# soz223/multi_modal_normative_modeling

Hardware: AMD Instinct MI355X
Metric: cVAE training-steps/sec (batch 256, 379-ROI x 3-modality) (higher is better)
Workload: dtype bf16; 1 GPU; SE-gPoE cVAE_multimodal sweep: 3 x 379 ROI, batch 256, c=29, H=[110,110], Z=10, 5 folds x replicas, 256 independent models per GPU, in-kernel reparameterisation draw; jobs_per_gpu=256, steps_per_launch=128, params_per_model=355437, train_rows_per_model=1024, parallelism=sweep-sharded x1

## Files before the change

include/nmhip.h:

```cpp
#ifndef NMHIP_H
#define NMHIP_H

#include <stddef.h>
#include <stdint.h>

#ifdef __cplusplus
extern "C" {
#endif

#define NM_MAX_MOD 8
#define NM_MAX_EXP 4
#define NM_MAX_CLS 5
#define NM_MAX_CLS_WIDTH 512
#define NM_MAX_CLASSES 4
#define NM_MAX_HID 8
#define NM_BATCH   256
#define NM_MAX_WIDTH 127
#define NM_MAX_LATENT 64
#define NM_WIDE_MAX_WIDTH 4096
#define NM_WIDE_MAX_LATENT 128

enum {
  NM_OK            = 0,
  NM_E_NULL        = -1,
  NM_E_MODALITIES  = -2,
  NM_E_LAYERS      = -3,
  NM_E_WIDTH       = -4,
  NM_E_LATENT      = -5,
  NM_E_LATENT_COV  = -6,
  NM_E_PITCH       = -7,
  NM_E_GEOMETRY    = -8,
  NM_E_COMBINE     = -9,
  NM_E_OFFSETS     = -10,
  NM_E_REG_HEAD    = -11,
  NM_E_METRICS     = -12,
  NM_E_CLS_HEAD    = -13,
  NM_E_COUNTS      = -14,
  NM_E_SHADOW      = -15,
  NM_E_RESIDENCY   = -16,
  NM_E_PREP        = -17,
  NM_E_OUTPUT      = -18,
  NM_E_WIDE_TC     = -19,
  NM_E_ROWSPLIT    = -20,
  NM_E_N_PARAMS    = -21,
  NM_E_DEVPASS     = -22
};

enum { NM_COMBINE_POE = 0, NM_COMBINE_GPOE = 1, NM_COMBINE_MOE = 2, NM_COMBINE_MOPOE = 3,
       NM_COMBINE_POE2V = 4 };

enum {
  NM_F_BACKWARD = 1,
  NM_F_ADAM     = 2,
  NM_F_GRADS    = 4,
  NM_F_EXPORT   = 8,
  NM_F_PROFILE  = 16,
  NM_F_ZGIVEN   = 32,
  NM_F_TRACE    = 64,
  NM_F_BNSTATS  = 256,
  NM_F_SPLIT    = 512,
  NM_F_FAULT_INJECT = 1024
};

typedef struct nm_modality {
  int32_t D;
  int32_t Kx;
  int32_t x_pitch;
  int32_t Cz;
  const float*    x_f32;
  const uint16_t* xb;
  const uint16_t* cz;
  int64_t enc_w[NM_MAX_HID], enc_b[NM_MAX_HID];
  int64_t mu_w, mu_b, lv_w, lv_b;
  int64_t logvar_out;
  int64_t dec_w[NM_MAX_HID], dec_b[NM_MAX_HID];
  int64_t out_w, out_b;
  int64_t alpha;
  int64_t enc_s[NM_MAX_HID];
  int64_t heads_s;
  int64_t dec_s[NM_MAX_HID];
  int64_t out_s;
  float* out_loc;
  float* out_sqerr;
  float* out_rowdev;
  const float* dloc_extra;
  const float* dloc_rowcoef;
} nm_modality_t;

typedef struct nm_job {
  int32_t M;
  int32_t M_enc;
  int32_t C;
  int32_t L;
  int32_t Z;
  int32_t H[NM_MAX_HID];
  int32_t combine;
  int32_t single_bypass;
  int32_t n_rows;
  int32_t non_linear;
  float   act_slope;
  int32_t out_kind;
  int32_t n_private;
  float   var_floor;
  float   tc_weight;
  int64_t w_off;
  int32_t dephase;
  int32_t shared_cov;
  int32_t wide;
  int32_t loss_cap;
  int32_t eps_cap;
  float   lr, beta1, beta2, adam_eps;
  int64_t adam_off;
  const double* lr_table;
  int32_t lr_cap;
  float   kl_weight;
  float   ll_weight;
  float*  params;
  float*  adam_m;
  float*  adam_v;
  float*  grads;
  const float* eps;
  uint64_t seed;
  float*  loss_log;
  void*   wsh;
  void*   workspace;
  int64_t workspace_stride;
  float*  out_mu;
  float*  out_logvar;
  float*  out_z;
  const float* dz_extra;
  int32_t reg_head;
  float   reg_lambda;
  int64_t reg_w[3], reg_b[3];
  int64_t reg_s;
  uint16_t* reg_resid;
  uint16_t* reg_dres;
  const float* fi_target;
  float*  out_fi_pred;
  int32_t cls_layers;
  int32_t cls_classes;
  int32_t cls_width[NM_MAX_CLS];
  int32_t cls_train;
  int32_t cls_use_mu;
  int64_t cls_w[NM_MAX_CLS + 1], cls_b[NM_MAX_CLS + 1];
  int64_t cls_bn_w[NM_MAX_CLS], cls_bn_b[NM_MAX_CLS];
  int64_t cls_bn_mean[NM_MAX_CLS], cls_bn_var[NM_MAX_CLS];
  float   cls_dropout;
  float   cls_margin;
  float   cls_w_ce;
  float   cls_w_contrast;
  const int32_t* labels;
  float*  out_logits;
  float*  dz_out;
  float*  rowcoef_out[NM_MAX_MOD];
  float*  gpart;
  int64_t gpart_stride;
  int64_t n_params;
  nm_modality_t mod[NM_MAX_MOD];
} nm_job_t;

#define NM_LOSS_STRIDE 16
#define NM_LOSS_TOTAL 0
#define NM_LOSS_KL    1
#define NM_LOSS_LL    2
#define NM_LOSS_LL_M  3
#define NM_LOSS_TC    11
#define NM_LOSS_REG   12
#define NM_LOSS_CE    13
#define NM_LOSS_CONTRAST 14

int64_t nm_fill_shadow(nm_job_t* job_host);

int nm_sync_shadow(const nm_job_t* jobs_dev, int n_jobs, void* stream);

int64_t nm_workspace_bytes(const nm_job_t* job_host);

int64_t nm_workspace_offset(const nm_job_t* job_host, int what);

int nm_validate_job(const nm_job_t* job_host);

int nm_launch(const nm_job_t* jobs_dev, int n_jobs, int step0, int steps_per_tile, int n_tiles,
              int flags, void* stream);

int nm_launch_split(const nm_job_t* jobs_dev, int n_jobs, int parts, int step0, int n_steps, int flags, void* stream);
int nm_launch_wide(const nm_job_t* jobs_dev, int n_jobs, int step0, int steps_per_tile, int n_tiles, int flags, void* stream);
int nm_launch_rowsplit(const nm_job_t* jobs_dev, int n_jobs, int M, int k, int helpers, int step0, int n_steps, int flags,
                       int spread_us, void* stream);
int nm_launch_rowsplit_mixed(const nm_job_t* jobs_dev, int n_jobs, const int* job_M_host, int k, int helpers, int step0,
                             int n_steps, int flags, int spread_us, void* stream);
#define NM_RS_MAX_GROUPS 128
#define NM_RS_GROUP_PAD  65535
int nm_rowsplit_groups(const int* job_M_host, int n_jobs, int* table_out, int cap);
#define NM_RS_MAX_PASSES 128
#define NM_RS_MAX_VSEGS  144
#define NM_RS_MAX_VEC    3072
int nm_rowsplit_ok(const nm_job_t* job_host);
int nm_sync_reset(const nm_job_t* jobs_dev, int n_jobs, void* stream);
int nm_devpass(const nm_job_t* jobs_dev, int n_jobs, int tile0, int n_tiles, int flags, void* stream);
int nm_trace_read_dv(unsigned long long* out512, int reset);
int nm_devpass_ok(const nm_job_t* job_host);
int nm_devpass_multi(const nm_job_t* jobs_dev, int n_jobs, int tile0, int n_tiles, int flags, void* stream);
int nm_devpass_multi_ok(const nm_job_t* job_host);
int nm_latent_pass(const nm_job_t* jobs_dev, int n_jobs, int tile0, int n_tiles, int flags, void* stream);
int nm_latent_pass_ok(const nm_job_t* job_host);
int nm_trace_read_rs(unsigned long long* out512, int reset);
#define NM_SYNC_ERR_TIMEOUT 1
#define NM_SYNC_ERR_SHAPE   2
int nm_split_errors(const nm_job_t* jobs_dev, int n_jobs, int* out_dev, int clear, void* stream);

int nm_train_steps(const nm_job_t* jobs_dev, int n_jobs, int step0, int n_steps, void* stream);
int nm_grads(const nm_job_t* jobs_dev, int n_jobs, int step, void* stream);
int nm_forward(const nm_job_t* jobs_dev, int n_jobs, int tile0, int n_tiles, void* stream);

int nm_head_regression(const nm_job_t* jobs_dev, int n_jobs, int step, int tile0, int n_tiles, int flags,
                       void* stream);

int nm_head_classifier(const nm_job_t* jobs_dev, int n_jobs, int step, int tile0, int n_tiles, int flags,
                       void* stream);

int nm_train_steps_head(const nm_job_t* jobs_dev, int n_jobs, int step0, int n_steps, int flags, void* stream);

int nm_train_steps_head_split(const nm_job_t* jobs_dev, int n_jobs, int parts, int step0, int n_steps, int flags, void* stream);

#define NM_METRICS_MAX_N  8192
#define NM_METRICS_STRIDE 8
int nm_posthoc_metrics(const float* scores, const int32_t* labels, const int32_t* offsets, int n_sets, int max_set,
                       const double* thr_in, double* out, void* stream);
int nm_confusion_metrics(const int32_t* pred, const int32_t* labels, const int32_t* offsets, int n_sets, double* out,
                         void* stream);
int nm_latent_stats(const float* mu, const int32_t* offsets, int n_sets, int Z, int pitch, float* mean_out, float* var_out,
                    void* stream);
int nm_latent_score(const float* mu, const float* logvar, const int32_t* offsets, int n_sets, int Z, int pitch,
                    const float* mean, const float* var, float* zsep_out, float* score_out, void* stream);

#define NM_ROI_Y_CHUNK 128
typedef struct { const float* x; const int32_t* group; int32_t rows; int32_t pitch; } nm_roi_set_t;
int nm_roi_effect(const nm_roi_set_t* sets_dev, int n_sets, int D, int max_rows, double* out, void* stream);

#define NM_ROI_MAX_PERM   65535
#define NM_ROI_PERM_CHUNK 64
#define NM_ROI_ROW_CHUNK  256
size_t nm_roi_significance_workspace(int n_sets, int D, int max_rows, int n_perm);
int nm_roi_significance(const nm_roi_set_t* sets_dev, int n_sets, int D, int max_rows, int n_perm, uint64_t seed,
                        void* workspace, size_t workspace_bytes, double* out, int32_t* maxstat_out, void* stream);

#define NM_BOOT_MAX   16384
#define NM_BOOT_CHUNK 64
size_t nm_auc_bootstrap_workspace(int n_sets, int max_set, int n_boot, int n_pairs);
int nm_auc_bootstrap(const float* scores, const int32_t* labels, const int32_t* offsets, const int32_t* streams,
                     int n_sets, int max_set, int n_boot, int lo_index, int hi_index, uint64_t seed,
                     const int32_t* pairs, int n_pairs, void* workspace, size_t workspace_bytes,
                     double* out, double* pairs_out, int32_t* boot_out, void* stream);

#define NM_REG_OLS      0
#define NM_REG_LOGIT    1
#define NM_REG_MAX_COV  4
#define NM_REG_MAX_ITER 35
#define NM_REG_TOL      1e-8
typedef struct nm_reg_set {
  const float*   x;
  const float*   target;
  const float*   cov;
  const int32_t* include;
  int32_t rows, pitch, cov_pitch, pad;
} nm_reg_set_t;
int nm_column_regress(const nm_reg_set_t* sets_dev, int n_sets, int D, int max_rows, int n_cov, int kind,
                      double* out , void* stream);
double nm_student_t_two_sided(double t, double df);

int nm_combine_latent(const float* mus, const float* variances, int M, int64_t n, int combine, const float* alpha_raw,
                      int single_bypass, int in_log, int out_log, float var_floor, float* out_mu, float* out_var,
                      void* stream);
int nm_total_correlation(const float* qz_xs, int M, int B, int Z, float* out, void* stream);

int nm_train_steps_persistent(const nm_job_t* jobs_dev, int n_jobs, int step0, int n_steps, void* stream);
int nm_deviation(const nm_job_t* jobs_dev, int n_jobs, int tile0, int n_tiles, void* stream);

int nm_adam_step(float* params, const float* grads, float* m, float* v, int64_t n,
                 float lr, float beta1, float beta2, float eps, int64_t t, void* stream);

int64_t nm_xb_elems(int rows_alloc, int Kx);
int nm_pack_table(const float* x, const float* c, int n_rows, int rows_alloc, int D, int C, int Kx,
                  uint16_t* xb, float* x_f32_out, int x_pitch, uint16_t* cz_out, int Cz, void* stream);

#define NM_PREP_MAX_ROWS 8192
int nm_prep_scaler_fit(const double* const* srcs_dev, const int32_t* src_D_dev, int n_src, int D, const int32_t* rows_dev,
                       int n_rows, double* center_dev, double* scale_dev, void* stream);
int nm_prep_onehot(const double* age_dev, const double* gender_dev, const int32_t* rows_dev, int n_rows, const double* age_edges_dev,
                   int age_bins, const double* gender_edges_dev, int gender_bins, float* c_out_dev, void* stream);
int nm_pack_table_raw(const double* const* srcs_dev, const int32_t* src_D_dev, int n_src, const int32_t* rows_dev, int n_rows,
// ... 23 lines not shown
```

multi_modal_normative_modeling_amd/_lib.py:

```python
from __future__ import annotations

import ctypes as C
from pathlib import Path

NM_MAX_MOD = 8
NM_MAX_EXP = 4
NM_RS_MAX_PASSES = 128
NM_RS_MAX_VSEGS = 144
NM_RS_MAX_VEC = 3 * 2 * 512
NM_RS_MAX_GROUPS = 128
NM_RS_GROUP_PAD = 65535
NM_MAX_HID = 8
NM_MAX_CLS = 5
NM_MAX_CLS_WIDTH = 512
NM_MAX_CLASSES = 4
NM_BATCH = 256
NM_MAX_WIDTH = 127
NM_MAX_LATENT = 64
NM_WIDE_MAX_WIDTH = 4096
NM_WIDE_MAX_LATENT = 128
NM_LOSS_STRIDE = 16

NM_COMBINE = {"poe": 0, "gpoe": 1, "moe": 2, "mopoe": 3, "poe2v": 4}

NM_F_BACKWARD = 1
NM_F_ADAM = 2
NM_F_GRADS = 4
NM_F_EXPORT = 8
NM_F_PROFILE = 16
NM_F_ZGIVEN = 32
NM_F_TRACE = 64
NM_LOSS_TC = 11
NM_LOSS_REG = 12
NM_LOSS_CE = 13
NM_LOSS_CONTRAST = 14
NM_F_BNSTATS = 256
NM_F_SPLIT = 512
NM_F_FAULT_INJECT = 1024
NM_SYNC_ERR_TIMEOUT = 1
NM_SYNC_ERR_SHAPE = 2
NM_METRICS_MAX_N = 8192
NM_METRICS_STRIDE = 8
NM_ROI_Y_CHUNK = 128
NM_ROI_MAX_PERM = 65535
NM_ROI_PERM_CHUNK = 64
NM_ROI_ROW_CHUNK = 256
NM_BOOT_MAX = 16384
NM_BOOT_CHUNK = 64
NM_REG_OLS = 0
NM_REG_LOGIT = 1
NM_REG_MAX_COV = 4
NM_REG_MAX_ITER = 35
NM_REG_TOL = 1e-8

NM_OK = 0
NM_E_NULL = -1
NM_E_MODALITIES = -2
NM_E_LAYERS = -3
NM_E_WIDTH = -4
NM_E_LATENT = -5
NM_E_LATENT_COV = -6
NM_E_PITCH = -7
NM_E_GEOMETRY = -8
NM_E_COMBINE = -9
NM_E_OFFSETS = -10
NM_E_REG_HEAD = -11
NM_E_METRICS = -12
NM_E_CLS_HEAD = -13
NM_E_COUNTS = -14
NM_E_SHADOW = -15
NM_E_RESIDENCY = -16
NM_E_PREP = -17
NM_E_OUTPUT = -18
NM_E_WIDE_TC = -19
NM_E_ROWSPLIT = -20
NM_E_N_PARAMS = -21
NM_E_DEVPASS = -22

LIB_PATH = Path(__file__).resolve().parent / "libnmhip.so"


class NmModality(C.Structure):
    _fields_ = [
        ("D", C.c_int32), ("Kx", C.c_int32), ("x_pitch", C.c_int32), ("Cz", C.c_int32),
        ("x_f32", C.c_void_p), ("xb", C.c_void_p), ("cz", C.c_void_p),
        ("enc_w", C.c_int64 * NM_MAX_HID), ("enc_b", C.c_int64 * NM_MAX_HID),
        ("mu_w", C.c_int64), ("mu_b", C.c_int64), ("lv_w", C.c_int64), ("lv_b", C.c_int64),
        ("logvar_out", C.c_int64),
        ("dec_w", C.c_int64 * NM_MAX_HID), ("dec_b", C.c_int64 * NM_MAX_HID),
        ("out_w", C.c_int64), ("out_b", C.c_int64),
        ("alpha", C.c_int64),
        ("enc_s", C.c_int64 * NM_MAX_HID), ("heads_s", C.c_int64), ("dec_s", C.c_int64 * NM_MAX_HID), ("out_s", C.c_int64),
        ("out_loc", C.c_void_p), ("out_sqerr", C.c_void_p), ("out_rowdev", C.c_void_p),
        ("dloc_extra", C.c_void_p), ("dloc_rowcoef", C.c_void_p),
    ]


class NmJob(C.Structure):
    _fields_ = [
        ("M", C.c_int32), ("M_enc", C.c_int32), ("C", C.c_int32), ("L", C.c_int32), ("Z", C.c_int32),
        ("H", C.c_int32 * NM_MAX_HID),
        ("combine", C.c_int32), ("single_bypass", C.c_int32), ("n_rows", C.c_int32), ("non_linear", C.c_int32),
        ("act_slope", C.c_float), ("out_kind", C.c_int32), ("n_private", C.c_int32),
        ("var_floor", C.c_float), ("tc_weight", C.c_float), ("w_off", C.c_int64), ("dephase", C.c_int32), ("shared_cov", C.c_int32), ("wide", C.c_int32),
        ("loss_cap", C.c_int32), ("eps_cap", C.c_int32),
        ("lr", C.c_float), ("beta1", C.c_float), ("beta2", C.c_float), ("adam_eps", C.c_float),
        ("adam_off", C.c_int64), ("lr_table", C.c_void_p), ("lr_cap", C.c_int32),
        ("kl_weight", C.c_float), ("ll_weight", C.c_float),
        ("params", C.c_void_p), ("adam_m", C.c_void_p), ("adam_v", C.c_void_p), ("grads", C.c_void_p),
        ("eps", C.c_void_p), ("seed", C.c_uint64),
        ("loss_log", C.c_void_p), ("wsh", C.c_void_p), ("workspace", C.c_void_p), ("workspace_stride", C.c_int64),
        ("out_mu", C.c_void_p), ("out_logvar", C.c_void_p), ("out_z", C.c_void_p), ("dz_extra", C.c_void_p),
        ("reg_head", C.c_int32), ("reg_lambda", C.c_float), ("reg_w", C.c_int64 * 3), ("reg_b", C.c_int64 * 3),
        ("reg_s", C.c_int64), ("reg_resid", C.c_void_p), ("reg_dres", C.c_void_p),
        ("fi_target", C.c_void_p), ("out_fi_pred", C.c_void_p),
        ("cls_layers", C.c_int32), ("cls_classes", C.c_int32), ("cls_width", C.c_int32 * NM_MAX_CLS),
        ("cls_train", C.c_int32), ("cls_use_mu", C.c_int32),
        ("cls_w", C.c_int64 * (NM_MAX_CLS + 1)), ("cls_b", C.c_int64 * (NM_MAX_CLS + 1)),
        ("cls_bn_w", C.c_int64 * NM_MAX_CLS), ("cls_bn_b", C.c_int64 * NM_MAX_CLS),
        ("cls_bn_mean", C.c_int64 * NM_MAX_CLS), ("cls_bn_var", C.c_int64 * NM_MAX_CLS),
        ("cls_dropout", C.c_float), ("cls_margin", C.c_float), ("cls_w_ce", C.c_float), ("cls_w_contrast", C.c_float),
        ("labels", C.c_void_p), ("out_logits", C.c_void_p), ("dz_out", C.c_void_p),
        ("rowcoef_out", C.c_void_p * NM_MAX_MOD),
        ("gpart", C.c_void_p), ("gpart_stride", C.c_int64), ("n_params", C.c_int64),
        ("mod", NmModality * NM_MAX_MOD),
    ]


class NmRoiSet(C.Structure):
    _fields_ = [("x", C.c_void_p), ("group", C.c_void_p), ("rows", C.c_int32), ("pitch", C.c_int32)]


class NmRegSet(C.Structure):
    _fields_ = [("x", C.c_void_p), ("target", C.c_void_p), ("cov", C.c_void_p), ("include", C.c_void_p),
                ("rows", C.c_int32), ("pitch", C.c_int32), ("cov_pitch", C.c_int32), ("pad", C.c_int32)]


class NmError(RuntimeError):
    pass


_lib = None


def load():
    global _lib
    if _lib is not None:
        return _lib
    if not LIB_PATH.exists():
        raise NmError(
            f"{LIB_PATH} is missing: build it with `python -c 'import __graft_entry__ as g; g.build()'` "
            f"(hipcc --offload-arch=gfx950).  There is no CPU fallback for the product path.")
    lib = C.CDLL(str(LIB_PATH))
    vp, i32, i64, f32 = C.c_void_p, C.c_int, C.c_int64, C.c_float
    lib.nm_version.restype = C.c_int
    lib.nm_status_string.restype = C.c_char_p
    lib.nm_status_string.argtypes = [C.c_int]
    lib.nm_abi_sizes.argtypes = [C.POINTER(i64), C.POINTER(i64)]
    lib.nm_workspace_bytes.restype = i64
    lib.nm_fill_shadow.restype = i64
    lib.nm_fill_shadow.argtypes = [C.POINTER(NmJob)]
    lib.nm_sync_shadow.argtypes = [vp, i32, vp]
    lib.nm_xb_elems.restype = i64
    lib.nm_xb_elems.argtypes = [i32, i32]
    lib.nm_workspace_bytes.argtypes = [C.POINTER(NmJob)]
    lib.nm_workspace_offset.restype = i64
    lib.nm_workspace_offset.argtypes = [C.POINTER(NmJob), i32]
    lib.nm_validate_job.argtypes = [C.POINTER(NmJob)]
    for name in ("nm_launch", "nm_launch_scalar_tr"):
        getattr(lib, name).argtypes = [vp, i32, i32, i32, i32, i32, vp]
    lib.nm_launch_split.argtypes = [vp, i32, i32, i32, i32, i32, vp]
    lib.nm_launch_wide.argtypes = [vp, i32, i32, i32, i32, i32, vp]
    lib.nm_split_errors.argtypes = [vp, i32, vp, i32, vp]
    lib.nm_launch_rowsplit.argtypes = [vp, i32, i32, i32, i32, i32, i32, i32, i32, vp]
    lib.nm_launch_rowsplit_mixed.argtypes = [vp, i32, C.POINTER(i32), i32, i32, i32, i32, i32, i32, vp]
    lib.nm_rowsplit_groups.argtypes = [C.POINTER(i32), i32, C.POINTER(i32), i32]
    lib.nm_rowsplit_ok.argtypes = [C.POINTER(NmJob)]
    lib.nm_sync_reset.argtypes = [vp, i32, vp]
    lib.nm_trace_read_rs.argtypes = [C.POINTER(C.c_ulonglong), i32]
    lib.nm_devpass.argtypes = [vp, i32, i32, i32, i32, vp]
    lib.nm_trace_read_dv.argtypes = [C.POINTER(C.c_ulonglong), i32]
    lib.nm_devpass_ok.argtypes = [C.POINTER(NmJob)]
    lib.nm_devpass_multi.argtypes = [vp, i32, i32, i32, i32, vp]
    lib.nm_devpass_multi_ok.argtypes = [C.POINTER(NmJob)]
    lib.nm_latent_pass.argtypes = [vp, i32, i32, i32, i32, vp]
    lib.nm_latent_pass_ok.argtypes = [C.POINTER(NmJob)]
    lib.nm_latent_stats.argtypes = [vp, vp, i32, i32, i32, vp, vp, vp]
    lib.nm_latent_score.argtypes = [vp, vp, vp, i32, i32, i32, vp, vp, vp, vp, vp]
    lib.nm_combine_latent.argtypes = [vp, vp, i32, i64, i32, vp, i32, i32, i32, f32, vp, vp, vp]
    lib.nm_total_correlation.argtypes = [vp, i32, i32, i32, vp, vp]
    lib.nm_train_steps.argtypes = [vp, i32, i32, i32, vp]
    lib.nm_train_steps_persistent.argtypes = [vp, i32, i32, i32, vp]
    lib.nm_deviation.argtypes = [vp, i32, i32, i32, vp]
    lib.nm_grads.argtypes = [vp, i32, i32, vp]
    lib.nm_forward.argtypes = [vp, i32, i32, i32, vp]
    lib.nm_head_regression.argtypes = [vp, i32, i32, i32, i32, i32, vp]
    lib.nm_head_classifier.argtypes = [vp, i32, i32, i32, i32, i32, vp]
    lib.nm_train_steps_head.argtypes = [vp, i32, i32, i32, i32, vp]
    lib.nm_train_steps_head.restype = i32
    lib.nm_train_steps_head_split.argtypes = [vp, i32, i32, i32, i32, i32, vp]
    lib.nm_train_steps_head_split.restype = i32
    lib.nm_posthoc_metrics.argtypes = [vp, vp, vp, i32, i32, vp, vp, vp]
    lib.nm_confusion_metrics.argtypes = [vp, vp, vp, i32, vp, vp]
    lib.nm_roi_effect.argtypes = [vp, i32, i32, i32, vp, vp]
    lib.nm_roi_significance_workspace.restype = C.c_size_t
    lib.nm_roi_significance_workspace.argtypes = [i32, i32, i32, i32]
    lib.nm_roi_significance.argtypes = [vp, i32, i32, i32, i32, C.c_uint64, vp, C.c_size_t, vp, vp, vp]
    lib.nm_auc_bootstrap_workspace.restype = C.c_size_t
    lib.nm_auc_bootstrap_workspace.argtypes = [i32, i32, i32, i32]
    lib.nm_auc_bootstrap.argtypes = [vp, vp, vp, vp, i32, i32, i32, i32, i32, C.c_uint64, vp, i32, vp, C.c_size_t, vp, vp, vp, vp]
    lib.nm_column_regress.argtypes = [vp, i32, i32, i32, i32, i32, vp, vp]
    lib.nm_student_t_two_sided.restype = C.c_double
    lib.nm_student_t_two_sided.argtypes = [C.c_double, C.c_double]
    lib.nm_adam_step.argtypes = [vp, vp, vp, vp, i64, f32, f32, f32, f32, i64, vp]
    lib.nm_pack_table.argtypes = [vp, vp, i32, i32, i32, i32, i32, vp, vp, i32, vp, i32, vp]
    lib.nm_prep_scaler_fit.argtypes = [vp, vp, i32, i32, vp, i32, vp, vp, vp]
    lib.nm_prep_onehot.argtypes = [vp, vp, vp, i32, vp, i32, vp, i32, vp, vp]
    lib.nm_pack_table_raw.argtypes = [vp, vp, i32, vp, i32, vp, vp, vp, i32, i32, i32, i32, vp, vp, i32, vp, i32, vp]
    lib.nm_test_gemm.argtypes = [i32, vp, vp, vp, i32, i32, i32, vp]
    lib.nm_prof_read.argtypes = [C.POINTER(C.c_ulonglong), i32]
    lib.nm_trace_read.argtypes = [C.POINTER(C.c_ulonglong), i32]
    lib.nm_wgtimes_read.argtypes = [C.POINTER(C.c_ulonglong)]
    sj, sm = i64(0), i64(0)
    lib.nm_abi_sizes(C.byref(sj), C.byref(sm))
    if sj.value != C.sizeof(NmJob) or sm.value != C.sizeof(NmModality):
        raise NmError(f"ABI mismatch: C sizeof(nm_job_t)={sj.value}, sizeof(nm_modality_t)={sm.value}; "
                      f"ctypes {C.sizeof(NmJob)}, {C.sizeof(NmModality)}")
    _lib = lib
    return lib


EXPORTED_SYMBOLS = [
    "nm_version", "nm_status_string", "nm_abi_sizes", "nm_workspace_bytes", "nm_validate_job", "nm_launch",
    "nm_launch_scalar_tr", "nm_train_steps", "nm_grads", "nm_forward", "nm_adam_step", "nm_pack_table",
    "nm_test_gemm", "nm_prof_read", "nm_trace_read", "nm_wgtimes_read", "nm_head_regression", "nm_head_classifier", "nm_train_steps_head", "nm_train_steps_head_split", "nm_train_steps_persistent", "nm_deviation", "nm_posthoc_metrics", "nm_confusion_metrics",
    "nm_fill_shadow", "nm_sync_shadow", "nm_xb_elems", "nm_launch_split", "nm_launch_wide", "nm_split_errors", "nm_combine_latent", "nm_total_correlation",
    "nm_prep_scaler_fit", "nm_prep_onehot", "nm_pack_table_raw",
    "nm_launch_rowsplit", "nm_rowsplit_ok", "nm_sync_reset", "nm_trace_read_rs", "nm_devpass", "nm_devpass_ok", "nm_trace_read_dv", "nm_workspace_offset",
    "nm_launch_rowsplit_mixed", "nm_rowsplit_groups", "nm_devpass_multi", "nm_devpass_multi_ok",
    "nm_latent_pass", "nm_latent_pass_ok", "nm_latent_stats", "nm_latent_score",
    "nm_roi_effect", "nm_roi_significance_workspace", "nm_roi_significance",
    "nm_auc_bootstrap_workspace", "nm_auc_bootstrap",
    "nm_column_regress", "nm_student_t_two_sided",
]


def check(status: int, what: str = "nmhip"):
    if status != 0:
        msg = load().nm_status_string(status).decode()
        raise NmError(f"{what} failed with status {status}: {msg}")
```

multi_modal_normative_modeling_amd/csrc/nm_core.inc:

```
#include <hip/hip_runtime.h>
#include <stdint.h>
#include <math.h>
#include "nmhip.h"
#include "nm_host.inc"

namespace {

constexpr int NWM = 2;
constexpr int NWN = 4;
constexpr int NWAVES = NWM * NWN;
constexpr int WG = NWAVES * 64;
constexpr int TROWS = NM_BATCH;
constexpr int RT = NM_BATCH / (NWM * 16);
constexpr int WROWS = RT * 16;
constexpr int ROWS = NM_BATCH;
#define NM_GEOM(RTV)                                                                                              \
  [[maybe_unused]] constexpr int RT = (RTV), WROWS = (RTV) * 16, ROWS = (RTV) * 32, XIMG_BYTES = ROWS * LDX * 2, \
                                 ACT_BYTES = ROWS * LDP * 2
constexpr int PW = 128;
constexpr int LDP = 136;
constexpr int LDX = 72;
constexpr int XCH = 64;
constexpr int STAGE_FLOATS = 4608;
constexpr int IMG_ROWS = 128;
constexpr int IMG_BYTES = IMG_ROWS * LDP * 2;
constexpr int VEC_BYTES = 1024;
constexpr int BLOB_BYTES = IMG_BYTES + VEC_BYTES;
constexpr int XIMG_BYTES = ROWS * LDX * 2;
constexpr int XIMG_TILE_BYTES = TROWS * LDX * 2;
constexpr int W0IMG_BYTES = 128 * LDX * 2;
constexpr int OCH = 64;
constexpr int OIMG_BYTES = OCH * LDP * 2;
constexpr int OBLOB_BYTES = 18432;
constexpr int ACT_BYTES = ROWS * LDP * 2;
constexpr int ROWS_BYTES_P = NM_BATCH * LDP * 2;
constexpr int PATCH_FLOATS = 16 * 16;
constexpr int SPATCH_OFF = 8192;
constexpr float LOG_SQRT_2PI = 0.91893853320467274178f;

typedef __attribute__((ext_vector_type(4))) float f32x4;
typedef __attribute__((ext_vector_type(8))) __bf16 bf16x8;
typedef __attribute__((ext_vector_type(4))) __bf16 bf16x4;
typedef __attribute__((ext_vector_type(4))) unsigned u32x4;

#define GAS __attribute__((address_space(1)))
typedef GAS float* gf32;
typedef const GAS float* gcf32;
typedef GAS __bf16* gbf16;
typedef const GAS __bf16* gcbf16;

__device__ unsigned long long nm_prof_cycles[32];
__device__ unsigned long long nm_trace_cycles[8][64];
__device__ unsigned long long nm_wg_times[512][2];

struct Ctx {
  unsigned long long t_last;
  const nm_job_t* job;
  __bf16* P;
  __bf16* Q;
  float* stage;
  float* vec;
  int part, nparts;
  int rsk, rsq, rloc0;
  int x_pre;
  GAS float* gpart;
  int64_t gp_stride;
  GAS char* ws0;
  int xwg;
  int gwt;
  int lstep;
  float slope;
  float* red;
  float* colacc;
  float* rowacc;
  float* lse;
  float* bgrad;
  unsigned* abort;
  unsigned long long* tlast;
  int wave_s;
  int tid, lane, wave, wm, wn, g, c16;
  int row0;
  int nrows;
  int flags;
  float inv_b;
  float step_size;
  float inv_bc2_sqrt;
  GAS char* ws;
};

__host__ __device__ inline int rup(int x, int m) { return (x + m - 1) / m * m; }
__host__ __device__ inline int wpad(int n) { return rup(n + 1, 32); }

constexpr int WS_RS_TAB_BYTES = 8192;
struct WsLayout {
  int64_t sync, rs_tab, mu_m, lv_m, mu_j, lv_j, es, dz, enc_act, dec_act, zc, total;
  int64_t lat, act;
  int Zs;
};
constexpr int WS_SYNC_BYTES = 256;
constexpr int WS_SYNC_ERR_WORD = 32;
constexpr unsigned WS_SYNC_ERR_TIMEOUT = NM_SYNC_ERR_TIMEOUT, WS_SYNC_ERR_SHAPE = NM_SYNC_ERR_SHAPE;
constexpr int WS_SYNC_C_WORD = 33, WS_SYNC_D_WORD = 40, WS_SYNC_LOSS_WORD = 48, WS_SYNC_XCC_WORD = 57;
__host__ __device__ inline WsLayout ws_layout(int M, int L, int Z) {
  WsLayout w;
  w.Zs = rup(Z, 16);
  int64_t o = 0;
  w.sync = o; o += WS_SYNC_BYTES;
  w.rs_tab = o; o += (int64_t)NM_MAX_EXP * WS_RS_TAB_BYTES;
  const int64_t lat = (int64_t)ROWS * w.Zs * 4;
  w.lat = lat;
  w.mu_m = o; o += lat * M * 2;
  w.lv_m = o; o += lat * M * 2;
  w.mu_j = o; o += lat * M;
  w.lv_j = o; o += lat * M;
  w.es = o; o += lat * M;
  w.dz = o; o += lat * M;
  const int64_t act = (int64_t)ROWS * LDP * 2;
  w.act = act;
  w.enc_act = o; o += act * M * L;
  w.dec_act = o; o += act * M * L;
  w.zc = o; o += act * M;
  w.total = (o + 255) / 256 * 256;
  return w;
}

enum { PH_ENC_L0 = 0, PH_ENC_REST, PH_HEADS, PH_LATENT, PH_DEC_ZC, PH_DEC_HID, PH_OUT_GEMM, PH_OUT_DLV, PH_OUT_DGRAD,
       PH_OUT_WGRAD, PH_NLL_RED, PH_DEC_FINISH, PH_DEC_LOAD, PH_DEC_DGRAD, PH_DEC_WGRAD, PH_DEC_DELTA, PH_ALPHA,
       PH_ENCB_PREP, PH_ENCB_HEADS_DGRAD, PH_ENCB_HEADS_WGRAD, PH_ENCB_LOAD, PH_ENCB_DGRAD, PH_ENCB_WGRAD,
       PH_ENCB_DELTA, PH_ENCB_L0_WGRAD, PH_X_LOADS, PH_X_MFMA, PH_X_EPI, PH_COUNT };
__device__ __forceinline__ void tr(const Ctx& c, int tag) {
  if ((c.flags & 64) && blockIdx.x == 0 && blockIdx.y == 0) {
    unsigned long long t = clock64();
    const int w = c.wave_s;
    nm_trace_cycles[w][tag] += t - c.tlast[w];
    c.tlast[w] = t;
  }
}
__device__ __forceinline__ void prof(Ctx& c, int phase) {
  if ((c.flags & NM_F_PROFILE) && blockIdx.x == 0 && blockIdx.y == 0 && c.wave_s == 0) {
    unsigned long long t = clock64();
    nm_prof_cycles[phase] += t - c.t_last;
    c.t_last = t;
  }
}

__device__ __forceinline__ void relaunder(Ctx& c) {
  int l = (int)__builtin_amdgcn_mbcnt_hi(~0u, __builtin_amdgcn_mbcnt_lo(~0u, 0u));
  asm volatile("" : "+v"(l));
  int w = c.wave_s;
  asm volatile("" : "+s"(w));
  c.lane = l;
  c.tid = w * 64 + l;
  c.wave = w;
  c.wm = w / NWN;
  c.wn = w % NWN;
  c.g = c.lane >> 4;
  c.c16 = c.lane & 15;
}

template <class T>
__device__ __forceinline__ GAS T* asg(T* p) {
  return (GAS T*)p;
}

__device__ __forceinline__ void lds_barrier() {
  asm volatile("s_waitcnt lgkmcnt(0)" ::: "memory");
  __builtin_amdgcn_s_barrier();
}

__device__ __forceinline__ float lrelu(float v, bool nl, float slope) { return (nl && v < 0.f) ? v * slope : v; }

__device__ __forceinline__ float fx_exp(float x) { return __builtin_amdgcn_exp2f(x * 1.4426950408889634f); }
__device__ __forceinline__ float fx_log(float x) { return __builtin_amdgcn_logf(x) * 0.6931471805599453f; }
__device__ __forceinline__ float fx_rcp(float x) { return __builtin_amdgcn_rcpf(x); }

__device__ __forceinline__ unsigned lds_addr(const void* p) {
  return (unsigned)(size_t)(const __attribute__((address_space(3))) void*)p;
}

__device__ __forceinline__ int idiv(int a, int b, float rb) {
  int q = (int)((float)a * rb);
  q += ((q + 1) * b <= a) ? 1 : 0;
  q -= (q * b > a) ? 1 : 0;
  return q;
// ... 674 lines not shown
    for (int rt = 0; rt < RT; ++rt) {
      bf16x8 a = lds_frag(A, lda, c.wm * WROWS + rt * 16 + c.c16, n_col0 + s * 32 + 8 * c.g);
      acc[0][rt] = mfma(wf0, a, acc[0][rt]);
      acc[1][rt] = mfma(wf1, a, acc[1][rt]);
    }
  }
}
template <int RTV>
__device__ __forceinline__ const __bf16* dgrad_hidden(const Ctx& cc, f32x4 (&acc)[2][RTV], const GAS char* w_img,
                                                      const GAS char* act_img, int N, int K) {
  NM_GEOM(RTV);
  Ctx c = cc;
  relaunder(c);
  char* Qb = reinterpret_cast<char*>(c.Q);
  dma_img(c, w_img, Qb, N, blob_kp(K), (const GAS char*)c.job->wsh);
  if (RTV < 8) {
    const int n_act = dma_act(c, act_img, Qb + IMG_BYTES, 0, ROWS, act_segs(K));
    wait_vm(n_act);
    lds_barrier();
    dgrad_tile(c, acc, c.P, LDP, 0, c.Q, LDP, wpad(N) / 32);
    return c.Q + IMG_ROWS * LDP;
  }
  const int n_hi = dma_act(c, act_img, Qb + IMG_BYTES, ROWS / 2, ROWS / 2, act_segs(K));
  wait_vm(n_hi);
  lds_barrier();
  dgrad_tile(c, acc, c.P, LDP, 0, c.Q, LDP, wpad(N) / 32);
  lds_barrier();
  dma_act(c, act_img, Qb, 0, ROWS / 2, act_segs(K));
  return c.Q;
}

template <int RTV>
__device__ __forceinline__ void finish_delta(const Ctx& cc, const f32x4 (&acc)[2][RTV], const __bf16* src, int K,
                                             bool act) {
  NM_GEOM(RTV);
  Ctx c = cc;
  relaunder(c);
  const int ntk = wpad(K) / 16;
#pragma unroll
  for (int t = 0; t < 2; ++t) {
    int kt = c.wn + 4 * t;
    if (kt >= ntk) continue;
    int k0 = kt * 16 + 4 * c.g;
#pragma unroll
    for (int rt = 0; rt < RT; ++rt) {
      int r = c.wm * WROWS + rt * 16 + c.c16;
      bf16x4 a = *reinterpret_cast<const bf16x4*>(src + r * LDP + k0);
      bf16x4 pk;
#pragma unroll
      for (int i = 0; i < 4; ++i) {
        float d = acc[t][rt][i];
        if (act && !((float)a[i] > 0.f)) d *= c.slope;
        if (k0 + i >= K) d = 0.f;
        pk[i] = (__bf16)d;
      }
      *reinterpret_cast<bf16x4*>(c.P + r * LDP + k0) = pk;
    }
  }
}

struct WgT {
  int64_t w_off;
  int64_t b_off;
  GAS char* sh;
  int sh_pitch;
  GAS float* sh_b;
  float* patch;
};
struct WgGeom { int N, K, k_base, ncols; WgT T; };
struct PMV { f32x4 p0, m0, v0, p1, m1, v1; };
__device__ __forceinline__ int wg_units(const WgGeom& G) { return ((G.N + 15) >> 4) * ((((G.ncols + 15) >> 4) + 1) >> 1); }
__device__ __forceinline__ int wg_bias_pair(const WgGeom& G) {
  const bool has_bias = (G.T.b_off >= 0) && (G.K >= G.k_base) && (G.K < G.k_base + G.ncols);
  return has_bias ? ((G.K - G.k_base) >> 5) : -1;
}
#define NM_GLOAD16(dst, voff, sbase) \
  asm volatile("s_nop 4\n\tglobal_load_dwordx4 %0, %1, %2" : "+v"(dst) : "v"(voff), "s"(sbase) : "memory")
#define NM_GLOAD16_NT(dst, voff, sbase) \
  asm volatile("s_nop 4\n\tglobal_load_dwordx4 %0, %1, %2 nt" : "+v"(dst) : "v"(voff), "s"(sbase) : "memory")
#define NM_GLOAD4(dst, voff, sbase) \
  asm volatile("s_nop 4\n\tglobal_load_dword %0, %1, %2" : "+v"(dst) : "v"(voff), "s"(sbase) : "memory")
constexpr int WG_LOADS = 6;

template <bool SCALAR_TR, int RTV = RT, bool PART = false>
__device__ __forceinline__ int wgrad_adam(const Ctx& cc, const __bf16* A, int lda, int a_col0, const __bf16* B, int ldb,
                                          const WgGeom& G, int pending = -1, int b_chunk = 0, float* bgrad_buf = nullptr) {
  NM_GEOM(RTV);
  Ctx c = cc;
  relaunder(c);
  const nm_job_t* J = c.job;
  const WgT& T = G.T;
  const int N = G.N, K = G.K, k_base = G.k_base, ncols = G.ncols;
  const int KT = ktiles(K), kt0 = k_base >> 4;
  const int nktp = (ncols + 15) >> 4;
  const int nkp = (nktp + 1) >> 1;
  const int nunits = wg_units(G);
  const int kb = K - k_base;
  const int kb_pair = wg_bias_pair(G), kb_j = (kb >> 4) & 1, kb_col = kb & 15;
  const bool do_adam = !PART && (c.flags & NM_F_ADAM) != 0;
  const bool do_grads = !PART && (c.flags & NM_F_GRADS) != 0;
  const AdamK ak = adam_consts(c);
  gf32 Pp = asg(J->params), Mp = asg(J->adam_m), Vp = asg(J->adam_v);
  float* patch = T.patch + c.wave * PATCH_FLOATS;
  float* const bgp = bgrad_buf ? bgrad_buf : c.bgrad;
  const int prow = c.lane >> 2, pcol = (c.lane & 3) * 4;
  float* const pw = patch + c.c16 * 16 + 4 * (c.g ^ ((c.c16 >> 1) & 3));
  const float* const pr = patch + prow * 16 + 4 * ((c.lane & 3) ^ ((prow >> 1) & 3));
  const float* const pb = patch + prow * 16 + 4 * ((kb_col >> 2) ^ ((prow >> 1) & 3)) + (kb_col & 3);
  const unsigned lane16 = (unsigned)c.lane << 4;

  const bool bias_wave = kb_pair >= 0 && do_adam && c.wave < 2;
  float bp, bm, bv;
  asm volatile("" : "=v"(bp), "=v"(bm), "=v"(bv));
  if (bias_wave) {
    const unsigned boff = (unsigned)(T.b_off + min(c.tid, N - 1)) << 2;
    NM_GLOAD4(bp, boff, Pp); NM_GLOAD4(bm, boff, Mp); NM_GLOAD4(bv, boff, Vp);
  }
  int young = 0;

  auto issue = [&](int u, PMV& s) {
    const int nt = u / nkp, kp = u - nt * nkp;
    const int ktl0 = 2 * kp, ktl1 = 2 * kp + 1;
    const bool v0 = ktl0 < nktp && kt0 + ktl0 < KT, v1 = ktl1 < nktp && kt0 + ktl1 < KT;
    const unsigned o0 = (v0 ? (unsigned)((T.w_off + ((int64_t)(nt * KT + kt0 + ktl0) << 8)) << 2) : 0u) + lane16;
    const unsigned o1 = (v1 ? (unsigned)((T.w_off + ((int64_t)(nt * KT + kt0 + ktl1) << 8)) << 2) : 0u) + lane16;
    NM_GLOAD16(s.p0, o0, Pp); NM_GLOAD16_NT(s.m0, o0, Mp); NM_GLOAD16_NT(s.v0, o0, Vp);
    NM_GLOAD16(s.p1, o1, Pp); NM_GLOAD16_NT(s.m1, o1, Mp); NM_GLOAD16_NT(s.v1, o1, Vp);
  };
  auto wait_set = [&](PMV& s, int younger) {
    wait_vm(younger);
    asm volatile("" : "+v"(s.p0), "+v"(s.m0), "+v"(s.v0), "+v"(s.p1), "+v"(s.m1), "+v"(s.v1));
  };
  auto unit_mfma = [&](int u, f32x4 (&acc)[2]) {
    const int nt = u / nkp, kp = u - nt * nkp;
    acc[0] = f32x4{0.f, 0.f, 0.f, 0.f}; acc[1] = acc[0];
    const int ncol0 = a_col0 + nt * 16;
    const __bf16* const Bu = b_chunk ? B + (kp >> 1) * b_chunk : B;
    const int kcol = b_chunk ? (kp & 1) * 32 : kp * 32;
    if (SCALAR_TR) {
      for (int rs = 0; rs < ROWS / 32; ++rs) {
        bf16x8 nf = lds_frag_tr_scalar(A, lda, rs * 32, ncol0, c.lane);
        acc[0] = mfma(lds_frag_tr_scalar(Bu, ldb, rs * 32, kcol, c.lane), nf, acc[0]);
        acc[1] = mfma(lds_frag_tr_scalar(Bu, ldb, rs * 32, kcol + 16, c.lane), nf, acc[1]);
      }
    } else {
      unsigned na = tr_addr_il(A, lda, 0, ncol0, c.lane);
      unsigned ka = tr_addr_il(Bu, ldb, 0, kcol, c.lane);
      const unsigned n_step = 32u * lda * 2u, k_step = 32u * ldb * 2u;
      const unsigned n4 = 1u * lda * 2u, k4 = 1u * ldb * 2u;
#pragma unroll 2
      for (int rs = 0; rs < ROWS / 32; rs += 2) {
        bf16x4 n0v, n1v, n2v, n3v, a0, a1, a2, a3, b0, b1, b2, b3;
        unsigned na1 = na + n4, ka1 = ka + k4, na2 = na + n_step, ka2 = ka + k_step;
        unsigned na3 = na2 + n4, ka3 = ka2 + k4;
        NM_TR_READ(n0v, na, 0);  NM_TR_READ(n1v, na1, 0);
        NM_TR_READ(a0, ka, 0);   NM_TR_READ(a1, ka1, 0);
        NM_TR_READ(b0, ka, 32);  NM_TR_READ(b1, ka1, 32);
        NM_TR_READ(n2v, na2, 0); NM_TR_READ(n3v, na3, 0);
        NM_TR_READ(a2, ka2, 0);  NM_TR_READ(a3, ka3, 0);
        NM_TR_READ(b2, ka2, 32); NM_TR_READ(b3, ka3, 32);
        asm volatile("s_waitcnt lgkmcnt(0)"
                     : "+v"(n0v), "+v"(n1v), "+v"(n2v), "+v"(n3v), "+v"(a0), "+v"(a1), "+v"(a2), "+v"(a3), "+v"(b0),
                       "+v"(b1), "+v"(b2), "+v"(b3));
        bf16x8 nf0 = join4(n0v, n1v), nf1 = join4(n2v, n3v);
        acc[0] = mfma(join4(a0, a1), nf0, acc[0]);
        acc[1] = mfma(join4(b0, b1), nf0, acc[1]);
        acc[0] = mfma(join4(a2, a3), nf1, acc[0]);
        acc[1] = mfma(join4(b2, b3), nf1, acc[1]);
        na += 2 * n_step; ka += 2 * k_step;
      }
    }
  };
  auto finish_unit = [&](int u, PMV& s, const f32x4 (&acc)[2]) {
    const int nt = u / nkp, kp = u - nt * nkp;
    const int n = nt * 16 + prow;
    int nst = 0;
    if constexpr (PART) {
      const int nr = nt * 16 + c.c16;
#pragma unroll
      for (int j = 0; j < 2; ++j) {
        const int ktl = 2 * kp + j;
        f32x4 g = acc[j];
        const int k0 = k_base + ktl * 16 + 4 * c.g;
        if (nt * 16 + 16 > N || k_base + ktl * 16 + 16 > K) {
#pragma unroll
          for (int i = 0; i < 4; ++i) g[i] = (nr < N && k0 + i < K) ? g[i] : 0.f;
        }
        if (ktl < nktp && kt0 + ktl < KT) {
          const int64_t idx = T.w_off + ((int64_t)(nt * KT + kt0 + ktl) << 8) + c.c16 * 16 + 4 * c.g;
          st16_g(c, c.gpart + idx, g);
          ++nst;
        }
        if (kp == kb_pair && j == kb_j) {
          if (c.g == (kb_col >> 2) && nr < N) bgp[nr] = acc[j][kb_col & 3];
        }
      }
      return nst;
    }
#pragma unroll
    for (int j = 0; j < 2; ++j) {
      const int ktl = 2 * kp + j;
      *reinterpret_cast<f32x4*>(pw) = acc[j];
      f32x4 g = *reinterpret_cast<const f32x4*>(pr);
      const float bg = *pb;
      const int k0 = k_base + ktl * 16 + pcol;
      if (nt * 16 + 16 > N || k_base + ktl * 16 + 16 > K) {
#pragma unroll
        for (int i = 0; i < 4; ++i) g[i] = (n < N && k0 + i < K) ? g[i] : 0.f;
      }
      if (ktl < nktp && kt0 + ktl < KT) {
        const int64_t idx = T.w_off + ((int64_t)(nt * KT + kt0 + ktl) << 8) + c.lane * 4;
        if (do_grads) { *(GAS f32x4*)(asg(J->grads) + idx) = g; ++nst; }
        if (do_adam) {
          f32x4 p4 = j ? s.p1 : s.p0, m4 = j ? s.m1 : s.m0, v4 = j ? s.v1 : s.v0;
#pragma unroll
          for (int i = 0; i < 4; ++i) { float pp = p4[i], mm = m4[i], v2 = v4[i]; adam1(ak, g[i], pp, mm, v2); p4[i] = pp; m4[i] = mm; v4[i] = v2; }
          *(GAS f32x4*)(Pp + idx) = p4;
          __builtin_nontemporal_store(m4, (GAS f32x4*)(Mp + idx));
          __builtin_nontemporal_store(v4, (GAS f32x4*)(Vp + idx));
          nst += 3;
          if (T.sh) {
            bf16x4 pk;
#pragma unroll
            for (int i = 0; i < 4; ++i) pk[i] = (__bf16)p4[i];
            *(GAS bf16x4*)(T.sh + (int64_t)n * T.sh_pitch + (ktl * 16 + pcol) * 2) = pk;
            ++nst;
          }
        }
      }
      if (kp == kb_pair && j == kb_j) {
        if (pcol == 0 && n < N) bgp[n] = bg;
      }
    }
    return nst;
  };

  PMV sa, sb;
  asm volatile("" : "=v"(sa.p0), "=v"(sa.m0), "=v"(sa.v0), "=v"(sa.p1), "=v"(sa.m1), "=v"(sa.v1));
  asm volatile("" : "=v"(sb.p0), "=v"(sb.m0), "=v"(sb.v0), "=v"(sb.p1), "=v"(sb.m1), "=v"(sb.v1));
  int u = c.wave, st_prev = 0;
  if (do_adam && u < nunits) { issue(u, sa); young += WG_LOADS; }
  if (pending >= 0) {
    wait_vm(min(pending + young + (bias_wave ? 3 : 0), 20));
    lds_barrier();
  }
  while (u < nunits) {
    f32x4 acc[2];
    const int u1 = u + NWAVES, u2 = u + 2 * NWAVES;
    const bool h1 = do_adam && u1 < nunits;
    if (h1) { issue(u1, sb); young += WG_LOADS; }
    unit_mfma(u, acc);
    if (do_adam) wait_set(sa, st_prev + (h1 ? WG_LOADS : 0));
    st_prev = finish_unit(u, sa, acc);
    young += st_prev;
    if (u1 >= nunits) break;
    const bool h2 = do_adam && u2 < nunits;
    if (h2) { issue(u2, sa); young += WG_LOADS; }
    unit_mfma(u1, acc);
    if (do_adam) wait_set(sb, st_prev + (h2 ? WG_LOADS : 0));
    st_prev = finish_unit(u1, sb, acc);
    young += st_prev;
    u = u2;
  }
  lds_barrier();
  if (PART) {
    if (kb_pair >= 0) {
      relaunder(c);
      for (int n = c.tid; n < N; n += WG) st4_g(c, c.gpart + T.b_off + n, bgp[n]);
    }
  } else if (kb_pair >= 0 && c.wave < 2) {
    relaunder(c);
    if (bias_wave) { wait_vm(min(young, 20)); asm volatile("" : "+v"(bp), "+v"(bm), "+v"(bv)); }
    const int n = c.tid;
    if (n < N) {
      const float bg = bgp[n];
      const int64_t bidx = T.b_off + n;
      if (do_grads) asg(J->grads)[bidx] = bg;
      if (do_adam) {
        adam1(ak, bg, bp, bm, bv);
        Pp[bidx] = bp; Mp[bidx] = bm; Vp[bidx] = bv;
        if (T.sh_b) T.sh_b[n] = bp;
      }
    }
  }
  return young;
}

__device__ __forceinline__ WgGeom geom_out(const nm_job_t* J, const nm_modality_t& md, int ch, float* patch) {
  const int Hl = J->H[0], d0 = ch * OCH, valid = min(OCH, md.D - d0);
  GAS char* const oimg = (GAS char*)J->wsh + md.out_s + (int64_t)ch * OBLOB_BYTES;
  return WgGeom{valid, Hl, 0, rup(Hl + 1, 16),
                WgT{md.out_w + (int64_t)(d0 >> 4) * ktiles(Hl) * 256, md.out_b + d0, oimg, LDP * 2, (GAS float*)(oimg + OIMG_BYTES), patch}};
}
__device__ __forceinline__ WgGeom geom_dec(const nm_job_t* J, const nm_modality_t& md, int d, float* patch) {
  const int L = J->L, Kin = (d == 0) ? J->Z + J->C : J->H[L - d], Nout = J->H[L - 1 - d];
  GAS char* const dimg = (GAS char*)J->wsh + md.dec_s[d];
  return WgGeom{Nout, Kin, 0, rup(Kin + 1, 16),
                WgT{md.dec_w[d], md.dec_b[d], dimg, blob_kp(Kin) * 2, (GAS float*)(dimg + cimg_bytes(Nout, Kin)), patch}};
}
__device__ __forceinline__ WgGeom geom_head(const nm_job_t* J, const nm_modality_t& md, int which, float* patch) {
  const int Hh = J->H[J->L - 1], Zs = rup(J->Z, 16), hkp = blob_kp(Hh);
  GAS char* const img = (GAS char*)J->wsh + md.heads_s;
  GAS float* const hvec = (GAS float*)(img + cimg_bytes(2 * Zs, Hh));
  return which == 0 ? WgGeom{J->Z, Hh, 0, rup(Hh + 1, 16), WgT{md.mu_w, md.mu_b, img, hkp * 2, hvec, patch}}
                    : WgGeom{J->Z, Hh, 0, rup(Hh + 1, 16), WgT{md.lv_w, md.lv_b, img + (int64_t)Zs * hkp * 2, hkp * 2, hvec + Zs, patch}};
}
__device__ __forceinline__ WgGeom geom_enc(const nm_job_t* J, const nm_modality_t& md, int e, float* patch) {
  const int Kin = J->H[e - 1], Nout = J->H[e];
  GAS char* const eimg = (GAS char*)J->wsh + md.enc_s[e];
  return WgGeom{Nout, Kin, 0, rup(Kin + 1, 16),
                WgT{md.enc_w[e], md.enc_b[e], eimg, blob_kp(Kin) * 2, (GAS float*)(eimg + cimg_bytes(Nout, Kin)), patch}};
}
__device__ __forceinline__ WgGeom geom_l0(const nm_job_t* J, const nm_modality_t& md, int kc, float* patch) {
  const int Kx = md.Kx, K0 = md.D + J->C, N0 = J->H[0];
  GAS char* const img = (GAS char*)J->wsh + md.enc_s[0];
  return WgGeom{N0, K0, kc * XCH, min(XCH, Kx - kc * XCH),
                WgT{md.enc_w[0], md.enc_b[0], img + (int64_t)kc * XCH * 2, Kx * 2, (GAS float*)(img + l0_img_bytes(N0, Kx)), patch}};
}

__device__ __forceinline__ int experts(const nm_job_t* J) { return J->M_enc > 0 ? J->M_enc : J->M; }
__host__ __device__ inline int head_chunk0(const nm_job_t* J, int m) {
  int q = 0;
  for (int i = 0; i < m; ++i) q += (J->mod[i].D + XCH - 1) / XCH;
  return q;
}
struct Fuse { float mu, lv, var; };
struct Lat { float mu[NM_MAX_EXP], lv[NM_MAX_EXP]; };
__device__ __forceinline__ void softmax_alpha(const nm_job_t* J, float (&al)[NM_MAX_EXP]) {
#pragma clang fp contract(off)
  float mx = -INFINITY;
#pragma unroll
  for (int m = 0; m < NM_MAX_EXP; ++m)
    if (m < experts(J)) mx = fmaxf(mx, asg(J->params)[J->mod[m].alpha]);
  float s = 0.f;
#pragma unroll
  for (int m = 0; m < NM_MAX_EXP; ++m) {
    al[m] = (m < experts(J)) ? fx_exp(asg(J->params)[J->mod[m].alpha] - mx) : 0.f;
    s += al[m];
  }
  const float rs_ = fx_rcp(s);
#pragma unroll
  for (int m = 0; m < NM_MAX_EXP; ++m) al[m] *= rs_;
}
__device__ __forceinline__ Fuse fuse_fwd(const nm_job_t* J, const Lat& L, const float (&al)[NM_MAX_EXP]) {
#pragma clang fp contract(off)
  const int M = experts(J);
  Fuse f;
  if (M == 1 && J->single_bypass) { f.mu = L.mu[0]; f.var = fx_exp(L.lv[0]); f.lv = fx_log(f.var); return f; }
  const int cb = J->combine;
  float S = 0.f, Smu = 0.f, sm = 0.f, sv = 0.f;
#pragma unroll
  for (int m = 0; m < NM_MAX_EXP; ++m) {
    if (m < M) {
      float var = fx_exp(L.lv[m]);
      float w = (cb == NM_COMBINE_POE2V) ? fx_exp(-var) : ((cb == NM_COMBINE_GPOE) ? al[m] * fx_rcp(var) : fx_rcp(var));
      S += w; Smu += L.mu[m] * w;
      sm += L.mu[m]; sv += var;
    }
  }
  if (cb == NM_COMBINE_MOE) { f.mu = sm * fx_rcp((float)M); f.var = sv * fx_rcp((float)M); }
  else {
    f.var = fx_rcp(S); f.mu = Smu * f.var;
    if (cb == NM_COMBINE_MOPOE) { f.mu = (sm + f.mu) * fx_rcp((float)(M + 1)); f.var = (sv + f.var) * fx_rcp((float)(M + 1)); }
    if (cb == NM_COMBINE_POE2V) f.var = fx_log(fx_rcp(S));
  }
  if (J->var_floor > 0.f) f.var = fmaxf(f.var, J->var_floor);
  f.lv = fx_log(f.var);
  return f;
}
struct FuseGrad { float dmu[NM_MAX_EXP], dlv[NM_MAX_EXP], dal[NM_MAX_EXP]; };
__device__ __forceinline__ FuseGrad fuse_bwd(const nm_job_t* J, const Lat& L, const float (&al)[NM_MAX_EXP], float dmu_j,
                                             float dlv_j) {
#pragma clang fp contract(off)
  const int M = experts(J);
  FuseGrad G;
#pragma unroll
  for (int m = 0; m < NM_MAX_EXP; ++m) { G.dmu[m] = 0.f; G.dlv[m] = 0.f; G.dal[m] = 0.f; }
  if (M == 1 && J->single_bypass) { G.dmu[0] = dmu_j; G.dlv[0] = dlv_j; return G; }
  const int cb = J->combine;
  float S = 0.f, Smu = 0.f, sv = 0.f;
#pragma unroll
  for (int m = 0; m < NM_MAX_EXP; ++m) {
    if (m < M) {
      float w = (cb == NM_COMBINE_POE2V) ? fx_exp(-fx_exp(L.lv[m])) : fx_exp(-L.lv[m]) * ((cb == NM_COMBINE_GPOE) ? al[m] : 1.0f);
      S += w; Smu += L.mu[m] * w;
      sv += fx_exp(L.lv[m]);
    }
  }
  if (J->var_floor > 0.f) {
    const float var_p0 = fx_rcp(S);
    const float var_u = (cb == NM_COMBINE_MOE) ? sv * fx_rcp((float)M) : (cb == NM_COMBINE_MOPOE) ? (sv + var_p0) * fx_rcp((float)(M + 1))
                        : (cb == NM_COMBINE_POE2V) ? fx_log(var_p0) : var_p0;
    if (!(var_u > J->var_floor)) dlv_j = 0.f;
  }
  if (cb == NM_COMBINE_POE2V) {
    const float rS = fx_rcp(S), mu_p = Smu * rS, u = fx_log(rS);
#pragma unroll
    for (int m = 0; m < NM_MAX_EXP; ++m) {
      if (m < M) {
        const float v = fx_exp(L.lv[m]), r = fx_exp(-v) * rS;
        G.dmu[m] = dmu_j * r;
        G.dlv[m] = -dmu_j * (L.mu[m] - mu_p) * r * v + dlv_j * r * v * fx_rcp(u);
      }
    }
    return G;
  }
  if (cb == NM_COMBINE_MOE) {
#pragma unroll
    for (int m = 0; m < NM_MAX_EXP; ++m)
      if (m < M) { G.dmu[m] = dmu_j * fx_rcp((float)M); G.dlv[m] = dlv_j * fx_exp(L.lv[m]) * fx_rcp(sv); }
    return G;
  }
  const float var_p = fx_rcp(S), mu_p = Smu * var_p;
  float dmu_p = dmu_j, dlv_p = dlv_j, e_mu = 0.f, e_lv = 0.f;
  if (cb == NM_COMBINE_MOPOE) {
    float var_j = (sv + var_p) * fx_rcp((float)(M + 1));
    dmu_p = dmu_j * fx_rcp((float)(M + 1));
    dlv_p = dlv_j * var_p * fx_rcp((M + 1) * var_j);
    e_mu = dmu_j * fx_rcp((float)(M + 1));
    e_lv = dlv_j * fx_rcp((M + 1) * var_j);
  }
#pragma unroll
  for (int m = 0; m < NM_MAX_EXP; ++m) {
    if (m < M) {
      float pm = fx_exp(-L.lv[m]);
      float r = var_p * pm * ((cb == NM_COMBINE_GPOE) ? al[m] : 1.0f);
      G.dmu[m] = dmu_p * r + e_mu;
      G.dlv[m] = -dmu_p * r * (L.mu[m] - mu_p) + dlv_p * r + e_lv * fx_exp(L.lv[m]);
      if (cb == NM_COMBINE_GPOE) G.dal[m] = dmu_p * var_p * pm * (L.mu[m] - mu_p) - dlv_p * var_p * pm;
    }
  }
  return G;
}
__device__ __forceinline__ float pick(const float (&a)[NM_MAX_EXP], int m) {
  float r = a[0];
#pragma unroll
  for (int q = 1; q < NM_MAX_EXP; ++q) {
    float t = (q == m) ? a[q] : r;
    asm volatile("" : "+v"(t));
    r = t;
  }
  return r;
}

template <bool SCALAR_TR, int MODE = 0, int RTV = RT>
__device__ __forceinline__ void run_step(Ctx& c, int step) {
  NM_GEOM(RTV);
  constexpr bool RS = RTV < 8;
  static_assert(!RS || MODE == 0, "row-split instantiations run the one-pass train step only");
  const nm_job_t* J = c.job;
  const int M = J->M, L = J->L, Z = J->Z, C = J->C;
  const int Me = experts(J);
  const bool nl = J->non_linear != 0;
  const bool bwd = MODE != 1 && MODE != 3 && (c.flags & NM_F_BACKWARD) != 0;
  constexpr bool FWD_ONLY = MODE == 1 || MODE == 3;
  const bool save = bwd || MODE == 1;
  const bool exportf = MODE != 2 && (c.flags & NM_F_EXPORT) != 0;
  const WsLayout wl = ws_layout(M, L, Z);
  const int Zs = wl.Zs;
  const bool split = c.part >= 0;
  const int part = split ? c.part : 0;
  const int S = J->n_private, Zc = Z - S;
  const float rZc = Zc > 0 ? 1.0f / (float)Zc : 0.f;
  const bool vec4 = S == 0 && (Z & 3) == 0;
  const bool fastlat = MODE == 3 && M == 1 && Me == 1 && J->single_bypass != 0 && !split && S == 0 && J->tc_weight == 0.f &&
                       J->w_off < 0 && !(c.flags & NM_F_ZGIVEN) && wl.Zs <= 32 &&
                       !((c.flags & NM_F_EXPORT) && (J->out_mu || J->out_logvar || J->out_z));
  __bf16* const zlds = reinterpret_cast<__bf16*>(c.stage);
  float kl_fast = 0.f;
  const bool sigm = J->out_kind == 1;
  gf32 ws_mu_m = (gf32)(c.ws + wl.mu_m + (int64_t)(step & 1) * M * wl.lat);
  gf32 ws_lv_m = (gf32)(c.ws + wl.lv_m + (int64_t)(step & 1) * M * wl.lat);
  gf32 ws_mu_j = (gf32)(c.ws + wl.mu_j + part * wl.lat);
  gf32 ws_lv_j = (gf32)(c.ws + wl.lv_j + part * wl.lat);
  gf32 ws_es = (gf32)(c.ws + wl.es + part * wl.lat);
  gf32 ws_dz0 = (gf32)(c.ws + wl.dz);
  GAS char* ws_enc = c.ws + wl.enc_act;
  GAS char* ws_dec0 = c.ws + wl.dec_act + (int64_t)part * L * wl.act;
  GAS char* ws_zc0 = c.ws + wl.zc + part * wl.act;
  GAS unsigned* sync_a = (GAS unsigned*)((RS ? c.ws0 : c.ws) + wl.sync) + (RS ? c.rsq : 0);
  GAS unsigned* sync_b = sync_a + 16;
  GAS unsigned* sync_err = (GAS unsigned*)((RS ? c.ws0 : c.ws) + wl.sync) + WS_SYNC_ERR_WORD;
  const unsigned sync_target = (unsigned)(c.lstep + 1) * (unsigned)c.nparts;
  GAS char* wsh = (GAS char*)J->wsh;
  char* const Sb = reinterpret_cast<char*>(c.stage);
  char* const Qb = reinterpret_cast<char*>(c.Q);
  char* const Pb = reinterpret_cast<char*>(c.P);

  tr(c, 17);
  for (int m = 0; m < (MODE == 2 ? 0 : Me); ++m) {
    if (split && m != part) continue;
    relaunder(c);
    const nm_modality_t& md = J->mod[m];
    gbf16 save0 = save ? (gbf16)(ws_enc + (int64_t)(m * L + 0) * ACT_BYTES) : (gbf16)nullptr;
    const GAS char* after0 = wsh + (L > 1 ? md.enc_s[1] : md.heads_s);
    fwd_first_layer<RTV>(c, (const GAS char*)asg(md.xb) + (int64_t)(c.row0 / TROWS) * ((md.Kx + XCH - 1) / XCH) * XIMG_TILE_BYTES +
                                (int64_t)c.rloc0 * (LDX * 2), md.Kx,
                         wsh + md.enc_s[0], blob_to_half(c, after0, 0, L > 1 ? J->H[1] : 2 * Zs, J->H[0]), J->H[0], nl, save0, true,
                         W0IMG_BYTES >> 10, 1 << 30, RS ? c.x_pre : 0);
    prof(c, PH_ENC_L0);
    int half = 0;
    for (int e = 1; e < L; ++e) {
      gbf16 sv = save ? (gbf16)(ws_enc + (int64_t)(m * L + e) * ACT_BYTES) : (gbf16)nullptr;
      const GAS char* nxt = wsh + (e + 1 < L ? md.enc_s[e + 1] : md.heads_s);
      fwd_layer<RTV>(c, half, blob_to_half(c, nxt, half ^ 1, e + 1 < L ? J->H[e + 1] : 2 * Zs, J->H[e]), J->H[e], J->H[e - 1], nl, sv,
                     save ? act_stores<RTV>(act_segs(J->H[e - 1])) : 0);
      half ^= 1;
    }
    tr(c, 1);
    prof(c, PH_ENC_REST);
    fwd_heads<RTV>(c, half, no_next(), Z, J->H[L - 1], ws_mu_m + (int64_t)m * ROWS * Zs, ws_lv_m + (int64_t)m * ROWS * Zs, Zs,
                   save ? act_stores<RTV>(act_segs(J->H[L - 1])) : 0, fastlat ? zlds : (__bf16*)nullptr, step, vec4, &kl_fast);
    prof(c, PH_HEADS);
  }

  if (split && c.nparts > 1) { if (!split_handoff(c, sync_a, sync_err, sync_target)) return; }
  else handoff_barrier();
  if (MODE != 2) issue_next(c, blob_to_half(c, wsh + J->mod[split ? part : 0].dec_s[0], 0, J->H[L - 1], Z + C));
  float al[NM_MAX_EXP] = {0.f, 0.f, 0.f, 0.f};
  if (J->combine == NM_COMBINE_GPOE && !(Me == 1 && J->single_bypass)) softmax_alpha(J, al);
  auto load_lat = [&](Lat& Lt, int r, int z) {
#pragma unroll
    for (int m = 0; m < NM_MAX_EXP; ++m) {
      Lt.mu[m] = (m < Me) ? ws_mu_m[((int64_t)m * ROWS + r) * Zs + z] : 0.f;
      Lt.lv[m] = (m < Me) ? ws_lv_m[((int64_t)m * ROWS + r) * Zs + z] : 0.f;
    }
  };
  float tc = 0.f;
  if (MODE != 2 && J->tc_weight != 0.f) {
    relaunder(c);
    for (int col = c.wave; col < Me * Z; col += NWAVES) {
      const int m = col / Z, z = col - m * Z;
      float v[4], mx = -3.0e38f;
#pragma unroll
      for (int k = 0; k < 4; ++k) {
        const int r = c.lane + 64 * k;
        const float x = ws_mu_m[((int64_t)m * ROWS + min(r, c.nrows - 1)) * Zs + z];
        v[k] = (r < c.nrows) ? x : -3.0e38f;
        mx = fmaxf(mx, v[k]);
      }
#pragma unroll
      for (int o = 32; o > 0; o >>= 1) mx = fmaxf(mx, __shfl_xor(mx, o, 64));
      float sx = 0.f;
#pragma unroll
      for (int k = 0; k < 4; ++k) sx += (c.lane + 64 * k < c.nrows) ? expf(v[k] - mx) : 0.f;
#pragma unroll
      for (int o = 32; o > 0; o >>= 1) sx += __shfl_xor(sx, o, 64);
      if (c.lane == 0) c.lse[col] = mx + logf(sx);
    }
    lds_barrier();
    for (int z = 0; z < Z; ++z) {
      float sm_ = 0.f;
      for (int m = 0; m < Me; ++m) sm_ += c.lse[m * Z + z];
      tc -= sm_ / (float)Me;
    }
  }
  float kl_w = J->kl_weight;
  if (J->w_off >= 0) {
    kl_w = 0.f;
    for (int m = 0; m < M; ++m) kl_w += asg(J->params)[J->w_off + m];
  }
  float kl_part = 0.f;
  relaunder(c);
  if (fastlat) {
    kl_part = kl_fast;
  } else if (vec4) {
    const int nq4 = (Z + 3) >> 2;
    const float rq4 = 1.0f / (float)nq4;
#pragma unroll 2
    for (int e = c.tid; e < (MODE == 2 ? 0 : ROWS * nq4); e += WG) {
      const int r = idiv(e, nq4, rq4), z0 = 4 * (e - r * nq4);
      f32x4 mu4[NM_MAX_EXP], lv4[NM_MAX_EXP];
#pragma unroll
      for (int m = 0; m < NM_MAX_EXP; ++m) {
        mu4[m] = f32x4{0.f, 0.f, 0.f, 0.f};
        lv4[m] = mu4[m];
        if (m < Me) {
          mu4[m] = *(const GAS f32x4*)(ws_mu_m + ((int64_t)m * ROWS + r) * Zs + z0);
          lv4[m] = *(const GAS f32x4*)(ws_lv_m + ((int64_t)m * ROWS + r) * Zs + z0);
        }
      }
      float ep[4];
      if (J->eps) {
#pragma unroll
        for (int i = 0; i < 4; ++i) ep[i] = asg(J->eps)[((int64_t)(step % J->eps_cap) * TROWS + c.rloc0 + r) * Z + min(z0 + i, Z - 1)];
      } else {
        randn2_ctr(J->seed, (uint32_t)step, (uint32_t)(c.row0 + r), (uint32_t)(z0 >> 1), ep[0], ep[1]);
        randn2_ctr(J->seed, (uint32_t)step, (uint32_t)(c.row0 + r), (uint32_t)(z0 >> 1) + 1u, ep[2], ep[3]);
      }
#pragma unroll
      for (int i = 0; i < 4; ++i) ep[i] = (z0 + i < Z) ? ep[i] : 0.f;
      f32x4 omu, olv, oes;
#pragma unroll
      for (int i = 0; i < 4; ++i) {
        Lat Lt;
#pragma unroll
        for (int m = 0; m < NM_MAX_EXP; ++m) { Lt.mu[m] = mu4[m][i]; Lt.lv[m] = lv4[m][i]; }
        Fuse f = fuse_fwd(J, Lt, al);
        float es = ep[i] * fx_exp(0.5f * f.lv);
        if (c.flags & NM_F_ZGIVEN) { f.mu = ep[i]; es = 0.f; }
        omu[i] = f.mu; olv[i] = f.lv; oes[i] = es;
        if (r < c.nrows && z0 + i < Z) {
          kl_part += -0.5f * (1.0f + f.lv - f.mu * f.mu - fx_exp(f.lv));
          if (exportf && part == 0) {
            int64_t gr = (int64_t)(c.row0 + r) * Z + z0 + i;
            if (J->out_mu) asg(J->out_mu)[gr] = f.mu;
            if (J->out_logvar) asg(J->out_logvar)[gr] = f.lv;
            if (J->out_z) asg(J->out_z)[gr] = f.mu + es;
          }
        }
      }
      *(GAS f32x4*)(ws_mu_j + r * Zs + z0) = omu;
      *(GAS f32x4*)(ws_lv_j + r * Zs + z0) = olv;
      *(GAS f32x4*)(ws_es + r * Zs + z0) = oes;
    }
  } else {
#pragma unroll 2
  for (int e = c.tid; e < (MODE == 2 ? 0 : ROWS * Zc); e += WG) {
    int r = idiv(e, Zc, rZc), z = e - r * Zc;
    Lat Lt;
    load_lat(Lt, r, S + z);
    Fuse f = fuse_fwd(J, Lt, al);
    float ep = J->eps ? asg(J->eps)[((int64_t)(step % J->eps_cap) * TROWS + c.rloc0 + r) * Z + z]
                      : randn_ctr(J->seed, (uint32_t)step, (uint32_t)(c.row0 + r), (uint32_t)z);
    float es = ep * fx_exp(0.5f * f.lv);
    if (c.flags & NM_F_ZGIVEN) { f.mu = ep; es = 0.f; }
    float zz = f.mu + es;
    ws_mu_j[r * Zs + z] = f.mu;
    ws_lv_j[r * Zs + z] = f.lv;
    ws_es[r * Zs + z] = es;
    if (r < c.nrows) {
      kl_part += -0.5f * (1.0f + f.lv - f.mu * f.mu - fx_exp(f.lv));
      if (exportf && part == 0) {
        int64_t gr = (int64_t)(c.row0 + r) * Z + z;
        if (J->out_mu) asg(J->out_mu)[gr] = f.mu;
        if (J->out_logvar) asg(J->out_logvar)[gr] = f.lv;
        if (J->out_z) asg(J->out_z)[gr] = zz;
      }
    }
  }
  }
  float kl = (MODE == 2) ? 0.f : block_sum(c, kl_part) * c.inv_b;
  GAS float* const lpart = (GAS float*)(c.ws + wl.sync) + WS_SYNC_LOSS_WORD;
  if (RS && c.tid == 0 && part == 0) st4_wt(lpart, kl);
  if (fastlat) lds_barrier();
  else handoff_barrier();
  tr(c, 3);
  prof(c, PH_LATENT);

  float ll_sum = 0.f;
  for (int m = 0; m < M; ++m) {
    if (split && m != part) continue;
    relaunder(c);
    const nm_modality_t& md = J->mod[m];
    const int D = md.D;
    const int Kd0 = Z + C;
    const int nck = (D + OCH - 1) / OCH;
    const GAS char* oblob = wsh + md.out_s;
    const bool reuse_zc = J->shared_cov && M > 1 && !split && S == 0;
    const bool part_slot = (MODE == 1 || MODE == 2) && split;
    GAS char* const ws_dec = ws_dec0 + ((MODE != 0 && !part_slot) ? (int64_t)m * L * wl.act : 0);
    GAS char* const ws_zc = ws_zc0 + ((MODE != 0 && !part_slot && !reuse_zc) ? (int64_t)m * wl.act : 0);
    if (MODE == 2) {
      lds_barrier();
      dma_act(c, ws_dec + (int64_t)(L - 1) * ACT_BYTES, Pb, 0, ROWS, act_segs(J->H[0]));
      dma_lin(c, oblob, Sb, OBLOB_BYTES >> 10);
    } else {
    if (m > 0 && !split) issue_next(c, blob_to_half(c, wsh + md.dec_s[0], 0, J->H[L - 1], Z + C));
    if (m == 0 || !reuse_zc) {
      build_zc<RTV>(c, c.P, md, ws_mu_j, ws_es, Z, C, Zs, S, ws_mu_m + (int64_t)min(m, Me - 1) * ROWS * Zs,
                    fastlat ? zlds : (const __bf16*)nullptr);
      lds_barrier();
      if (save || reuse_zc) store_act_img<RTV>(c, (gbf16)ws_zc, c.P, act_segs(Kd0));
    } else {
      dma_act(c, ws_zc, Pb, 0, ROWS, act_segs(Kd0));
    }
    tr(c, 4);
    prof(c, PH_DEC_ZC);
    int half = 0;
    for (int d = 0; d < L; ++d) {
      int Kin = (d == 0) ? Kd0 : J->H[L - d];
      int Nout = J->H[L - 1 - d];
      gbf16 sv = (save && (d < L - 1 || MODE == 1)) ? (gbf16)(ws_dec + (int64_t)d * ACT_BYTES) : (gbf16)nullptr;
      Next nx = (d + 1 < L) ? blob_to_half(c, wsh + md.dec_s[d + 1], half ^ 1, J->H[L - 2 - d], Nout)
                            : Next{oblob, Sb, OBLOB_BYTES >> 10, nullptr, nullptr, 0, 0};
      fwd_layer<RTV>(c, half, nx, Nout, Kin, nl, sv, (d > 0 && save) ? act_stores<RTV>(act_segs(Kin)) : 0);
      half ^= 1;
    }
    }
    tr(c, 5);
    prof(c, PH_DEC_HID);
    const int Hl = J->H[0];
    gcf32 xf = asg(md.x_f32);
    const int xp = md.x_pitch;
    constexpr int DEF_PITCH = 6 * OCH + 8;
    const bool deferred = RS && RTV == 2 && nck <= 6;
    static_assert(!(RS && RTV == 2) || (RTV * 32 * DEF_PITCH * 2 + OBLOB_BYTES <= ROWS_BYTES_P), "deferred output-layer layout of Q");
    __bf16* const Dq = c.Q;
    const int dpitch = deferred ? DEF_PITCH : LDX;
    char* const slotA = deferred ? Qb + ROWS * DEF_PITCH * 2 : Qb + XIMG_BYTES;
    float* const opatch = deferred ? reinterpret_cast<float*>(Pb + ROWS * LDP * 2) : reinterpret_cast<float*>(Qb + XIMG_BYTES + OBLOB_BYTES);
    f32x4 accg[2][RT];
    zero_acc(accg);
    float nll_part = 0.f;
    if (exportf && md.out_rowdev) { for (int r = c.tid; r < ROWS; r += WG) c.rowacc[r] = 0.f; }
    constexpr int NRC = MODE == 2 ? RT : 1, NRD = FWD_ONLY ? RT : 1;
    float rcv[NRC], rdev[NRD];
#pragma unroll
    for (int rt = 0; rt < NRD; ++rt) rdev[rt] = 0.f;
#pragma unroll
    for (int rt = 0; rt < NRC; ++rt)
      rcv[rt] = (MODE == 2 && md.dloc_rowcoef) ? asg(md.dloc_rowcoef)[c.row0 + c.wm * WROWS + rt * 16 + c.c16] : 0.f;
    const float ll_w = (J->w_off >= 0) ? asg(J->params)[J->w_off + m] : J->ll_weight;
    const float llw_b = ll_w * c.inv_b;
    const int hq_all = (J->reg_head && m < Me) ? head_chunk0(J, Me) : 0;
    const int64_t hq_m = (J->reg_head && m < Me) ? head_chunk0(J, m) : 0;
    GAS char* const res_out = (exportf && hq_all > 0 && J->reg_resid)
        ? (GAS char*)asg(J->reg_resid) + ((int64_t)(c.row0 / TROWS) * hq_all + hq_m) * XIMG_TILE_BYTES : (GAS char*)nullptr;
    const GAS char* const dres_in = (MODE == 2 && hq_all > 0 && J->reg_dres)
        ? (const GAS char*)asg(J->reg_dres) + hq_m * XIMG_TILE_BYTES : (const GAS char*)nullptr;
    int young_prev = RT;
    auto load_xin = [&](int chx, f32x4 (&xv)[RT]) {
      const int dcl = min(chx * OCH + c.wn * 16 + 4 * c.g, xp - 4);
#pragma unroll
      for (int rt = 0; rt < RT; ++rt)
        xv[rt] = *(const GAS f32x4*)(xf + (int64_t)(c.row0 + c.wm * WROWS + rt * 16 + c.c16) * xp + dcl);
    };
    auto chunk = [&](const int ch, f32x4 (&xin)[RT], f32x4 (&xnx)[RT]) {
      relaunder(c);
      const int d0 = ch * OCH;
      const int valid = min(OCH, D - d0);
      char* const slot = (ch & 1) ? slotA : Sb;
      char* const other = (ch & 1) ? Sb : slotA;
      const __bf16* Wc = reinterpret_cast<const __bf16*>(slot);
      const float* vb = reinterpret_cast<const float*>(slot + OIMG_BYTES);
      const WgGeom Go = geom_out(J, md, ch, opatch);
      if (c.tid < OCH) c.colacc[c.tid] = 0.f;
      const bool lvo_adam = !RS && bwd && (c.flags & NM_F_ADAM) && !sigm && c.wave == 0;
      float lvp, lvm, lvv;
      asm volatile("" : "=v"(lvp), "=v"(lvm), "=v"(lvv));
      if (lvo_adam) {
        const unsigned lo = (unsigned)(md.logvar_out + d0 + min(c.tid, valid - 1)) << 2;
        gf32 Pq = asg(J->params), Mq = asg(J->adam_m), Vq = asg(J->adam_v);
        NM_GLOAD4(lvp, lo, Pq); NM_GLOAD4(lvm, lo, Mq); NM_GLOAD4(lvv, lo, Vq);
      }
      wait_vm(ch > 0 ? min(young_prev + (lvo_adam ? 3 : 0), 20) : 0);
      lds_barrier();
      int n_blob = 0;
      if (ch + 1 < nck) n_blob = dma_lin(c, oblob + (int64_t)(ch + 1) * OBLOB_BYTES, other, OBLOB_BYTES >> 10);
      const int dl0 = c.wn * 16 + 4 * c.g;
      const int dg0 = d0 + dl0;
      if (!FWD_ONLY && !RS) load_xin(ch, xin);
      bf16x4 exh[RT];
      if (MODE == 2 && dres_in) {
#pragma unroll
        for (int rt = 0; rt < RT; ++rt)
          exh[rt] = *(const GAS bf16x4*)(dres_in + (int64_t)ch * XIMG_TILE_BYTES + ((c.wm * WROWS + rt * 16 + c.c16) * LDX + dl0) * 2);
      }
      f32x4 acc[RT];
#pragma unroll
      for (int rt = 0; rt < RT; ++rt) acc[rt] = f32x4{0.f, 0.f, 0.f, 0.f};
      {
        const int ksteps = wpad(Hl) / 32;
#pragma unroll
        for (int ks = 0; ks < 4; ++ks) {
          if (ks < ksteps) {
            const bf16x8 wf = lds_frag(Wc, LDP, c.wn * 16 + c.c16, ks * 32 + 8 * c.g);
#pragma unroll
            for (int rt = 0; rt < RT; ++rt) {
              bf16x8 a = lds_frag(c.P, LDP, c.wm * WROWS + rt * 16 + c.c16, ks * 32 + 8 * c.g);
              acc[rt] = mfma(wf, a, acc[rt]);
            }
          }
        }
      }
      tr(c, 6);
      if (RS && ch + 1 < nck) load_xin(ch + 1, xnx);
      if (FWD_ONLY) {
        wait_vm(ch > 0 ? young_prev - RT + n_blob : 0);
        if (ch + 1 < nck) load_xin(ch + 1, xnx);
      }
      {
        const f32x4 bo = *reinterpret_cast<const f32x4*>(vb + dl0);
        const f32x4 sv = *reinterpret_cast<const f32x4*>(vb + OCH + dl0);
        float inv[4], colq[4], coef[4];
#pragma unroll
        for (int i = 0; i < 4; ++i) {
          inv[i] = sigm ? 1.0f : expf(-sv[i]);
          colq[i] = 0.f;
          coef[i] = (dg0 + i < D) ? llw_b * inv[i] : 0.f;
        }
        int nvalid = 0;
#pragma unroll
        for (int rt = 0; rt < RT; ++rt) {
          const int r = c.wm * WROWS + rt * 16 + c.c16;
          const bool rv = r < c.nrows;
          nvalid += rv ? 1 : 0;
          acc[rt] += bo;
          float dsig[4] = {1.f, 1.f, 1.f, 1.f};
          if (sigm) {
#pragma unroll
            for (int i = 0; i < 4; ++i) {
              const float sg = 1.0f / (1.0f + expf(-acc[rt][i]));
              acc[rt][i] = sg;
              dsig[i] = sg * (1.0f - sg);
            }
          }
          bf16x4 pk;
          f32x4 ex = {0.f, 0.f, 0.f, 0.f};
          if (md.dloc_extra)
            ex = *(const GAS f32x4*)(asg(md.dloc_extra) + (int64_t)(c.row0 + r) * xp + min(dg0, xp - 4));
          if (MODE == 2 && dres_in) {
#pragma unroll
            for (int i = 0; i < 4; ++i) ex[i] += (float)exh[rt][i];
          }
          float rc = rcv[MODE == 2 ? rt : 0];
          if (MODE != 2 && md.dloc_rowcoef) rc = asg(md.dloc_rowcoef)[c.row0 + r];
#pragma unroll
          for (int i = 0; i < 4; ++i) {
            const float diff = rv ? acc[rt][i] - xin[rt][i] : 0.f;
            colq[i] = fmaf(diff, diff, colq[i]);
            const bool dv = dg0 + i < D;
            pk[i] = (__bf16)((diff * (coef[i] + (dv ? rc : 0.f)) + ((rv && dv) ? ex[i] : 0.f)) * dsig[i]);
          }
          if (bwd) *reinterpret_cast<bf16x4*>(Dq + r * dpitch + (deferred ? d0 : 0) + dl0) = pk;
          if (res_out) {
            bf16x4 rk;
#pragma unroll
            for (int i = 0; i < 4; ++i) rk[i] = (__bf16)((rv && dg0 + i < D) ? xin[rt][i] - acc[rt][i] : 0.f);
            *(GAS bf16x4*)(res_out + (int64_t)ch * XIMG_TILE_BYTES + (r * LDX + dl0) * 2) = rk;
          }
        }
        float colsum[4];
#pragma unroll
        for (int i = 0; i < 4; ++i) {
          const bool dv = dg0 + i < D;
          const float hq = 0.5f * inv[i] * colq[i];
          nll_part += dv ? hq + (sigm ? 0.f : (float)nvalid * (0.5f * sv[i] + LOG_SQRT_2PI)) : 0.f;
          colsum[i] = dv ? 0.5f * (float)nvalid - hq : 0.f;
        }
        const bool wave_cols = d0 + c.wn * 16 < xp;
        if (exportf && (FWD_ONLY ? wave_cols : dg0 < xp)) {
#pragma unroll
          for (int rt = 0; rt < RT; ++rt) {
            const int r = c.wm * WROWS + rt * 16 + c.c16;
            const bool rv = r < c.nrows;
            if (FWD_ONLY || rv) {
              f32x4 lo, sq;
              float rs = 0.f;
#pragma unroll
              for (int i = 0; i < 4; ++i) {
                const bool dv = dg0 + i < D && rv;
                const float xh = acc[rt][i], diff = xh - xin[rt][i];
                lo[i] = dv ? xh : 0.f;
                sq[i] = dv ? diff * diff : 0.f;
                rs += sq[i];
              }
              const int64_t gi = (int64_t)(c.row0 + r) * xp + dg0;
              if (!FWD_ONLY || dg0 < xp) {
                if (md.out_loc) *(GAS f32x4*)(asg(md.out_loc) + gi) = lo;
                if (md.out_sqerr) *(GAS f32x4*)(asg(md.out_sqerr) + gi) = sq;
              }
              if (FWD_ONLY) rdev[FWD_ONLY ? rt : 0] += rs;
              else if (md.out_rowdev) atomicAdd(&c.rowacc[r], rs);
            }
          }
        }
        if (FWD_ONLY)
          young_prev = RT + (res_out ? RT : 0) +
                       ((exportf && wave_cols) ? RT * ((md.out_loc ? 1 : 0) + (md.out_sqerr ? 1 : 0)) : 0);
        if (bwd) {
#pragma unroll
          for (int i = 0; i < 4; ++i) {
            float s = colsum[i];
            s += __shfl_xor(s, 1, 64);
            s += __shfl_xor(s, 2, 64);
            s += __shfl_xor(s, 4, 64);
            s += __shfl_xor(s, 8, 64);
            if (c.c16 == 0 && dg0 + i < D) atomicAdd(&c.colacc[dl0 + i], s);
          }
        }
      }
      prof(c, PH_X_EPI);
      tr(c, 7);
      if (!bwd) return;
      lds_barrier();
      relaunder(c);
      if (lvo_adam) {
        asm volatile("" : "+v"(lvp), "+v"(lvm), "+v"(lvv));
        if (c.tid < valid) {
          const float g = ll_w * c.colacc[c.tid] * c.inv_b;
          const int64_t idx = md.logvar_out + d0 + c.tid;
          if (c.flags & NM_F_GRADS) asg(J->grads)[idx] = g;
          adam1(adam_consts(c), g, lvp, lvm, lvv);
          asg(J->params)[idx] = lvp; asg(J->adam_m)[idx] = lvm; asg(J->adam_v)[idx] = lvv;
          ((GAS float*)(oblob + (int64_t)ch * OBLOB_BYTES + OIMG_BYTES))[OCH + c.tid] = lvp;
        }
      } else if (RS) {
        if (c.tid < valid && !sigm) st4_g(c, c.gpart + md.logvar_out + d0 + c.tid, ll_w * c.colacc[c.tid] * c.inv_b);
      } else if (c.tid < valid && !sigm) {
        apply_grad(c, md.logvar_out + d0 + c.tid, ll_w * c.colacc[c.tid] * c.inv_b,
                   (GAS float*)(oblob + (int64_t)ch * OBLOB_BYTES + OIMG_BYTES) + OCH + c.tid);
      }
      dgrad_tile(c, accg, Dq, dpitch, deferred ? d0 : 0, Wc, LDP, OCH / 32);
      tr(c, 8);
      prof(c, PH_OUT_DGRAD);
      const int n_wg = deferred ? 0 : wgrad_adam<SCALAR_TR, RTV, RS>(c, Dq, LDX, 0, c.P, LDP, Go);
      young_prev = RT + n_wg;
      tr(c, 9);
      prof(c, PH_OUT_WGRAD);
    };
    if (FWD_ONLY) {
      f32x4 xa[RT], xb[RT];
      load_xin(0, xa);
      for (int ch = 0; ch < nck; ch += 2) {
        chunk(ch, xa, xb);
        if (ch + 1 < nck) chunk(ch + 1, xb, xa);
      }
    } else if (RS) {
      f32x4 xa[RT], xb[RT];
      load_xin(0, xa);
      for (int ch = 0; ch < nck; ch += 2) {
        chunk(ch, xa, xb);
        if (ch + 1 < nck) chunk(ch + 1, xb, xa);
      }
    } else {
      f32x4 xa[RT];
      for (int ch = 0; ch < nck; ++ch) chunk(ch, xa, xa);
    }
    if constexpr (RS) {
      if (exportf && md.out_rowdev) {
        lds_barrier();
        for (int r = c.tid; r < c.nrows; r += WG) asg(md.out_rowdev)[c.row0 + r] = c.rowacc[r] / (float)D;
        lds_barrier();
      }
      if (deferred && bwd) {
        WgGeom Gall = geom_out(J, md, 0, opatch);
        Gall.N = D;
        wgrad_adam<SCALAR_TR, RTV, true>(c, Dq, DEF_PITCH, 0, c.P, LDP, Gall, -1, 0, c.rowacc);
        tr(c, 9);
      }
    }
    float nll = block_sum(c, nll_part);
    float ll_this = -nll * c.inv_b;
    if (J->w_off >= 0) {
      if (c.tid == 0 && bwd) apply_grad(c, J->w_off + m, kl - ll_this, nullptr);
      ll_this *= ll_w;
    }
    ll_sum += ll_this;
    if (RS) { if (c.tid == 0) st4_wt(lpart + 1 + m, ll_this); }
    else if (c.tid == 0 && J->loss_log)
      asg(J->loss_log)[(int64_t)(step % J->loss_cap) * NM_LOSS_STRIDE + NM_LOSS_LL_M + m] = ll_this;
    prof(c, PH_NLL_RED);
    if (!RS && exportf && md.out_rowdev) {
      if (FWD_ONLY) {
#pragma unroll
        for (int rt = 0; rt < NRD; ++rt) {
          float v = rdev[rt];
          v += __shfl_xor(v, 16, 64);
          v += __shfl_xor(v, 32, 64);
          if (c.g == 0) atomicAdd(&c.rowacc[c.wm * WROWS + rt * 16 + c.c16], v);
        }
      }
      lds_barrier();
      for (int r = c.tid; r < c.nrows; r += WG) asg(md.out_rowdev)[c.row0 + r] = c.rowacc[r] / (float)D;
    }
    if (!bwd) { lds_barrier(); continue; }

    finish_delta(c, accg, c.P, Hl, nl);
    lds_barrier();
    prof(c, PH_DEC_FINISH);
    float* const spatch = reinterpret_cast<float*>(Sb + SPATCH_OFF);
    for (int d = L - 1; d >= 0; --d) {
      relaunder(c);
      int Kin = (d == 0) ? Kd0 : J->H[L - d];
      int Nout = J->H[L - 1 - d];
      f32x4 acc[2][RT];
      zero_acc(acc);
      const GAS char* act_img = d == 0 ? ws_zc : ws_dec + (int64_t)(d - 1) * ACT_BYTES;
      GAS char* const dimg = wsh + md.dec_s[d];
      const WgGeom Gd = geom_dec(J, md, d, spatch);
      const __bf16* const Qact = dgrad_hidden(c, acc, dimg, act_img, Nout, Kin);
      tr(c, 10);
      prof(c, PH_DEC_DGRAD);
      wgrad_adam<SCALAR_TR, RTV, RS>(c, c.P, LDP, 0, Qact, LDP, Gd, 0);
      tr(c, 11);
      prof(c, PH_DEC_WGRAD);
      if (d > 0) {
        finish_delta(c, acc, Qact, Kin, nl);
        lds_barrier();
      } else {
        const int ntk = wpad(Kin) / 16;
#pragma unroll
        for (int t = 0; t < 2; ++t) {
          int kt = c.wn + 4 * t;
          if (kt >= ntk) continue;
          int k0 = kt * 16 + 4 * c.g;
          if (k0 < Z) {
#pragma unroll
            for (int rt = 0; rt < RT; ++rt) {
              int r = c.wm * WROWS + rt * 16 + c.c16;
              st16_x(c, ws_dz0 + (int64_t)m * ROWS * Zs + r * Zs + k0, acc[t][rt]);
            }
          }
        }
        lds_barrier();
      }
      prof(c, PH_DEC_DELTA);
    }
  }

  if (split && c.nparts > 1) { if (!split_handoff(c, sync_b, sync_err, sync_target)) return; }
  else handoff_barrier();
  if (!RS && MODE != 2 && c.tid == 0 && J->loss_log && part == 0) {
    gf32 row = asg(J->loss_log) + (int64_t)(step % J->loss_cap) * NM_LOSS_STRIDE;
    if (split) {
      ll_sum = 0.f;
      for (int m = 0; m < M; ++m) ll_sum += row[NM_LOSS_LL_M + m];
    }
    const float llw_tot = (J->w_off >= 0) ? 1.0f : J->ll_weight;
    row[NM_LOSS_KL] = kl_w * kl;
    row[NM_LOSS_LL] = ll_sum;
    row[NM_LOSS_TC] = tc;
    row[NM_LOSS_TOTAL] = kl_w * kl - llw_tot * ll_sum + J->tc_weight * tc;
  }
  if (!bwd) return;
  if (split && part >= Me) return;
  prof(c, PH_ALPHA);
  auto load_dz = [&](int r, int z) {
    float dq[NM_MAX_MOD];
#pragma unroll
    for (int q = 0; q < NM_MAX_MOD; ++q) dq[q] = (q < M) ? ws_dz0[(int64_t)q * ROWS * Zs + r * Zs + z] : 0.f;
    float d = dq[0];
#pragma unroll
    for (int q = 1; q < NM_MAX_MOD; ++q) d += dq[q];
    return d;
  };
  auto load_dz4 = [&](int r, int z0) {
    f32x4 dq[NM_MAX_MOD];
#pragma unroll
    for (int q = 0; q < NM_MAX_MOD; ++q) {
      dq[q] = f32x4{0.f, 0.f, 0.f, 0.f};
      if (q < M) dq[q] = *(const GAS f32x4*)(ws_dz0 + (int64_t)q * ROWS * Zs + r * Zs + z0);
    }
    f32x4 d = dq[0];
#pragma unroll
    for (int q = 1; q < NM_MAX_MOD; ++q) d += dq[q];
    return d;
  };

  const bool fused = !(Me == 1 && J->single_bypass);
  const float klw = kl_w * c.inv_b;
  const float tcw = J->tc_weight / (float)Me;
  gbf16 ws_fz = (gbf16)ws_zc0;
  const bool once = fused && Me >= 2 && Me * 2 * Zs <= PW && !split && S == 0;
  const bool once_ws = fused && Me >= 2 && !once && 2 * Zs <= PW && !split && S == 0;
  if (once || once_ws || (fused && J->combine == NM_COMBINE_GPOE && !split)) {
    relaunder(c);
    float dal[NM_MAX_EXP] = {0.f, 0.f, 0.f, 0.f};
    if (once) {
      const int npz = Zs - Z, cols = Me * 2 * npz;
      const float rc_ = cols > 0 ? 1.0f / (float)cols : 0.f;
      for (int e = c.tid; e < ROWS * cols; e += WG) {
        const int r = idiv(e, cols, rc_), j = e - r * cols;
        const int blk = idiv(j, npz, 1.0f / (float)npz), k = j - blk * npz;
        c.Q[r * LDP + blk * Zs + Z + k] = (__bf16)0.0f;
      }
    }
    if (once_ws && Zs > Z) {
      const int npz = Zs - Z, cols = Me * 2 * npz;
      const float rc_ = 1.0f / (float)cols;
      for (int e = c.tid; e < ROWS * cols; e += WG) {
        const int r = idiv(e, cols, rc_), j = e - r * cols;
        const int blk = idiv(j, npz, 1.0f / (float)npz), k = j - blk * npz;
        ((gbf16)(ws_zc0 + (int64_t)(blk >> 1) * wl.act))[r * PW + (blk & 1) * Zs + Z + k] = (__bf16)0.0f;
      }
    }
    if (vec4) {
      const int nq4 = (Z + 3) >> 2;
      const float rq4 = 1.0f / (float)nq4;
      for (int e = c.tid; e < ROWS * nq4; e += WG) {
        const int r = idiv(e, nq4, rq4), z0 = 4 * (e - r * nq4);
        f32x4 mu4[NM_MAX_EXP], lv4[NM_MAX_EXP];
#pragma unroll
        for (int m = 0; m < NM_MAX_EXP; ++m) {
          mu4[m] = f32x4{0.f, 0.f, 0.f, 0.f};
          lv4[m] = mu4[m];
          if (m < Me) {
            mu4[m] = *(const GAS f32x4*)(ws_mu_m + ((int64_t)m * ROWS + r) * Zs + z0);
            lv4[m] = *(const GAS f32x4*)(ws_lv_m + ((int64_t)m * ROWS + r) * Zs + z0);
          }
        }
        const f32x4 mj4 = *(const GAS f32x4*)(ws_mu_j + r * Zs + z0), lj4 = *(const GAS f32x4*)(ws_lv_j + r * Zs + z0);
        const f32x4 es4 = *(const GAS f32x4*)(ws_es + r * Zs + z0);
        f32x4 dz4 = load_dz4(r, z0);
        if (J->dz_extra) {
#pragma unroll
          for (int i = 0; i < 4; ++i) dz4[i] += asg(J->dz_extra)[(int64_t)(c.row0 + r) * Z + min(z0 + i, Z - 1)];
        }
        bf16x4 pmu[NM_MAX_EXP], plv[NM_MAX_EXP];
        const bool rv = r < c.nrows;
#pragma unroll
        for (int i = 0; i < 4; ++i) {
          Lat Lt;
#pragma unroll
          for (int m = 0; m < NM_MAX_EXP; ++m) { Lt.mu[m] = mu4[m][i]; Lt.lv[m] = lv4[m][i]; }
          const float dmu_j = dz4[i] + klw * mj4[i];
          const float dlv_j = 0.5f * dz4[i] * es4[i] + klw * 0.5f * (fx_exp(lj4[i]) - 1.0f);
          FuseGrad G = fuse_bwd(J, Lt, al, dmu_j, dlv_j);
          const bool ok = rv && z0 + i < Z;
#pragma unroll
          for (int m = 0; m < NM_MAX_EXP; ++m) {
            dal[m] += ok ? G.dal[m] : 0.f;
            if ((once || once_ws) && m < Me) {
              if (tcw != 0.f) G.dmu[m] -= tcw * expf(Lt.mu[m] - c.lse[m * Z + min(z0 + i, Z - 1)]);
              pmu[m][i] = (__bf16)(ok ? G.dmu[m] : 0.f);
              plv[m][i] = (__bf16)(ok ? G.dlv[m] : 0.f);
            }
          }
        }
#pragma unroll
        for (int m = 0; m < NM_MAX_EXP; ++m) {
          if (once && m < Me) {
            *reinterpret_cast<bf16x4*>(c.Q + r * LDP + m * 2 * Zs + z0) = pmu[m];
            *reinterpret_cast<bf16x4*>(c.Q + r * LDP + m * 2 * Zs + Zs + z0) = plv[m];
          }
          if (once_ws && m < Me) {
            gbf16 blk = (gbf16)(ws_zc0 + (int64_t)m * wl.act);
            *(GAS bf16x4*)(blk + r * PW + z0) = pmu[m];
            *(GAS bf16x4*)(blk + r * PW + Zs + z0) = plv[m];
          }
        }
      }
    } else {
      for (int e = c.tid; e < ROWS * Zc; e += WG) {
        int r = idiv(e, Zc, rZc), z = e - r * Zc;
        Lat Lt;
        load_lat(Lt, r, S + z);
        float mj = ws_mu_j[r * Zs + z], lj = ws_lv_j[r * Zs + z], es = ws_es[r * Zs + z], dz = load_dz(r, z);
        if (J->dz_extra) dz += asg(J->dz_extra)[(int64_t)(c.row0 + r) * Z + z];
        float dmu_j = dz + klw * mj;
        float dlv_j = 0.5f * dz * es + klw * 0.5f * (fx_exp(lj) - 1.0f);
        FuseGrad G = fuse_bwd(J, Lt, al, dmu_j, dlv_j);
        const bool rv = r < c.nrows;
  #pragma unroll
        for (int m = 0; m < NM_MAX_EXP; ++m) {
          dal[m] += rv ? G.dal[m] : 0.f;
          if (once && m < Me) {
            if (tcw != 0.f) G.dmu[m] -= tcw * expf(Lt.mu[m] - c.lse[m * Z + z]);
            c.Q[r * LDP + m * 2 * Zs + z] = (__bf16)(rv ? G.dmu[m] : 0.f);
            c.Q[r * LDP + m * 2 * Zs + Zs + z] = (__bf16)(rv ? G.dlv[m] : 0.f);
          }
          if (once_ws && m < Me) {
            if (tcw != 0.f) G.dmu[m] -= tcw * expf(Lt.mu[m] - c.lse[m * Z + z]);
            gbf16 blk = (gbf16)(ws_zc0 + (int64_t)m * wl.act);
            blk[r * PW + z] = (__bf16)(rv ? G.dmu[m] : 0.f);
            blk[r * PW + Zs + z] = (__bf16)(rv ? G.dlv[m] : 0.f);
          }
        }
      }
    }
    if (J->combine == NM_COMBINE_GPOE) {
      float tot[NM_MAX_EXP];
#pragma unroll
      for (int m = 0; m < NM_MAX_EXP; ++m) tot[m] = block_sum(c, dal[m]);
      if (c.tid == 0) {
        float dot = 0.f;
#pragma unroll
        for (int m = 0; m < NM_MAX_EXP; ++m) dot += al[m] * tot[m];
#pragma unroll
        for (int m = 0; m < NM_MAX_EXP; ++m)
          if (m < Me && (!split || m == part)) apply_grad(c, J->mod[m].alpha, al[m] * (tot[m] - dot), nullptr);
      }
    }
    lds_barrier();
    if (once) store_act<RTV>(c, ws_fz, c.Q, Me * 2 * Zs);
    handoff_barrier();
  }
  tr(c, 12);

  float* const spatch = reinterpret_cast<float*>(Sb + SPATCH_OFF);
  for (int m = 0; m < Me; ++m) {
    if (split && m != part) continue;
    relaunder(c);
    const nm_modality_t& md = J->mod[m];
    const int Hh = J->H[L - 1];
    const int whp = rup(2 * Zs, 32);
    const GAS char* act_last = ws_enc + (int64_t)(m * L + (L - 1)) * ACT_BYTES;
    dma_img(c, wsh + md.heads_s, Qb, 2 * Zs, blob_kp(Hh), (const GAS char*)J->wsh);
    if (RS) dma_act(c, act_last, Qb + IMG_BYTES, 0, ROWS, act_segs(Hh));
    else dma_act(c, act_last, Qb + IMG_BYTES, ROWS / 2, ROWS / 2, act_segs(Hh));
    const __bf16* Qact = RS ? c.Q + IMG_ROWS * LDP : c.Q;
    if (once || once_ws) {
      const int segs = (2 * Zs) >> 3;
      const float rs_ = 1.0f / (float)segs;
      gcbf16 src = once ? (gcbf16)(ws_fz + m * 2 * Zs) : (gcbf16)(ws_zc0 + (int64_t)m * wl.act);
      for (int p_ = c.tid; p_ < ROWS * segs; p_ += WG) {
        const int row = idiv(p_, segs, rs_), seg = p_ - row * segs;
        *reinterpret_cast<u32x4*>(c.P + row * LDP + seg * 8) = *(const GAS u32x4*)(src + row * PW + seg * 8);
      }
    } else {
      float dal_s[NM_MAX_EXP] = {0.f, 0.f, 0.f, 0.f};
      const int npad = whp - 2 * Z;
      const float rnp = npad > 0 ? 1.0f / (float)npad : 0.f;
      for (int e = c.tid; e < ROWS * npad; e += WG) {
        int r = idiv(e, npad, rnp), j = e - r * npad;
        int k = (j < Zs - Z) ? Z + j : Zs + Z + (j - (Zs - Z));
        c.P[r * LDP + k] = (__bf16)0.0f;
      }
      for (int e = c.tid; e < ROWS * S; e += WG) {
        const int r = e / S, i = e - r * S;
        const float d = ws_dz0[(int64_t)m * ROWS * Zs + r * Zs + Zc + i];
        c.P[r * LDP + i] = (__bf16)(r < c.nrows ? d : 0.f);
        c.P[r * LDP + Zs + i] = (__bf16)0.0f;
      }
      if (vec4) {
        const int nq4 = (Z + 3) >> 2;
        const float rq4 = 1.0f / (float)nq4;
        for (int e = c.tid; e < ROWS * nq4; e += WG) {
          const int r = idiv(e, nq4, rq4), z0 = 4 * (e - r * nq4);
          f32x4 mu4[NM_MAX_EXP], lv4[NM_MAX_EXP];
#pragma unroll
          for (int q = 0; q < NM_MAX_EXP; ++q) {
            mu4[q] = f32x4{0.f, 0.f, 0.f, 0.f};
            lv4[q] = mu4[q];
            if (q < Me) {
              mu4[q] = *(const GAS f32x4*)(ws_mu_m + ((int64_t)q * ROWS + r) * Zs + z0);
              lv4[q] = *(const GAS f32x4*)(ws_lv_m + ((int64_t)q * ROWS + r) * Zs + z0);
            }
          }
          const f32x4 mj4 = *(const GAS f32x4*)(ws_mu_j + r * Zs + z0), lj4 = *(const GAS f32x4*)(ws_lv_j + r * Zs + z0);
          const f32x4 es4 = *(const GAS f32x4*)(ws_es + r * Zs + z0);
          f32x4 dz4 = load_dz4(r, z0);
          if (J->dz_extra) {
#pragma unroll
            for (int i = 0; i < 4; ++i) dz4[i] += asg(J->dz_extra)[(int64_t)(c.row0 + r) * Z + min(z0 + i, Z - 1)];
          }
          bf16x4 pmu, plv;
          const bool rv = r < c.nrows;
#pragma unroll
          for (int i = 0; i < 4; ++i) {
            Lat Lt;
#pragma unroll
            for (int q = 0; q < NM_MAX_EXP; ++q) { Lt.mu[q] = mu4[q][i]; Lt.lv[q] = lv4[q][i]; }
            const float dmu_j = dz4[i] + klw * mj4[i];
            const float dlv_j = 0.5f * dz4[i] * es4[i] + klw * 0.5f * (fx_exp(lj4[i]) - 1.0f);
            FuseGrad G = fuse_bwd(J, Lt, al, dmu_j, dlv_j);
            const bool ok = rv && z0 + i < Z;
            float dmu_m = pick(G.dmu, m);
            if (tcw != 0.f) dmu_m -= tcw * expf(pick(Lt.mu, m) - c.lse[m * Z + min(z0 + i, Z - 1)]);
            pmu[i] = (__bf16)(ok ? dmu_m : 0.f);
            plv[i] = (__bf16)(ok ? pick(G.dlv, m) : 0.f);
#pragma unroll
            for (int q = 0; q < NM_MAX_EXP; ++q) dal_s[q] += ok ? G.dal[q] : 0.f;
          }
          *reinterpret_cast<bf16x4*>(c.P + r * LDP + z0) = pmu;
          *reinterpret_cast<bf16x4*>(c.P + r * LDP + Zs + z0) = plv;
        }
      } else {
#pragma unroll 2
        for (int e = c.tid; e < ROWS * Zc; e += WG) {
          int r = idiv(e, Zc, rZc), z = e - r * Zc;
          Lat Lt;
          load_lat(Lt, r, S + z);
          float mj = ws_mu_j[r * Zs + z], lj = ws_lv_j[r * Zs + z], es = ws_es[r * Zs + z], dz = load_dz(r, z);
          if (J->dz_extra) dz += asg(J->dz_extra)[(int64_t)(c.row0 + r) * Z + z];
          float dmu_j = dz + klw * mj;
          float dlv_j = 0.5f * dz * es + klw * 0.5f * (fx_exp(lj) - 1.0f);
          FuseGrad G = fuse_bwd(J, Lt, al, dmu_j, dlv_j);
          const bool rv = r < c.nrows;
          float dmu_m = pick(G.dmu, m);
          if (tcw != 0.f) dmu_m -= tcw * expf(pick(Lt.mu, m) - c.lse[m * Z + z]);
          c.P[r * LDP + S + z] = (__bf16)(rv ? dmu_m : 0.f);
          c.P[r * LDP + Zs + S + z] = (__bf16)(rv ? pick(G.dlv, m) : 0.f);
#pragma unroll
          for (int q = 0; q < NM_MAX_EXP; ++q) dal_s[q] += rv ? G.dal[q] : 0.f;
        }
      }
      if (split && fused && J->combine == NM_COMBINE_GPOE) {
        float tot[NM_MAX_EXP];
#pragma unroll
        for (int q = 0; q < NM_MAX_EXP; ++q) tot[q] = block_sum(c, dal_s[q]);
        if (c.tid == 0) {
          float dot = 0.f;
#pragma unroll
          for (int q = 0; q < NM_MAX_EXP; ++q) dot += al[q] * tot[q];
          if (RS) st4_g(c, c.gpart + md.alpha, pick(al, m) * (pick(tot, m) - dot));
          else apply_grad(c, md.alpha, pick(al, m) * (pick(tot, m) - dot), nullptr);
        }
      }
    }
    wait_vm(0);
    lds_barrier();
    prof(c, PH_ENCB_PREP);
    f32x4 acc[2][RT];
    zero_acc(acc);
    dgrad_tile(c, acc, c.P, LDP, 0, c.Q, LDP, (2 * Zs) / 32);
    lds_barrier();
    prof(c, PH_ENCB_HEADS_DGRAD);
    if (!RS) dma_act(c, act_last, Qb, 0, ROWS / 2, act_segs(Hh));
    tr(c, 13);
    {
      const WgGeom Gm = geom_head(J, md, 0, spatch);
      wgrad_adam<SCALAR_TR, RTV, RS>(c, c.P, LDP, 0, Qact, LDP, Gm, 0);
      const WgGeom Gl = geom_head(J, md, 1, spatch);
      wgrad_adam<SCALAR_TR, RTV, RS>(c, c.P, LDP, Zs, Qact, LDP, Gl, 0);
    }
    prof(c, PH_ENCB_HEADS_WGRAD);
    finish_delta(c, acc, Qact, Hh, nl);
    lds_barrier();
    prof(c, PH_ENCB_DELTA);
    for (int e = L - 1; e >= 1; --e) {
      int Kin = J->H[e - 1], Nout = J->H[e];
      zero_acc(acc);
      GAS char* const eimg = wsh + md.enc_s[e];
      const WgGeom Ge = geom_enc(J, md, e, spatch);
      Qact = dgrad_hidden(c, acc, eimg, ws_enc + (int64_t)(m * L + (e - 1)) * ACT_BYTES, Nout, Kin);
      prof(c, PH_ENCB_DGRAD);
      wgrad_adam<SCALAR_TR, RTV, RS>(c, c.P, LDP, 0, Qact, LDP, Ge, 0);
      prof(c, PH_ENCB_WGRAD);
      finish_delta(c, acc, Qact, Kin, nl);
      lds_barrier();
      prof(c, PH_ENCB_DELTA);
    }
    tr(c, 14);
    {
      const int Kx = md.Kx;
      const int nch = (Kx + XCH - 1) / XCH;
      const GAS char* xsrc = (const GAS char*)asg(md.xb) + (int64_t)(c.row0 / TROWS) * nch * XIMG_TILE_BYTES + (int64_t)c.rloc0 * (LDX * 2);
      auto geom = [&](int kc) { return geom_l0(J, md, kc, spatch); };
      if constexpr (RS) {
        constexpr int NS = ROWS_BYTES_P / XIMG_BYTES;
        if (nch <= NS) {
          for (int j = 0; j < nch; ++j) dma_lin<0>(c, xsrc + (int64_t)j * XIMG_TILE_BYTES, Qb + j * XIMG_BYTES, XIMG_BYTES >> 10);
          WgGeom Gall = geom_l0(J, md, 0, spatch);
          Gall.ncols = Kx;
          wgrad_adam<SCALAR_TR, RTV, RS>(c, c.P, LDP, 0, c.Q, LDX, Gall, 0, ROWS * LDX);
          prof(c, PH_ENCB_L0_WGRAD);
        } else {
        int cnt[NS];
#pragma unroll
        for (int j = 0; j < NS; ++j) cnt[j] = 0;
#pragma unroll
        for (int j = 0; j < NS - 1; ++j)
          if (j < nch) cnt[j] = dma_lin<0>(c, xsrc + (int64_t)j * XIMG_TILE_BYTES, Qb + j * XIMG_BYTES, XIMG_BYTES >> 10);
        for (int kc = 0; kc < nch; ++kc) {
          const int kn = kc + NS - 1;
          const int n_new = kn < nch ? dma_lin<0>(c, xsrc + (int64_t)kn * XIMG_TILE_BYTES, Qb + (kn % NS) * XIMG_BYTES, XIMG_BYTES >> 10) : 0;
          int behind = n_new;
#pragma unroll
          for (int j = 1; j < NS - 1; ++j) behind += cnt[j];
          const __bf16* Xc = reinterpret_cast<const __bf16*>(Qb + (kc % NS) * XIMG_BYTES);
          wgrad_adam<SCALAR_TR, RTV, RS>(c, c.P, LDP, 0, Xc, LDX, geom(kc), behind);
#pragma unroll
          for (int j = 0; j < NS - 2; ++j) cnt[j] = cnt[j + 1];
          cnt[NS - 2] = n_new;
        }
        prof(c, PH_ENCB_L0_WGRAD);
        }
      } else {
      dma_lin<0>(c, xsrc, Qb, XIMG_BYTES >> 10);
      for (int kc = 0; kc < nch; ++kc) {
        int n_next = 0;
        if (kc + 1 < nch) n_next = dma_lin<0>(c, xsrc + (int64_t)(kc + 1) * XIMG_TILE_BYTES, Qb + ((kc + 1) & 1) * XIMG_BYTES, XIMG_BYTES >> 10);
        const __bf16* Xc = reinterpret_cast<const __bf16*>(Qb + (kc & 1) * XIMG_BYTES);
        wgrad_adam<SCALAR_TR, RTV, RS>(c, c.P, LDP, 0, Xc, LDX, geom(kc), n_next);
      }
      prof(c, PH_ENCB_L0_WGRAD);
      }
    }
    tr(c, 15);
  }
}

constexpr int SMEM_BYTES = 2 * ROWS * LDP * 2 + STAGE_FLOATS * 4 + 2 * VEC_BYTES + (64 + 128 + 256 + 256 + 128 + 16 + 4) * 4;
static_assert(SMEM_BYTES <= 160 * 1024, "LDS budget");
static_assert(XIMG_BYTES + OBLOB_BYTES + NWAVES * PATCH_FLOATS * 4 <= ACT_BYTES, "output-chunk layout of Q");
static_assert(2 * XIMG_BYTES - ACT_BYTES <= SPATCH_OFF && SPATCH_OFF + NWAVES * PATCH_FLOATS * 4 <= STAGE_FLOATS * 4, "S layout");

__device__ __forceinline__ void carve_lds(Ctx& c, unsigned char* smem) {
  c.wave_s = __builtin_amdgcn_readfirstlane((int)(threadIdx.x >> 6));
  c.rsk = 1; c.rsq = 0; c.rloc0 = 0; c.x_pre = 0; c.gpart = nullptr; c.gp_stride = 0; c.ws0 = nullptr; c.xwg = 0; c.gwt = 0;
  c.P = reinterpret_cast<__bf16*>(smem);
  c.Q = c.P + ROWS * LDP;
  c.stage = reinterpret_cast<float*>(c.Q + ROWS * LDP);
  c.vec = c.stage + STAGE_FLOATS;
  c.red = c.vec + 2 * (VEC_BYTES / 4);
  c.colacc = c.red + 64;
  c.rowacc = c.colacc + 128;
  c.lse = c.rowacc + 256;
  c.bgrad = c.lse + 256;
  c.tlast = reinterpret_cast<unsigned long long*>(c.bgrad + 128);
  c.abort = reinterpret_cast<unsigned*>(c.tlast + 8);
}

__host__ __device__ __forceinline__ void adam_bias_consts(double lr, float beta1, float beta2, int64_t t, float& step_size,
                                                          float& inv_bc2_sqrt) {
  const double tt = (double)t;
  step_size = (float)(lr / (1.0 - pow((double)beta1, tt)));
  inv_bc2_sqrt = (float)(1.0 / sqrt(1.0 - pow((double)beta2, tt)));
}
__device__ __forceinline__ void adam_step_consts(const nm_job_t* J, int64_t t_opt, float& step_size, float& inv_bc2_sqrt) {
  const double lr_t = (J->lr_table && J->lr_cap > 0) ? J->lr_table[(t_opt - 1) % J->lr_cap] : (double)J->lr;
  adam_bias_consts(lr_t, J->beta1, J->beta2, t_opt, step_size, inv_bc2_sqrt);
}

__device__ __forceinline__ void tile_rows(Ctx& c, const nm_job_t* J, int b) {
  c.row0 = b * ROWS;
  c.nrows = min(ROWS, J->n_rows - c.row0);
  c.inv_b = 1.0f / (float)c.nrows;
}

__device__ __forceinline__ void wait_us(int us) {
  const unsigned long long t0 = __builtin_amdgcn_s_memrealtime(), ticks = 100ull * (unsigned long long)min(us, 20000);
  while (__builtin_amdgcn_s_memrealtime() - t0 < ticks) __builtin_amdgcn_s_sleep(16);
}

template <bool SCALAR_TR, int MODE = 0>
__global__ __launch_bounds__(WG) void nm_step_kernel(const nm_job_t* __restrict__ jobs, int step0, int steps_per_tile,
                                                     int flags, int n_jobs, int nparts) {
  extern __shared__ __attribute__((aligned(16))) unsigned char smem[];
  int job_idx = blockIdx.x, part = -1;
  if ((flags & 64) && blockIdx.y == 0 && blockIdx.x < 512 && threadIdx.x == 0) nm_wg_times[blockIdx.x][0] = __builtin_amdgcn_s_memrealtime();
  if (flags & NM_F_SPLIT) {
    const int xcd = blockIdx.x & 7, idx = blockIdx.x >> 3;
    job_idx = (idx / nparts) * 8 + xcd;
    part = idx % nparts;
    if (job_idx >= n_jobs) return;
    if ((flags & NM_F_FAULT_INJECT) && part == 1) return;
  }
  const int tile_idx = blockIdx.y;
  const nm_job_t* J = jobs + job_idx;
  Ctx c;
  c.job = J;
  c.part = part;
  c.nparts = nparts;
  c.slope = J->act_slope;
  carve_lds(c, smem);
  relaunder(c);
  c.flags = flags;
  c.t_last = 0;
  c.ws = (GAS char*)J->workspace + (int64_t)tile_idx * J->workspace_stride;
  for (int i = c.tid; i < SMEM_BYTES / 4; i += WG) reinterpret_cast<uint32_t*>(smem)[i] = 0u;
  __syncthreads();
  {
    constexpr int FWD_DEPHASE_DIV = 4;
    int us = steps_per_tile >= 64 ? J->dephase : (steps_per_tile >= 8 ? (J->dephase >> 2) : 0);
    if (MODE == 3) us = (tile_idx == 0 && gridDim.y > 1) ? J->dephase / FWD_DEPHASE_DIV : 0;
    if (us > 0) wait_us(us);
  }
  const int nb = (J->n_rows + ROWS - 1) / ROWS;
  const int s_begin = step0 + tile_idx * steps_per_tile;
  for (int s = s_begin; s < s_begin + steps_per_tile; ++s) {
    c.lstep = s - s_begin;
    tile_rows(c, J, s % nb);
    adam_step_consts(J, J->adam_off + (int64_t)s + 1, c.step_size, c.inv_bc2_sqrt);
    if (flags & NM_F_PROFILE) c.t_last = clock64();
    if (flags & 64) c.tlast[c.wave_s] = clock64();
    lds_barrier();
    relaunder(c);
    run_step<SCALAR_TR, MODE>(c, s);
    if ((flags & NM_F_SPLIT) && *c.abort != 0u) break;
    tr(c, 62);
    handoff_barrier();
    tr(c, 63);
  }
  if ((flags & 64) && blockIdx.y == 0 && blockIdx.x < 512 && c.tid == 0) nm_wg_times[blockIdx.x][1] = __builtin_amdgcn_s_memrealtime();
}
```

multi_modal_normative_modeling_amd/csrc/nmhip.hip:

```cpp
#include "nm_core.inc"

#include "nm_wide.inc"

__host__ __device__ inline int64_t trunk_ws_bytes(const nm_job_t* J) {
  return J->wide ? wide_ws_layout(J).total : ws_layout(J->M, J->L, J->Z).total;
}

__device__ __forceinline__ void relu_to_P(const Ctx& c, const f32x4 (&acc)[2][RT], int N) {
#pragma unroll
  for (int t = 0; t < 2; ++t) {
    const int f0 = (c.wn + 4 * t) * 16 + 4 * c.g;
    if (f0 >= N) continue;
#pragma unroll
    for (int rt = 0; rt < RT; ++rt) {
      const int r = c.wm * WROWS + rt * 16 + c.c16;
      bf16x4 pk;
#pragma unroll
      for (int i = 0; i < 4; ++i) pk[i] = (__bf16)fmaxf(acc[t][rt][i], 0.f);
      *reinterpret_cast<bf16x4*>(c.P + r * LDP + f0) = pk;
    }
  }
}

__device__ __forceinline__ bool head_setup(Ctx& c, unsigned char* smem, const nm_job_t* J, int step, int tile0, int flags) {
// ... 1086 lines not shown
  Ctx c;
  carve_lds(c, smem);
  relaunder(c);
  for (int i = c.tid; i < SMEM_BYTES / 4; i += WG) reinterpret_cast<uint32_t*>(smem)[i] = 0u;
  __syncthreads();
  if (mode == 0 || mode == 1) {
    int KA = (mode == 0) ? K : N;
    for (int e = c.tid; e < ROWS * KA; e += WG) { int r = e / KA, k = e - r * KA; c.P[r * LDP + k] = (__bf16)A[e]; }
    __syncthreads();
    f32x4 acc[2][RT];
    zero_acc(acc);
    int ncols = (mode == 0) ? N : K;
    if (mode == 0) {
      for (int ks = 0; ks < rup(K, 32) / 32; ++ks) {
        bf16x8 wf[2];
        for (int t = 0; t < 2; ++t) wf[t] = w_frag(asg(B), N, K, (c.wn + 4 * t) * 16 + c.c16, ks * 32 + 8 * c.g);
#pragma unroll
        for (int rt = 0; rt < RT; ++rt) {
          bf16x8 a = lds_frag(c.P, LDP, c.wm * WROWS + rt * 16 + c.c16, ks * 32 + 8 * c.g);
#pragma unroll
          for (int t = 0; t < 2; ++t) acc[t][rt] = mfma(wf[t], a, acc[t][rt]);
        }
      }
    } else {
      dgrad_acc(c, acc, c.P, asg(B), N, K, rup(N, 32) / 32, 0);
    }
#pragma unroll
    for (int t = 0; t < 2; ++t) {
      int f0 = (c.wn + 4 * t) * 16 + 4 * c.g;
#pragma unroll
      for (int rt = 0; rt < RT; ++rt)
#pragma unroll
        for (int i = 0; i < 4; ++i) {
          int r = c.wm * WROWS + rt * 16 + c.c16;
          if (f0 + i < ncols) Cout[(int64_t)r * ncols + f0 + i] = acc[t][rt][i];
        }
    }
  } else {
    for (int e = c.tid; e < ROWS * N; e += WG) { int r = e / N, k = e - r * N; c.P[r * LDP + k] = (__bf16)A[e]; }
    for (int e = c.tid; e < ROWS * K; e += WG) { int r = e / K, k = e - r * K; c.Q[r * LDP + k] = (__bf16)B[e]; }
    __syncthreads();
    const int ntn = (N + 15) / 16, nkt = (K + 15) / 16, kpairs = (nkt + 1) / 2;
    for (int u = c.wave; u < ntn * kpairs; u += NWAVES) {
      int nt = u / kpairs, kp = u % kpairs;
      f32x4 acc[2] = {f32x4{0, 0, 0, 0}, f32x4{0, 0, 0, 0}};
      for (int rs = 0; rs < ROWS / 32; ++rs) {
        bf16x8 bn, ak[2];
        if (mode == 3) {
          bn = lds_frag_tr_scalar(c.P, LDP, rs * 32, nt * 16, c.lane);
          for (int t = 0; t < 2; ++t) ak[t] = lds_frag_tr_scalar(c.Q, LDP, rs * 32, (kp * 2 + t) * 16, c.lane);
        } else {
          unsigned na = tr_addr_il(c.P, LDP, rs * 32, nt * 16, c.lane);
          unsigned ka = tr_addr_il(c.Q, LDP, rs * 32, kp * 32, c.lane);
          unsigned na1 = na + 1u * LDP * 2u, ka1 = ka + 1u * LDP * 2u;
          bf16x4 n0v, n1v, k0v[2], k1v[2];
          NM_TR_READ(n0v, na, 0); NM_TR_READ(n1v, na1, 0);
          NM_TR_READ(k0v[0], ka, 0);  NM_TR_READ(k1v[0], ka1, 0);
          NM_TR_READ(k0v[1], ka, 32); NM_TR_READ(k1v[1], ka1, 32);
          asm volatile("s_waitcnt lgkmcnt(0)"
                       : "+v"(n0v), "+v"(n1v), "+v"(k0v[0]), "+v"(k1v[0]), "+v"(k0v[1]), "+v"(k1v[1]));
          bn = join4(n0v, n1v);
          for (int t = 0; t < 2; ++t) ak[t] = join4(k0v[t], k1v[t]);
        }
#pragma unroll
        for (int t = 0; t < 2; ++t) acc[t] = mfma(ak[t], bn, acc[t]);
      }
#pragma unroll
      for (int t = 0; t < 2; ++t) {
        int n = nt * 16 + c.c16;
#pragma unroll
        for (int i = 0; i < 4; ++i) {
          int k = (kp * 2 + t) * 16 + 4 * c.g + i;
          if (n < N && k < K) Cout[(int64_t)n * K + k] = acc[t][i];
        }
      }
    }
  }
}

}

extern "C" {

int nm_version(void) { return 10; }

int nm_prof_read(unsigned long long* out32, int reset) {
  return read_counters(out32, nm_prof_cycles, reset);
}

int nm_trace_read(unsigned long long* out512, int reset) {
  return read_counters(out512, nm_trace_cycles, reset);
}

int nm_wgtimes_read(unsigned long long* out1024) {
  if (!out1024) return NM_E_NULL;
  return (int)hipMemcpyFromSymbol(out1024, HIP_SYMBOL(nm_wg_times), sizeof(unsigned long long) * 1024);
}

int nm_abi_sizes(int64_t* sizeof_job, int64_t* sizeof_modality) {
  if (!sizeof_job || !sizeof_modality) return NM_E_NULL;
  *sizeof_job = (int64_t)sizeof(nm_job_t);
  *sizeof_modality = (int64_t)sizeof(nm_modality_t);
  return 0;
}

const char* nm_status_string(int status) {
  switch (status) {
    case NM_OK: return "ok";
    case NM_E_NULL: return "null pointer";
    case NM_E_MODALITIES: return "modalities out of range (1..NM_MAX_MOD decoders, 1..NM_MAX_EXP experts)";
    case NM_E_LAYERS: return "hidden layers out of range (1..NM_MAX_HID)";
    case NM_E_WIDTH: return "hidden width out of range (1..NM_MAX_WIDTH)";
    case NM_E_LATENT: return "latent out of range (1..NM_MAX_LATENT)";
    case NM_E_LATENT_COV: return "latent + c_dim exceeds NM_MAX_WIDTH";
    case NM_E_PITCH: return "table pitch: Kx must be a multiple of 32 and >= D + C + 1, x_pitch a multiple of 4 and >= D, Cz a multiple of 8 and >= C + 1";
    case NM_E_GEOMETRY: return "bad launch geometry";
    case NM_E_COMBINE: return "unknown combine";
    case NM_E_OFFSETS: return "parameter tensor offsets must be multiples of 4 floats (weight matrices: of 256)";
    case NM_E_REG_HEAD: return "regression head: needs reg_w / reg_b offsets (weights: multiples of 256, biases: of 4) and the reg_resid / reg_dres image buffers (16-byte aligned)";
    case NM_E_METRICS: return "metrics: n_sets >= 1 and 1 <= max_set <= NM_METRICS_MAX_N";
    case NM_E_CLS_HEAD: return "classifier head: 0..NM_MAX_CLS blocks of width 1..NM_MAX_CLS_WIDTH, 2..NM_MAX_CLASSES classes, offsets multiples of 4, out_mu/out_z export";
    case NM_E_COUNTS: return "n_rows, loss_cap and eps_cap must be >= 1";
    case NM_E_SHADOW: return "wsh (shadow images) missing: allocate nm_fill_shadow() bytes, zero them and call nm_sync_shadow()";
    case NM_E_RESIDENCY: return "split launch: jobs x parts exceeds the number of CUs (the parts of a model wait for each other and must all be resident)";
    case NM_E_PREP: return "input preparation: 1 <= rows <= NM_PREP_MAX_ROWS, at least one source / column / bin";
    case NM_E_OUTPUT: return "out_kind must be 0 or 1, 0 <= n_private <= Z, and a private latent needs an encoder per decoder";
    case NM_E_WIDE_TC: return "general-shape path (wide): mvtCAE's total correlation needs experts x latent <= 256";
    case NM_E_ROWSPLIT: return "row-split launch: the job uses a switch that needs the whole batch in one workgroup, or lacks gpart / workspace tiles";
    case NM_E_N_PARAMS: return "n_params must be set and stay below 2^30 floats (32-bit byte offsets into params / adam_m / adam_v)";
    case NM_E_DEVPASS: return "deviation-pass kernel: one expert with the single-expert bypass, first hidden width <= 112, latent <= 32, Gaussian output only";
    default: return status > 0 ? hipGetErrorString((hipError_t)status) : "unknown argument error";
  }
}

int nm_validate_job(const nm_job_t* j) {
  if (!j) return NM_E_NULL;
  if (j->M < 1 || j->M > NM_MAX_MOD) return NM_E_MODALITIES;
  if (j->M_enc < 0 || j->M_enc > j->M || (j->M_enc == 0 ? j->M : j->M_enc) > NM_MAX_EXP) return NM_E_MODALITIES;
  if (j->L < 1 || j->L > NM_MAX_HID) return NM_E_LAYERS;
  if (j->wide) {
    for (int i = 0; i < j->L; ++i)
      if (j->H[i] < 1 || j->H[i] > NM_WIDE_MAX_WIDTH) return NM_E_WIDTH;
    if (j->Z < 1 || j->Z > NM_WIDE_MAX_LATENT) return NM_E_LATENT;
    if (j->tc_weight != 0.f && (j->M_enc > 0 ? j->M_enc : j->M) * j->Z > 256) return NM_E_WIDE_TC;
  } else {
  for (int i = 0; i < j->L; ++i)
    if (j->H[i] < 1 || j->H[i] > NM_MAX_WIDTH) return NM_E_WIDTH;
  if (j->Z < 1 || j->Z > NM_MAX_LATENT) return NM_E_LATENT;
  if (j->Z + j->C > NM_MAX_WIDTH) return NM_E_LATENT_COV;
  }
  if (j->combine < 0 || j->combine > NM_COMBINE_POE2V) return NM_E_COMBINE;
  if (j->out_kind < 0 || j->out_kind > 1 || j->n_private < 0 || j->n_private > j->Z) return NM_E_OUTPUT;
  if (j->n_private > 0 && j->M_enc != 0 && j->M_enc != j->M) return NM_E_OUTPUT;
  if (j->n_rows < 1 || j->loss_cap < 1 || j->eps_cap < 1) return NM_E_COUNTS;
  if (j->n_params < 1 || j->n_params >= ((int64_t)1 << 30)) return NM_E_N_PARAMS;
  if (!j->wsh && !j->wide) return NM_E_SHADOW;
  for (int m = 0; m < j->M; ++m) {
    const nm_modality_t& md = j->mod[m];
    if (md.D < 1 || md.Kx % 32 != 0 || md.Kx < md.D + j->C + 1) return NM_E_PITCH;
    if (md.x_pitch % 4 != 0 || md.x_pitch < md.D) return NM_E_PITCH;
    if (md.Cz % 8 != 0 || md.Cz < j->C + 1) return NM_E_PITCH;
    for (int i = 0; i < j->L; ++i) {
      if ((md.enc_b[i] | md.dec_b[i]) & 3) return NM_E_OFFSETS;
      if ((md.enc_w[i] | md.dec_w[i]) & 255) return NM_E_OFFSETS;
    }
    if ((md.mu_b | md.lv_b | md.out_b) & 3) return NM_E_OFFSETS;
    if (j->out_kind == 0 && (md.logvar_out < 0 || (md.logvar_out & 3))) return NM_E_OFFSETS;
// ... 16 lines not shown
  }
  return 0;
}

int64_t nm_fill_shadow(nm_job_t* j) {
  if (!j) return NM_E_NULL;
  if (j->M < 1 || j->M > NM_MAX_MOD || j->L < 1 || j->L > NM_MAX_HID) return NM_E_MODALITIES;
  const int Me = j->M_enc > 0 ? j->M_enc : j->M;
  const int Zs = rup(j->Z, 16), L = j->L;
  int64_t o = WSH_ZERO_BYTES;
  for (int m = 0; m < j->M; ++m) {
    nm_modality_t& md = j->mod[m];
    if (md.Kx < 32 || md.D < 1) return NM_E_PITCH;
    for (int i = 0; i < NM_MAX_HID; ++i) { md.enc_s[i] = 0; md.dec_s[i] = 0; }
    md.heads_s = 0;
    md.out_s = 0;
    if (j->wide) continue;
    if (m < Me) {
      const int nch = (md.Kx + XCH - 1) / XCH;
      md.enc_s[0] = o; o += (int64_t)l0_img_bytes(j->H[0], md.Kx) + VEC_BYTES;
      for (int e = 1; e < L; ++e) { md.enc_s[e] = o; o += cblob_bytes(j->H[e], j->H[e - 1]); }
      md.heads_s = o; o += cblob_bytes(2 * Zs, j->H[L - 1]);
    }
    for (int d = 0; d < L; ++d) {
      md.dec_s[d] = o;
      o += cblob_bytes(j->H[L - 1 - d], d == 0 ? j->Z + j->C : j->H[L - d]);
    }
    md.out_s = o; o += (int64_t)((md.D + OCH - 1) / OCH) * OBLOB_BYTES;
  }
  j->reg_s = 0;
  if (j->reg_head) { j->reg_s = o; o += (int64_t)head_chunk0(j, Me) * W0IMG_BYTES + VEC_BYTES; }
  return o;
}

int nm_sync_shadow(const nm_job_t* jobs_dev, int n_jobs, void* stream) {
  if (!jobs_dev) return NM_E_NULL;
  if (n_jobs < 1) return NM_E_GEOMETRY;
  const int slices = n_jobs >= 64 ? 4 : (n_jobs >= 8 ? 16 : 64);
  return launch_kernel(sync_shadow_kernel, dim3(n_jobs, slices), dim3(256), 0, stream, jobs_dev);
}

int64_t nm_workspace_offset(const nm_job_t* j, int what) {
  if (!j || what < 0 || what > 1) return NM_E_NULL;
  if (j->wide) {
    const WideWs ww = wide_ws_layout(j);
    return what == 0 ? ww.mu_m : ww.lv_m;
  }
  const WsLayout w = ws_layout(j->M, j->L, j->Z);
  return what == 0 ? w.mu_m : w.lv_m;
}

int64_t nm_workspace_bytes(const nm_job_t* j) {
  if (!j) return NM_E_NULL;
  int64_t b = trunk_ws_bytes(j);
  int64_t hb = 0;
  if (j->reg_head) hb = ACT_BYTES;
  if (j->cls_layers > 0 || j->cls_classes > 0) hb = hb > cls_ws_bytes(j) ? hb : cls_ws_bytes(j);
  return b + (hb + 255) / 256 * 256;
}

int nm_sync_reset(const nm_job_t* jobs_dev, int n_jobs, void* stream) {
  if (!jobs_dev) return NM_E_NULL;
  if (n_jobs < 1) return NM_E_GEOMETRY;
  return launch_kernel(sync_reset_kernel, dim3((n_jobs * (WS_SYNC_BYTES / 4) + 255) / 256), dim3(256), 0, stream, jobs_dev, n_jobs);
}

int nm_rowsplit_ok(const nm_job_t* j) {
  if (!j) return NM_E_NULL;
  if (j->wide || j->reg_head || j->cls_classes > 0 || j->cls_layers > 0) return NM_E_ROWSPLIT;
  if (j->w_off >= 0 || j->tc_weight != 0.f || j->n_private != 0 || j->out_kind != 0) return NM_E_ROWSPLIT;
  if (j->M_enc != 0 && j->M_enc != j->M) return NM_E_ROWSPLIT;
  if (j->M > NM_MAX_EXP) return NM_E_ROWSPLIT;
  for (int m = 0; m < j->M; ++m) {
    const int nck = (j->mod[m].D + OCH - 1) / OCH, nch = (j->mod[m].Kx + XCH - 1) / XCH;
    if (nck + 2 * j->L + 1 + nch > NM_RS_MAX_PASSES || 2 * nck + 2 * j->L + 3 > NM_RS_MAX_VSEGS) return NM_E_ROWSPLIT;
    int64_t vtot = 2 * (int64_t)j->mod[m].D + 2 * j->Z + 1;
    for (int i = 0; i < j->L; ++i) vtot += 2 * j->H[i];
    if (vtot > NM_RS_MAX_VEC) return NM_E_ROWSPLIT;
  }
  if (!j->gpart || j->gpart_stride < j->n_params || (j->gpart_stride & 255) || j->gpart_stride >= ((int64_t)1 << 28)) return NM_E_ROWSPLIT;
  return 0;
}

static int launch_impl(const nm_job_t* jobs_dev, int n_jobs, int step0, int steps_per_tile, int n_tiles, int flags,
                       void* stream, bool scalar_tr, int parts = 1) {
  if (int bad = check_launch_geometry(jobs_dev, n_jobs, n_tiles, steps_per_tile, step0, flags)) return bad;
  dim3 grid(n_jobs, n_tiles);
  flags &= ~NM_F_SPLIT;
  if (parts <= 1) flags &= ~NM_F_FAULT_INJECT;
  if (parts > 1) {
    if (n_tiles != 1 || parts > NM_MAX_MOD || !(flags & NM_F_BACKWARD)) return NM_E_GEOMETRY;
    const int cus = cu_count();
    if (cus < 1) return NM_E_GEOMETRY;
    const int wgs = (n_jobs + 7) / 8 * 8 * parts;
    if (wgs > cus) return NM_E_RESIDENCY;
    grid = dim3(wgs, 1);
    flags |= NM_F_SPLIT;
    nm_sync_reset(jobs_dev, n_jobs, stream);
  }
  auto kernel = nm_step_kernel<false, 3>;
  if (scalar_tr) kernel = nm_step_kernel<true>;
  else if (flags & NM_F_BACKWARD) kernel = nm_step_kernel<false>;
  return launch_kernel(kernel, grid, dim3(WG), SMEM_BYTES, stream, jobs_dev, step0, steps_per_tile, flags, n_jobs, parts);
}

int nm_launch_wide(const nm_job_t* jobs_dev, int n_jobs, int step0, int steps_per_tile, int n_tiles, int flags, void* stream) {
  if (int bad = check_launch_geometry(jobs_dev, n_jobs, n_tiles, steps_per_tile, step0, flags)) return bad;
  flags &= (NM_F_BACKWARD | NM_F_ADAM | NM_F_GRADS | NM_F_EXPORT | NM_F_ZGIVEN | NM_F_TRACE);
  return launch_kernel(nm_wide_step_kernel, dim3(n_jobs, n_tiles), dim3(WG), SMEM_BYTES, stream, jobs_dev, step0, steps_per_tile, flags);
}

int nm_launch_split(const nm_job_t* jobs_dev, int n_jobs, int parts, int step0, int n_steps, int flags, void* stream) {
  return launch_impl(jobs_dev, n_jobs, step0, n_steps, 1, flags, stream, false, parts);
}

int nm_split_errors(const nm_job_t* jobs_dev, int n_jobs, int* out_dev, int clear, void* stream) {
  if (!jobs_dev || !out_dev) return NM_E_NULL;
  if (n_jobs < 1) return NM_E_GEOMETRY;
  return launch_kernel(split_errors_kernel, dim3((n_jobs + 255) / 256), dim3(256), 0, stream, jobs_dev, n_jobs, out_dev, clear);
}

int nm_launch(const nm_job_t* jobs_dev, int n_jobs, int step0, int steps_per_tile, int n_tiles, int flags,
              void* stream) {
  return launch_impl(jobs_dev, n_jobs, step0, steps_per_tile, n_tiles, flags, stream, false);
}

int nm_launch_scalar_tr(const nm_job_t* jobs_dev, int n_jobs, int step0, int steps_per_tile, int n_tiles, int flags,
                        void* stream) {
  return launch_impl(jobs_dev, n_jobs, step0, steps_per_tile, n_tiles, flags, stream, true);
}

int nm_head_regression(const nm_job_t* jobs_dev, int n_jobs, int step, int tile0, int n_tiles, int flags, void* stream) {
  if (int bad = check_launch_geometry(jobs_dev, n_jobs, n_tiles, 1, step < tile0 ? step : tile0, flags)) return bad;
  return launch_kernel(nm_reghead_kernel, dim3(n_jobs, n_tiles), dim3(WG), SMEM_BYTES, stream, jobs_dev, step, tile0, flags);
}

int nm_head_classifier(const nm_job_t* jobs_dev, int n_jobs, int step, int tile0, int n_tiles, int flags, void* stream) {
  if (int bad = check_launch_geometry(jobs_dev, n_jobs, n_tiles, 1, step < tile0 ? step : tile0, flags)) return bad;
  return launch_kernel(nm_clshead_kernel, dim3(n_jobs, n_tiles), dim3(WG), SMEM_BYTES, stream, jobs_dev, step, tile0, flags);
}

int nm_train_steps_head(const nm_job_t* jobs_dev, int n_jobs, int step0, int n_steps, int flags, void* stream) {
  if (int bad = check_launch_geometry(jobs_dev, n_jobs, 1, n_steps, step0, flags)) return bad;
  if ((flags & NM_F_GRADS) && n_steps != 1) return NM_E_GEOMETRY;
  return launch_kernel(nm_head_step_kernel<false>, dim3(n_jobs), dim3(WG), SMEM_BYTES, stream, jobs_dev, step0, n_steps,
                       flags & (NM_F_PROFILE | NM_F_TRACE | NM_F_GRADS | NM_F_BNSTATS), n_jobs, 1);
}

int nm_train_steps_head_split(const nm_job_t* jobs_dev, int n_jobs, int parts, int step0, int n_steps, int flags, void* stream) {
  if (int bad = check_launch_geometry(jobs_dev, n_jobs, 1, n_steps, step0, flags)) return bad;
  if (parts < 2 || parts > NM_MAX_MOD) return NM_E_GEOMETRY;
  if ((flags & NM_F_GRADS) && n_steps != 1) return NM_E_GEOMETRY;
  const int cus = cu_count();
  if (cus < 1) return NM_E_GEOMETRY;
  const int wgs = (n_jobs + 7) / 8 * 8 * parts;
  if (wgs > cus) return NM_E_RESIDENCY;
  if (int bad = nm_sync_reset(jobs_dev, n_jobs, stream)) return bad;
  return launch_kernel(nm_head_step_kernel<true>, dim3(wgs), dim3(WG), SMEM_BYTES, stream, jobs_dev, step0, n_steps,
                       flags & (NM_F_PROFILE | NM_F_TRACE | NM_F_GRADS | NM_F_BNSTATS), n_jobs, parts);
}

int nm_train_steps(const nm_job_t* jobs_dev, int n_jobs, int step0, int n_steps, void* stream) {
  return nm_launch(jobs_dev, n_jobs, step0, n_steps, 1, NM_F_BACKWARD | NM_F_ADAM, stream);
}

int nm_grads(const nm_job_t* jobs_dev, int n_jobs, int step, void* stream) {
  return nm_launch(jobs_dev, n_jobs, step, 1, 1, NM_F_BACKWARD | NM_F_GRADS | NM_F_EXPORT, stream);
}

int nm_forward(const nm_job_t* jobs_dev, int n_jobs, int tile0, int n_tiles, void* stream) {
  return nm_launch(jobs_dev, n_jobs, tile0, 1, n_tiles, NM_F_EXPORT, stream);
}

int nm_train_steps_persistent(const nm_job_t* jobs_dev, int n_jobs, int step0, int n_steps, void* stream) {
  return nm_train_steps(jobs_dev, n_jobs, step0, n_steps, stream);
}

int nm_deviation(const nm_job_t* jobs_dev, int n_jobs, int tile0, int n_tiles, void* stream) {
  return nm_forward(jobs_dev, n_jobs, tile0, n_tiles, stream);
}

int nm_adam_step(float* params, const float* grads, float* m, float* v, int64_t n, float lr, float beta1, float beta2,
                 float eps, int64_t t, void* stream) {
  if (!params || !grads || !m || !v) return NM_E_NULL;
// ... 39 lines not shown
```

multi_modal_normative_modeling_amd/engine.py:

```python
from __future__ import annotations

import ctypes as C
import functools
import math
import os
import zlib
from typing import Dict, List, Optional, Sequence

import numpy as np
import torch

from . import _lib
from .layout import ModelSpec, ParamLayout, rowsplit_limit

BATCH = _lib.NM_BATCH

DEVPASS_MULTI_AUTO = {2: True, 3: True, 4: True}

LATENT_AUTO = {1: True, 2: False, 3: True, 4: True}


_RAW_STREAM = getattr(torch._C, "_cuda_getCurrentRawStream", None)


# ... 132 lines not shown
        self.loss_log = torch.zeros(self.loss_cap, _lib.NM_LOSS_STRIDE, dtype=torch.float32, device=dev)
        self.eps: Optional[torch.Tensor] = None
        self.eps_cap = 1
        self.lr_table: Optional[torch.Tensor] = None
        self._ws = None
        self._ws_tiles = 0
        self._version = 0
        self._wsh = None
        self._gpart = None
        self._gpart_k = 0
        self._rs_ok_version = None
        self._rs_limit = (None, None)
        self.shadow_dirty = True
        self._ensure_workspace(n_tiles_ws)
        self.out_mu = self.out_logvar = self.out_z = None
        nk = len(self.kmods)
        self.out_loc: List[Optional[torch.Tensor]] = [None] * nk
        self.out_sqerr: List[Optional[torch.Tensor]] = [None] * nk
        self.out_rowdev: List[Optional[torch.Tensor]] = [None] * nk

    def _ensure_workspace(self, n_tiles: int):
        if self._ws is not None and self._ws_tiles >= n_tiles:
            return
        lib = _lib.load()
        probe = _lib.NmJob()
        probe.M, probe.L, probe.Z = len(self.kmods), len(self.spec.hidden), self.spec.latent
        probe.C, probe.wide = self.spec.net_c_dim, int(self.spec.wide)
        for i, h in enumerate(self.spec.hidden):
            probe.H[i] = h
        probe.cls_layers, probe.cls_classes = len(self.spec.classifier_layers), (self.spec.num_classes if self.spec.classifier_layers else 0)
        for i, w in enumerate(self.spec.classifier_layers):
            probe.cls_width[i] = w
        probe.reg_head = 1 if self.spec.kind == "regression" else 0
        probe.M_enc = self.spec.M
        for k, (m, _, _) in enumerate(self.kmods):
            probe.mod[k].D = self.tables[m].D
            probe.mod[k].Kx = self.tables[m].Kx
        self.ws_bytes = int(lib.nm_workspace_bytes(C.byref(probe)))
        if self._wsh is None:
            if self.spec.wide and self.spec.kind != "regression":
                self._wsh = torch.zeros(256, dtype=torch.uint8, device=self.device)
            else:
                nb = int(lib.nm_fill_shadow(C.byref(probe)))
                if nb < 0:
                    _lib.check(nb, "nm_fill_shadow")
                self._wsh = torch.zeros(nb, dtype=torch.uint8, device=self.device)
        self._ws = torch.zeros(self.ws_bytes * n_tiles, dtype=torch.uint8, device=self.device)
        self._ws_tiles = n_tiles
        self._version += 1

    @property
    def gpart_stride(self) -> int:
        return (int(self.params.numel()) + 255) // 256 * 256

    def _ensure_rowsplit(self, k: int):
        self._ensure_workspace(k)
        if self._gpart is None or self._gpart_k < k:
            self._gpart = torch.zeros(k * self.gpart_stride, dtype=torch.float32, device=self.device)
            self._gpart_k = k
            self._version += 1

    def devpass_ok(self) -> bool:
        s = self.spec
        return (not s.wide and len(self.kmods) == 1 and s.M == 1 and self.single_bypass and s.n_private == 0 and not s.is_dm
                and self.tc_weight == 0.0 and s.kind != "weighted_dmvae" and s.hidden[0] <= 112 and (s.latent + 15) // 16 * 16 <= 32
                and self.out_mu is None and self.out_logvar is None and self.out_z is None)

    def devpass_multi_ok(self) -> bool:
        s = self.spec
        return (not s.wide and len(self.kmods) == s.M and 2 <= s.M <= _lib.NM_MAX_EXP and s.n_private == 0 and not s.is_dm
                and self.tc_weight == 0.0 and s.kind != "weighted_dmvae" and s.hidden[0] <= 112 and (s.latent + 15) // 16 * 16 <= 32
                and self.out_mu is None and self.out_logvar is None and self.out_z is None)

    def latent_ok(self) -> bool:
        s = self.spec
        return (not s.wide and len(self.kmods) == s.M and 1 <= s.M <= _lib.NM_MAX_EXP and s.n_private == 0 and not s.is_dm
                and self.tc_weight == 0.0 and s.kind != "weighted_dmvae" and s.hidden[0] <= 112 and (s.latent + 15) // 16 * 16 <= 32)

    def rowsplit_ok(self) -> bool:
        s = self.spec
        return (not s.wide and s.kind in ("single", "multimodal") and len(self.kmods) == s.M and s.M <= _lib.NM_MAX_EXP
                and self.tc_weight == 0.0 and self.rowsplit_limit() is None)

    def rowsplit_limit(self) -> Optional[str]:
        kxs = tuple(self.tables[m].Kx for m, _, _ in self.kmods)
        if self._rs_limit[0] != kxs:
            self._rs_limit = (kxs, rowsplit_limit(self.spec, kxs))
        return self._rs_limit[1]

    def set_fi(self, fi):
        ra = self.tables[0].rows_alloc
        f = torch.as_tensor(fi, dtype=torch.float32).reshape(-1)
        if f.numel() != self.tables[0].N:
            raise ValueError(f"fi has {f.numel()} values for {self.tables[0].N} table rows")
        self.fi_target = torch.zeros(ra, device=self.device)
        self.fi_target[: f.numel()] = f.to(self.device)
        self._version += 1

    def set_labels(self, labels):
        ra = self.tables[0].rows_alloc
        l = torch.as_tensor(labels).reshape(-1).to(torch.int32)
        if l.numel() != self.tables[0].N:
            raise ValueError(f"labels has {l.numel()} values for {self.tables[0].N} table rows")
        self.labels = torch.zeros(ra, dtype=torch.int32, device=self.device)
        self.labels[: l.numel()] = l.to(self.device)
        self._version += 1

    def prepare_classifier(self):
        if self.out_z is None or any(o is None for o in self.out_rowdev) or self.out_logits is None:
            self.enable_exports(loc=False, sqerr=False, rowdev=True, latent=True)
        ra = self.tables[0].rows_alloc
        if self.dz_extra is None:
            self.dz_extra = torch.zeros(ra, self.spec.latent, device=self.device)
            self._version += 1
        if any(d is None for d in self.dloc_rowcoef):
            self.dloc_rowcoef = [torch.zeros(ra, device=self.device) for _ in self.kmods]
            self._version += 1

    def prepare_regression(self):
        nq = sum((self.tables[m].D + 63) // 64 for m in range(self.spec.M))
        img = 256 * 72 * 2
        if self.reg_resid is None or self.reg_resid.numel() < self.tables[0].n_tiles * nq * img:
            self.reg_resid = torch.zeros(self.tables[0].n_tiles * nq * img, dtype=torch.uint8, device=self.device)
            self.reg_dres = torch.zeros(nq * img, dtype=torch.uint8, device=self.device)
            self._version += 1
        if self.out_fi_pred is None:
            self.out_fi_pred = torch.zeros(self.tables[0].rows_alloc, device=self.device)
            self._version += 1

    def touch(self):
        self._version += 1

    def set_lr_table(self, lrs):
        self.lr_table = None if lrs is None else torch.as_tensor(np.asarray(lrs, dtype=np.float64)).to(self.device).contiguous()
        self._version += 1

    def set_eps(self, eps: Optional[torch.Tensor]):
        self._version += 1
        if eps is None:
            self.eps, self.eps_cap = None, 1
            return
        e = torch.as_tensor(eps, dtype=torch.float32)
        if e.dim() == 2:
            e = e.unsqueeze(0)
        if e.shape[1] != BATCH or e.shape[2] != self.spec.latent:
            pad = torch.zeros(e.shape[0], BATCH, self.spec.latent, dtype=torch.float32)
            pad[:, :e.shape[1]] = e
            e = pad
        self.eps = e.to(self.device).contiguous()
        self.eps_cap = int(self.eps.shape[0])

    def enable_exports(self, loc=True, sqerr=True, rowdev=True, latent=True):
        ra = self.tables[0].rows_alloc
        Z = self.spec.latent
        self._version += 1
        if latent:
            self.out_mu = torch.zeros(ra, Z, device=self.device)
            self.out_logvar = torch.zeros(ra, Z, device=self.device)
            self.out_z = torch.zeros(ra, Z, device=self.device)
        if self.spec.kind == "regression":
            self.out_fi_pred = torch.zeros(ra, device=self.device)
        if self.spec.kind == "endtoend" and self.spec.classifier_layers:
            self.out_logits = torch.zeros(ra, _lib.NM_MAX_CLASSES, device=self.device)
        for j, (m, _, _) in enumerate(self.kmods):
            t = self.tables[m]
            self.out_loc[j] = torch.zeros(ra, t.x_pitch, device=self.device)[:, :t.D] if loc else None
# ... 54 lines not shown
        j.out_logvar = self.out_logvar.data_ptr() if self.out_logvar is not None else None
        j.out_z = self.out_z.data_ptr() if self.out_z is not None else None
        j.dz_extra = self.dz_extra.data_ptr() if self.dz_extra is not None else None
        self.layout.fill_head(j)
        if j.reg_head:
            self.prepare_regression()
            j.reg_resid, j.reg_dres = self.reg_resid.data_ptr(), self.reg_dres.data_ptr()
        j.reg_lambda = self.reg_lambda
        j.fi_target = self.fi_target.data_ptr() if self.fi_target is not None else None
        j.out_fi_pred = self.out_fi_pred.data_ptr() if self.out_fi_pred is not None else None
        if j.cls_classes and (self.out_z is None or self.out_mu is None):
            j.cls_layers, j.cls_classes = 0, 0
        j.cls_train, j.cls_use_mu = int(self.cls_train), int(self.cls_use_mu)
        j.cls_dropout, j.cls_margin = self.cls_dropout, self.cls_margin
        j.cls_w_ce, j.cls_w_contrast = self.cls_w_ce, self.cls_w_contrast
        j.labels = self.labels.data_ptr() if self.labels is not None else None
        j.out_logits = self.out_logits.data_ptr() if self.out_logits is not None else None
        j.dz_out = self.dz_extra.data_ptr() if self.dz_extra is not None else None
        for k, (m, _, _) in enumerate(self.kmods):
            t = self.tables[m]
            md = j.mod[k]
            md.D, md.Kx, md.x_pitch, md.Cz = t.D, t.Kx, t.x_pitch, t.Cz
            md.x_f32, md.xb, md.cz = t.x_f32.data_ptr(), t.xb.data_ptr(), t.cz.data_ptr()
            self.layout.fill_modality(md, k)
            md.out_loc = self.out_loc[k].data_ptr() if self.out_loc[k] is not None else None
            md.out_sqerr = self.out_sqerr[k].data_ptr() if self.out_sqerr[k] is not None else None
            md.out_rowdev = self.out_rowdev[k].data_ptr() if self.out_rowdev[k] is not None else None
            md.dloc_extra = self.dloc_extra[k].data_ptr() if self.dloc_extra[k] is not None else None
            md.dloc_rowcoef = self.dloc_rowcoef[k].data_ptr() if self.dloc_rowcoef[k] is not None else None
            j.rowcoef_out[k] = md.dloc_rowcoef
        if not s.wide or s.kind == "regression":
            nb = int(_lib.load().nm_fill_shadow(C.byref(j)))
            if nb != self._wsh.numel():
                raise _lib.NmError(f"shadow size changed: {nb} vs {self._wsh.numel()} bytes")
        _lib.check(_lib.load().nm_validate_job(C.byref(j)), "nm_validate_job")
        return j

    def state_dict(self) -> Dict[str, torch.Tensor]:
        return {k: v.detach().cpu().clone() for k, v in self.layout.unflatten(self.params).items()}

    def load_state_dict(self, state: Dict[str, torch.Tensor]):
        self.params.copy_(self.layout.flatten(state, device=self.device))
        self.shadow_dirty = True

    def params_changed(self):
        self.shadow_dirty = True

    def grads_dict(self) -> Dict[str, torch.Tensor]:
        return {k: v.detach().cpu().clone() for k, v in self.layout.unflatten(self.grads).items()}

    def adam_dicts(self):
        m = {k: v.detach().cpu().clone() for k, v in self.layout.unflatten(self.adam_m).items()}
        v = {k: v.detach().cpu().clone() for k, v in self.layout.unflatten(self.adam_v).items()}
        return m, v

    @property
    def batches_per_epoch(self) -> int:
        return math.ceil(self.tables[0].N / BATCH)


_HANDOFF_KINDS = {"nm_launch_split": "split", "nm_launch_rowsplit": "rowsplit", "nm_launch_rowsplit_mixed": "rowsplit",
                  "nm_train_steps_head_split": "split"}


class JobSet:

    def __init__(self, jobs: Sequence[Job]):
        if not jobs:
            raise ValueError("empty job set")
        self.jobs = list(jobs)
        self.wide = bool(jobs[0].spec.wide)
        if any(bool(j.spec.wide) != self.wide for j in jobs):
            raise ValueError("a job set holds either fused-kernel shapes or general-shape (wide) models, not both")
        self.device = jobs[0].device
        self.lib = _lib.load()
        self._dev = None
        self._sig = None
        self._dephase_vals = None
        self._split_pending = False
        self._pending_kinds = set()
        self._err_kinds = set()
        self._err_inflight = None
        self._err_dev = self._err_host = None

    @functools.cached_property
    def _cus(self) -> int:
        return torch.cuda.get_device_properties(self.device).multi_processor_count

    def check_split_errors(self, block: bool = True):
        if self._err_inflight is not None:
            ev, host = self._err_inflight
            if block:
                ev.synchronize()
            if ev.query():
                self._err_inflight = None
                kinds = self._err_kinds
                vals = host.tolist()
                shape = [i for i, v in enumerate(vals) if v == _lib.NM_SYNC_ERR_SHAPE]
                bad = [i for i, v in enumerate(vals) if v != 0 and v != _lib.NM_SYNC_ERR_SHAPE]
                if shape:
                    raise _lib.NmError(f"row-split launch: job(s) {shape[:8]} exceed the Adam sweep's tables (passes, vector "
                                       f"segments or vector elements; nm_rowsplit_ok) -- or the launch's group map lists them "
                                       f"with a modality count that is not theirs -- and were refused by the kernel; their "
                                       f"parameters were not updated -- run them with rowsplit=1 or NMHIP_ROWSPLIT=0")
                if bad:
                    switch = " / ".join(v for kd, v in (("rowsplit", "NMHIP_ROWSPLIT=0"), ("split", "NMHIP_SPLIT=0"))
                                        if kd in kinds) or "NMHIP_SPLIT=0"
                    what = "row-split" if kinds == {"rowsplit"} else "split"
                    raise _lib.NmError(f"{what} launch: the hand-off between the workgroups of job(s) {bad[:8]} timed out "
                                       f"(the parts of a model must all be resident at once: another stream or process "
                                       f"occupying CUs breaks that); their parameters are not valid -- re-run with {switch}")
        if self._split_pending and self._dev is not None and self._err_inflight is None:
            n = len(self.jobs)
            if self._err_dev is None:
                self._err_dev = torch.zeros(n, dtype=torch.int32, device=self.device)
                self._err_host = torch.zeros(n, dtype=torch.int32).pin_memory()
            _lib.check(self.lib.nm_split_errors(self._dev.data_ptr(), n, self._err_dev.data_ptr(), 1,
                                                _stream_ptr(self.device)), "nm_split_errors")
            self._err_host.copy_(self._err_dev, non_blocking=True)
            ev = torch.cuda.Event()
            ev.record(torch.cuda.current_stream(self.device))
            self._err_inflight = (ev, self._err_host)
            self._err_kinds, self._pending_kinds = self._pending_kinds, set()
            self._split_pending = False
            if block:
                self.check_split_errors(True)

    def _set_dephase(self):
        vals = self._dephase_vals
        if vals is not None and all(j.dephase_sleeps == v for j, v in zip(self.jobs, vals)):
            return
        n = len(self.jobs)
        per_xcd = max(1, (n + 7) // 8)
        for b, j in enumerate(self.jobs):
            step_us = j.layout.n_params * 2.05e-3
            frac = 0.0 if n < 16 else ((b >> 3) + (b & 7) / 8) / per_xcd
            s = int(round(step_us * frac))
            if s != j.dephase_sleeps:
                j.dephase_sleeps = s
                j._version += 1
        self._dephase_vals = [j.dephase_sleeps for j in self.jobs]

    def _upload(self, n_tiles: int = 1):
        self.check_split_errors(block=False)
        self._set_dephase()
        for j in self.jobs:
            j._ensure_workspace(n_tiles)
        sig = tuple((j._version, j.t - j.step) for j in self.jobs)
        if self._dev is None or sig != self._sig:
            arr = (_lib.NmJob * len(self.jobs))(*[j.struct() for j in self.jobs])
            host = torch.frombuffer(bytearray(bytes(arr)), dtype=torch.uint8)
            self._dev = host.to(self.device)
            self._sig = sig
        if self.wide:
            for j in self.jobs:
                j.shadow_dirty = j.shadow_dirty and j.spec.kind == "regression"
        if any(j.shadow_dirty for j in self.jobs):
            _lib.check(self.lib.nm_sync_shadow(self._dev.data_ptr(), len(self.jobs), _stream_ptr(self.device)), "nm_sync_shadow")
            for j in self.jobs:
                j.shadow_dirty = False
        return self._dev.data_ptr()

    def _issue(self, entry: str, n_tiles: int, *args):
        ptr = self._upload(n_tiles)
        args = [a if isinstance(a, C.Array) else int(a) for a in args]
        _lib.check(getattr(self.lib, entry)(ptr, len(self.jobs), *args, _stream_ptr(self.device)), entry)
        kind = _HANDOFF_KINDS.get(entry)
        if kind is not None:
            self._split_pending = True
            self._pending_kinds.add(kind)

    def _launch(self, step0, steps_per_tile, n_tiles, flags, scalar_tr=False):
        entry = "nm_launch_wide" if self.wide else ("nm_launch_scalar_tr" if scalar_tr else "nm_launch")
        self._issue(entry, n_tiles, step0, steps_per_tile, n_tiles, flags)

    def _launch_split(self, step0, n_steps, flags):
        self._issue("nm_launch_split", 1, len(self.jobs[0].kmods), step0, n_steps, flags)

    def split_parts(self) -> int:
        M = len(self.jobs[0].kmods)
        mode = os.environ.get("NMHIP_SPLIT", "auto")
        if mode == "0" or M < 2 or self.wide or any(len(j.kmods) != M for j in self.jobs):
            return 1
        fits = (len(self.jobs) + 7) // 8 * 8 * M <= self._cus
        return M if fits else 1

    def rowsplit_k(self, mixed: bool = False) -> int:
        mode = os.environ.get("NMHIP_ROWSPLIT", "auto")
        M = len(self.jobs[0].kmods)
        if mode == "0" or self.wide:
            return 1
        groups = ((self._rs_groups() if mixed else len(self.jobs) * M) + 7) // 8 * 8
        kmax = int(mode) if mode in ("2", "4") else 4
        ks = [k for k in (4, 2) if k <= kmax and groups * k <= self._cus and groups <= _lib.NM_RS_MAX_GROUPS]
        if not ks or any((len(j.kmods) != M and not mixed) or not j.rowsplit_ok() for j in self.jobs):
            return 1
        return ks[0]

    def _rs_groups(self) -> int:
        return sum(len(j.kmods) for j in self.jobs)

    def rowsplit_helpers(self, k: int) -> int:
        env = os.environ.get("NMHIP_RS_HELPERS", "auto")
        groups = (self._rs_groups() + 7) // 8 * 8
        room = max(0, min(self._cus // groups, 32) - k)
        return min(int(env), room) if env != "auto" else min(room, 12)

    def _launch_rowsplit(self, k: int, step0: int, n_steps: int, flags: int, helpers: Optional[int] = None):
        for i, j in enumerate(self.jobs):
            j._ensure_rowsplit(k)
            if j._rs_ok_version != j._version:
                if self.lib.nm_rowsplit_ok(C.byref(j.struct())) != 0:
                    why = j.rowsplit_limit() or "not a plain cVAE / cVAE_multimodal model on the fused kernel"
                    raise ValueError(f"job {i} of the set cannot run row-split (nm_rowsplit_ok): {why}")
                j._rs_ok_version = j._version
        h = self.rowsplit_helpers(k) if helpers is None else int(helpers)
        Ms = [len(j.kmods) for j in self.jobs]
        spread = int(max(j.layout.n_params for j in self.jobs) * 0.37e-3 * (4 / k)) if sum(Ms) * k >= 96 else 0
        if all(m == Ms[0] for m in Ms):
            self._issue("nm_launch_rowsplit", k, Ms[0], k, h, step0, n_steps, flags, spread)
        else:
            self._issue("nm_launch_rowsplit_mixed", k, (C.c_int * len(Ms))(*Ms), k, h, step0, n_steps, flags, spread)

    def _training_form(self, split: Optional[bool], rowsplit: Optional[int]):
        k = (self.rowsplit_k() if split is None else 1) if rowsplit is None else int(rowsplit)
        if k > 1:
            return "rowsplit", k
        parts = self.split_parts() if split is None else (len(self.jobs[0].kmods) if split else 1)
        return ("split", parts) if parts > 1 else ("whole", 1)

    def _launch_form(self, form, step0: int, n_steps: int, flags: int, helpers: Optional[int], scalar_tr: bool):
        kind, k = form
        if kind == "rowsplit":
            self._launch_rowsplit(k, step0, n_steps, flags, helpers)
        elif kind == "split":
            self._launch_split(step0, n_steps, flags)
        else:
            self._launch(step0, n_steps, 1, flags, scalar_tr)

    def _check_jobs(self, head: Optional[str] = None, caller: str = "", at_step: bool = True) -> int:
        step0 = self.jobs[0].step
        for j in self.jobs:
            if head == "regression" and (j.spec.kind != "regression" or j.fi_target is None):
                raise ValueError(f"{caller} needs regression jobs with fi_target set")
            if head == "endtoend" and (j.spec.kind != "endtoend" or not j.spec.classifier_layers or j.labels is None):
                raise ValueError(f"{caller} needs end-to-end jobs with a classifier and labels set")
            if at_step and j.step != step0:
                raise ValueError("jobs of one set must be at the same step")
        if head is not None and any(j.batches_per_epoch != self.jobs[0].batches_per_epoch for j in self.jobs):
            raise ValueError("jobs of one set must have the same number of batches")
        return step0

    def _advance(self, n_steps: int):
        for j in self.jobs:
            j.step += n_steps
            j.t += n_steps

    def train(self, n_steps: int, scalar_tr: bool = False, profile: bool = False, split: Optional[bool] = None,
              rowsplit: Optional[int] = None, helpers: Optional[int] = None):
        step0 = self._check_jobs()
        flags = _lib.NM_F_BACKWARD | _lib.NM_F_ADAM | (_lib.NM_F_PROFILE if profile else 0)
        form = ("whole", 1) if scalar_tr else self._training_form(split, rowsplit)
        self._launch_form(form, step0, n_steps, flags, helpers, scalar_tr)
        self._advance(n_steps)

    def grads(self, step: Optional[int] = None, export: bool = True, scalar_tr: bool = False, split: bool = False,
              rowsplit: int = 1, helpers: Optional[int] = None):
        s = self.jobs[0].step if step is None else step
        flags = _lib.NM_F_BACKWARD | _lib.NM_F_GRADS | (_lib.NM_F_EXPORT if export else 0)
        self._launch_form(self._training_form(split, rowsplit), s, 1, flags, helpers, scalar_tr)

    def devpass_ok(self) -> bool:
        if self.wide or os.environ.get("NMHIP_DEVPASS", "1") == "0":
            return False
        return all(j.devpass_ok() for j in self.jobs)

    def devpass_multi_ok(self) -> bool:
        if self.wide or os.environ.get("NMHIP_DEVPASS", "1") == "0":
            return False
        return all(j.devpass_multi_ok() for j in self.jobs)

    def devpass_multi_pick(self) -> bool:
        env = os.environ.get("NMHIP_DEVPASS_MULTI", "auto")
        if env == "0" or not self.devpass_multi_ok():
            return False
        return env == "1" or all(DEVPASS_MULTI_AUTO.get(len(j.kmods), False) for j in self.jobs)

    def forward(self, tile0: int = 0, n_tiles: Optional[int] = None, loss: bool = True, trace: bool = False,
                compact: Optional[bool] = None):
        nt = self.jobs[0].tables[0].n_tiles if n_tiles is None else n_tiles
        if not loss and self.devpass_ok():
            self._issue("nm_devpass", 1, tile0 * 2, nt * 2, _lib.NM_F_TRACE if trace else 0)
            return
        if compact and (loss or not self.devpass_multi_ok()):
            raise ValueError("compact=True: the set cannot run on nm_devpass_multi (loss wanted, latent exports on, "
                             "NMHIP_DEVPASS=0, or a shape nm_devpass_multi_ok refuses)")
        if not loss and (compact or (compact is None and self.devpass_multi_pick())):
            self._issue("nm_devpass_multi", nt, tile0 * 2, nt * 2, _lib.NM_F_TRACE if trace else 0)
            return
        self._launch(tile0, 1, nt, _lib.NM_F_EXPORT)

    def latent_ok(self) -> bool:
        if self.wide or os.environ.get("NMHIP_LATENT", "1") == "0":
            return False
        return all(j.latent_ok() for j in self.jobs)

    def latent_pick(self) -> bool:
        return self.latent_ok() and all(LATENT_AUTO.get(len(j.kmods), False) for j in self.jobs)

    def latent(self, tile0: int = 0, n_tiles: Optional[int] = None, compact: Optional[bool] = None, trace: bool = False):
        for j in self.jobs:
            if j.out_mu is None or j.out_logvar is None:
                j.set_latent_exports(True)
        nt = self.jobs[0].tables[0].n_tiles if n_tiles is None else n_tiles
        if compact and not self.latent_ok():
            raise ValueError("compact=True: the set cannot run on nm_latent_pass: " + self._latent_refusal())
        if compact or (compact is None and self.latent_pick()):
            ws_tiles = nt if any(len(j.kmods) > 1 for j in self.jobs) else 1
            self._issue("nm_latent_pass", ws_tiles, tile0 * 2, nt * 2, _lib.NM_F_TRACE if trace else 0)
            return
        self._launch(tile0, 1, nt, _lib.NM_F_EXPORT)

    def _latent_refusal(self) -> str:
        if os.environ.get("NMHIP_LATENT", "1") == "0":
            return "NMHIP_LATENT=0"
        if self.wide:
            return "general-shape path (a hidden width or latent beyond the fused kernel's tile)"
        for i, j in enumerate(self.jobs):
            if not j.latent_ok():
                s = j.spec
                return (f"job {i}: nm_latent_pass_ok refuses its shape (kind {s.kind!r}, {s.M} modalities of which "
                        f"{len(j.kmods)} in the kernel, hidden {list(s.hidden)}, latent {s.latent}, private {s.n_private}, "
                        f"tc_weight {j.tc_weight})")
        return "nothing"

    def latent_stats(self):
        return latent_stats([j.out_mu[:j.tables[0].N] for j in self._latent_jobs()])

    def latent_scores(self, mean: torch.Tensor, var: torch.Tensor):
        jobs = self._latent_jobs()
        return latent_scores([j.out_mu[:j.tables[0].N] for j in jobs], [j.out_logvar[:j.tables[0].N] for j in jobs], mean, var)

    def _latent_jobs(self):
        if any(j.out_mu is None or j.out_logvar is None for j in self.jobs):
            raise ValueError("latent exports are off: run JobSet.latent() (or forward() with enable_exports(latent=True)) first")
        if any(j.spec.latent != self.jobs[0].spec.latent for j in self.jobs):
# ... 163 lines not shown
```

Baseline: 371,700 steps/s.

## Add specialized plain-training kernel instantiation that compiles out unused feature branches

Result: faster. 389,600 steps/s, median of 6 (+4.8%).

```diff
diff --git a/include/nmhip.h b/include/nmhip.h
--- a/include/nmhip.h
+++ b/include/nmhip.h
@@ -59,7 +59,8 @@
   NM_F_TRACE    = 64,
   NM_F_BNSTATS  = 256,
   NM_F_SPLIT    = 512,
-  NM_F_FAULT_INJECT = 1024
+  NM_F_FAULT_INJECT = 1024,
+  NM_F_PLAIN    = 2048
 };
 
 typedef struct nm_modality {
@@ -195,6 +196,7 @@
 #define NM_RS_MAX_VSEGS  144
 #define NM_RS_MAX_VEC    3072
 int nm_rowsplit_ok(const nm_job_t* job_host);
+int nm_plain_ok(const nm_job_t* job_host);
 int nm_sync_reset(const nm_job_t* jobs_dev, int n_jobs, void* stream);
 int nm_devpass(const nm_job_t* jobs_dev, int n_jobs, int tile0, int n_tiles, int flags, void* stream);
 int nm_trace_read_dv(unsigned long long* out512, int reset);
@@ -206,6 +208,7 @@
 int nm_trace_read_rs(unsigned long long* out512, int reset);
 #define NM_SYNC_ERR_TIMEOUT 1
 #define NM_SYNC_ERR_SHAPE   2
+#define NM_SYNC_ERR_PLAIN   3
 int nm_split_errors(const nm_job_t* jobs_dev, int n_jobs, int* out_dev, int clear, void* stream);
 
 int nm_train_steps(const nm_job_t* jobs_dev, int n_jobs, int step0, int n_steps, void* stream);
diff --git a/multi_modal_normative_modeling_amd/_lib.py b/multi_modal_normative_modeling_amd/_lib.py
--- a/multi_modal_normative_modeling_amd/_lib.py
+++ b/multi_modal_normative_modeling_amd/_lib.py
@@ -37,8 +37,10 @@
 NM_F_BNSTATS = 256
 NM_F_SPLIT = 512
 NM_F_FAULT_INJECT = 1024
+NM_F_PLAIN = 2048
 NM_SYNC_ERR_TIMEOUT = 1
 NM_SYNC_ERR_SHAPE = 2
+NM_SYNC_ERR_PLAIN = 3
 NM_METRICS_MAX_N = 8192
 NM_METRICS_STRIDE = 8
 NM_ROI_Y_CHUNK = 128
@@ -176,6 +178,7 @@
     lib.nm_launch_rowsplit_mixed.argtypes = [vp, i32, C.POINTER(i32), i32, i32, i32, i32, i32, i32, vp]
     lib.nm_rowsplit_groups.argtypes = [C.POINTER(i32), i32, C.POINTER(i32), i32]
     lib.nm_rowsplit_ok.argtypes = [C.POINTER(NmJob)]
+    lib.nm_plain_ok.argtypes = [C.POINTER(NmJob)]
     lib.nm_sync_reset.argtypes = [vp, i32, vp]
     lib.nm_trace_read_rs.argtypes = [C.POINTER(C.c_ulonglong), i32]
     lib.nm_devpass.argtypes = [vp, i32, i32, i32, i32, vp]
@@ -242,6 +245,7 @@
     "nm_roi_effect", "nm_roi_significance_workspace", "nm_roi_significance",
     "nm_auc_bootstrap_workspace", "nm_auc_bootstrap",
     "nm_column_regress", "nm_student_t_two_sided",
+    "nm_plain_ok",
 ]
 
 
diff --git a/multi_modal_normative_modeling_amd/csrc/nm_core.inc b/multi_modal_normative_modeling_amd/csrc/nm_core.inc
--- a/multi_modal_normative_modeling_amd/csrc/nm_core.inc
+++ b/multi_modal_normative_modeling_amd/csrc/nm_core.inc
@@ -100,6 +100,7 @@
 constexpr int WS_SYNC_BYTES = 256;
 constexpr int WS_SYNC_ERR_WORD = 32;
 constexpr unsigned WS_SYNC_ERR_TIMEOUT = NM_SYNC_ERR_TIMEOUT, WS_SYNC_ERR_SHAPE = NM_SYNC_ERR_SHAPE;
+constexpr unsigned WS_SYNC_ERR_PLAIN = NM_SYNC_ERR_PLAIN;
 constexpr int WS_SYNC_C_WORD = 33, WS_SYNC_D_WORD = 40, WS_SYNC_LOSS_WORD = 48, WS_SYNC_XCC_WORD = 57;
 __host__ __device__ inline WsLayout ws_layout(int M, int L, int Z) {
   WsLayout w;
@@ -940,7 +941,7 @@
   asm volatile("s_nop 4\n\tglobal_load_dword %0, %1, %2" : "+v"(dst) : "v"(voff), "s"(sbase) : "memory")
 constexpr int WG_LOADS = 6;
 
-template <bool SCALAR_TR, int RTV = RT, bool PART = false>
+template <bool SCALAR_TR, int RTV = RT, bool PART = false, bool PLAIN = false>
 __device__ __forceinline__ int wgrad_adam(const Ctx& cc, const __bf16* A, int lda, int a_col0, const __bf16* B, int ldb,
                                           const WgGeom& G, int pending = -1, int b_chunk = 0, float* bgrad_buf = nullptr) {
   NM_GEOM(RTV);
@@ -955,8 +956,9 @@
   const int nunits = wg_units(G);
   const int kb = K - k_base;
   const int kb_pair = wg_bias_pair(G), kb_j = (kb >> 4) & 1, kb_col = kb & 15;
-  const bool do_adam = !PART && (c.flags & NM_F_ADAM) != 0;
-  const bool do_grads = !PART && (c.flags & NM_F_GRADS) != 0;
+  static_assert(!PLAIN || !PART, "the plain instantiation owns the whole batch");
+  const bool do_adam = PLAIN || (!PART && (c.flags & NM_F_ADAM) != 0);
+  const bool do_grads = !PLAIN && !PART && (c.flags & NM_F_GRADS) != 0;
   const AdamK ak = adam_consts(c);
   gf32 Pp = asg(J->params), Mp = asg(J->adam_m), Vp = asg(J->adam_v);
   float* patch = T.patch + c.wave * PATCH_FLOATS;
@@ -1077,7 +1079,7 @@
           __builtin_nontemporal_store(m4, (GAS f32x4*)(Mp + idx));
           __builtin_nontemporal_store(v4, (GAS f32x4*)(Vp + idx));
           nst += 3;
-          if (T.sh) {
+          if (PLAIN || T.sh) {
             bf16x4 pk;
 #pragma unroll
             for (int i = 0; i < 4; ++i) pk[i] = (__bf16)p4[i];
@@ -1176,6 +1178,18 @@
                 WgT{md.enc_w[0], md.enc_b[0], img + (int64_t)kc * XCH * 2, Kx * 2, (GAS float*)(img + l0_img_bytes(N0, Kx)), patch}};
 }
 
+__host__ __device__ inline bool plain_job(const nm_job_t* j) {
+  if (j->wide || j->reg_head || j->reg_resid || j->reg_dres || j->cls_layers > 0 || j->cls_classes > 0 || j->dz_extra) return false;
+  if (j->out_kind != 0 || j->n_private != 0 || j->tc_weight != 0.f || j->w_off >= 0) return false;
+  if (j->M < 1 || j->M > NM_MAX_MOD || (j->M_enc != 0 && j->M_enc != j->M)) return false;
+  if (!j->wsh || j->out_mu || j->out_logvar || j->out_z) return false;
+  for (int m = 0; m < j->M; ++m) {
+    const nm_modality_t& md = j->mod[m];
+    if (md.out_loc || md.out_sqerr || md.out_rowdev || md.dloc_extra || md.dloc_rowcoef) return false;
+  }
+  return true;
+}
+
 __device__ __forceinline__ int experts(const nm_job_t* J) { return J->M_enc > 0 ? J->M_enc : J->M; }
 __host__ __device__ inline int head_chunk0(const nm_job_t* J, int m) {
   int q = 0;
@@ -1290,6 +1304,13 @@
   }
   return G;
 }
+template <bool VEC4>
+__device__ __forceinline__ void plain_latent_deltas(float dz, float es, float mj, float lj, float klw, float& dmu_j, float& dlv_j) {
+#pragma clang fp contract(off)
+  const float e1 = fx_exp(lj) - 1.0f, hdz = 0.5f * dz, hk = klw * 0.5f;
+  dmu_j = fmaf(klw, mj, dz);
+  dlv_j = VEC4 ? fmaf(hdz, es, hk * e1) : fmaf(hk, e1, hdz * es);
+}
 __device__ __forceinline__ float pick(const float (&a)[NM_MAX_EXP], int m) {
   float r = a[0];
 #pragma unroll
@@ -1301,24 +1322,84 @@
   return r;
 }
 
-template <bool SCALAR_TR, int MODE = 0, int RTV = RT>
+template <int RTV>
+__device__ __forceinline__ void out_epilogue_plain(const Ctx& c, f32x4 (&acc)[RTV], const f32x4 (&xin)[RTV], const float* vb, __bf16* Dq,
+                                                   int d0, int D, float llw_b, float (&colsum)[4], float& nll_part) {
+#pragma clang fp contract(off)
+  NM_GEOM(RTV);
+  const int dl0 = c.wn * 16 + 4 * c.g, dg0 = d0 + dl0;
+  const f32x4 bo = *reinterpret_cast<const f32x4*>(vb + dl0);
+  const f32x4 sv = *reinterpret_cast<const f32x4*>(vb + OCH + dl0);
+  float inv[4], colq[4], coef[4];
+#pragma unroll
+  for (int i = 0; i < 4; ++i) {
+    inv[i] = expf(-sv[i]);
+    colq[i] = 0.f;
+    coef[i] = ((dg0 + i < D) ? llw_b * inv[i] : 0.f) + 0.0f;
+  }
+  int nvalid = 0;
+  if (c.nrows == ROWS && d0 + OCH <= D) {
+    nvalid = RT;
+#pragma unroll
+    for (int rt = 0; rt < RT; ++rt) {
+      const int r = c.wm * WROWS + rt * 16 + c.c16;
+      acc[rt] += bo;
+      bf16x4 pk;
+#pragma unroll
+      for (int i = 0; i < 4; ++i) {
+        const float diff = acc[rt][i] - xin[rt][i];
+        colq[i] = fmaf(diff, diff, colq[i]);
+        pk[i] = (__bf16)fmaf(diff, coef[i], 0.0f);
+      }
+      *reinterpret_cast<bf16x4*>(Dq + r * LDX + dl0) = pk;
+    }
+  } else {
+#pragma unroll
+    for (int rt = 0; rt < RT; ++rt) {
+      const int r = c.wm * WROWS + rt * 16 + c.c16;
+      const bool rv = r < c.nrows;
+      nvalid += rv ? 1 : 0;
+      acc[rt] += bo;
+      bf16x4 pk;
+#pragma unroll
+      for (int i = 0; i < 4; ++i) {
+        const float diff = rv ? acc[rt][i] - xin[rt][i] : 0.f;
+        colq[i] = fmaf(diff, diff, colq[i]);
+        pk[i] = (__bf16)fmaf(diff, coef[i], 0.0f);
+      }
+      *reinterpret_cast<bf16x4*>(Dq + r * LDX + dl0) = pk;
+    }
+  }
+  const float nv = (float)nvalid;
+#pragma unroll
+  for (int i = 0; i < 4; ++i) {
+    const bool dv = dg0 + i < D;
+    const float hq = (0.5f * inv[i]) * colq[i];
+    const float t = nv * fmaf(0.5f, sv[i], LOG_SQRT_2PI);
+    nll_part += dv ? hq + t : 0.f;
+    colsum[i] = dv ? fmaf(nv, 0.5f, -hq) : 0.f;
+  }
+}
+
+template <bool SCALAR_TR, int MODE = 0, int RTV = RT, bool PLAIN = false>
 __device__ __forceinline__ void run_step(Ctx& c, int step) {
   NM_GEOM(RTV);
   constexpr bool RS = RTV < 8;
   static_assert(!RS || MODE == 0, "row-split instantiations run the one-pass train step only");
+  static_assert(!PLAIN || (MODE == 0 && !RS && !SCALAR_TR), "the plain instantiation is the whole-batch one-pass train step");
   const nm_job_t* J = c.job;
   const int M = J->M, L = J->L, Z = J->Z, C = J->C;
   const int Me = experts(J);
   const bool nl = J->non_linear != 0;
-  const bool bwd = MODE != 1 && MODE != 3 && (c.flags & NM_F_BACKWARD) != 0;
+  const bool bwd = PLAIN || (MODE != 1 && MODE != 3 && (c.flags & NM_F_BACKWARD) != 0);
   constexpr bool FWD_ONLY = MODE == 1 || MODE == 3;
   const bool save = bwd || MODE == 1;
-  const bool exportf = MODE != 2 && (c.flags & NM_F_EXPORT) != 0;
+  const bool exportf = !PLAIN && MODE != 2 && (c.flags & NM_F_EXPORT) != 0;
   const WsLayout wl = ws_layout(M, L, Z);
   const int Zs = wl.Zs;
-  const bool split = c.part >= 0;
+  const bool split = !PLAIN && c.part >= 0;
   const int part = split ? c.part : 0;
-  const int S = J->n_private, Zc = Z - S;
+  const int S = PLAIN ? 0 : J->n_private, Zc = Z - S;
   const float rZc = Zc > 0 ? 1.0f / (float)Zc : 0.f;
   const bool vec4 = S == 0 && (Z & 3) == 0;
   const bool fastlat = MODE == 3 && M == 1 && Me == 1 && J->single_bypass != 0 && !split && S == 0 && J->tc_weight == 0.f &&
@@ -1326,7 +1407,7 @@
                        !((c.flags & NM_F_EXPORT) && (J->out_mu || J->out_logvar || J->out_z));
   __bf16* const zlds = reinterpret_cast<__bf16*>(c.stage);
   float kl_fast = 0.f;
-  const bool sigm = J->out_kind == 1;
+  const bool sigm = !PLAIN && J->out_kind == 1;
   gf32 ws_mu_m = (gf32)(c.ws + wl.mu_m + (int64_t)(step & 1) * M * wl.lat);
   gf32 ws_lv_m = (gf32)(c.ws + wl.lv_m + (int64_t)(step & 1) * M * wl.lat);
   gf32 ws_mu_j = (gf32)(c.ws + wl.mu_j + part * wl.lat);
@@ -1385,7 +1466,8 @@
     }
   };
   float tc = 0.f;
-  if (MODE != 2 && J->tc_weight != 0.f) {
+  if constexpr (PLAIN) asm volatile("" : "+v"(tc));
+  if (!PLAIN && MODE != 2 && J->tc_weight != 0.f) {
     relaunder(c);
     for (int col = c.wave; col < Me * Z; col += NWAVES) {
       const int m = col / Z, z = col - m * Z;
@@ -1414,7 +1496,7 @@
     }
   }
   float kl_w = J->kl_weight;
-  if (J->w_off >= 0) {
+  if (!PLAIN && J->w_off >= 0) {
     kl_w = 0.f;
     for (int m = 0; m < M; ++m) kl_w += asg(J->params)[J->w_off + m];
   }
@@ -1455,6 +1537,7 @@
 #pragma unroll
         for (int m = 0; m < NM_MAX_EXP; ++m) { Lt.mu[m] = mu4[m][i]; Lt.lv[m] = lv4[m][i]; }
         Fuse f = fuse_fwd(J, Lt, al);
+        if constexpr (PLAIN) asm volatile("" : "+v"(f.mu), "+v"(f.lv));
         float es = ep[i] * fx_exp(0.5f * f.lv);
         if (c.flags & NM_F_ZGIVEN) { f.mu = ep[i]; es = 0.f; }
         omu[i] = f.mu; olv[i] = f.lv; oes[i] = es;
@@ -1479,6 +1562,7 @@
     Lat Lt;
     load_lat(Lt, r, S + z);
     Fuse f = fuse_fwd(J, Lt, al);
+    if constexpr (PLAIN) asm volatile("" : "+v"(f.mu), "+v"(f.lv));
     float ep = J->eps ? asg(J->eps)[((int64_t)(step % J->eps_cap) * TROWS + c.rloc0 + r) * Z + z]
                       : randn_ctr(J->seed, (uint32_t)step, (uint32_t)(c.row0 + r), (uint32_t)z);
     float es = ep * fx_exp(0.5f * f.lv);
@@ -1569,10 +1653,10 @@
 #pragma unroll
     for (int rt = 0; rt < NRC; ++rt)
       rcv[rt] = (MODE == 2 && md.dloc_rowcoef) ? asg(md.dloc_rowcoef)[c.row0 + c.wm * WROWS + rt * 16 + c.c16] : 0.f;
-    const float ll_w = (J->w_off >= 0) ? asg(J->params)[J->w_off + m] : J->ll_weight;
+    const float ll_w = (!PLAIN && J->w_off >= 0) ? asg(J->params)[J->w_off + m] : J->ll_weight;
     const float llw_b = ll_w * c.inv_b;
-    const int hq_all = (J->reg_head && m < Me) ? head_chunk0(J, Me) : 0;
-    const int64_t hq_m = (J->reg_head && m < Me) ? head_chunk0(J, m) : 0;
+    const int hq_all = (!PLAIN && J->reg_head && m < Me) ? head_chunk0(J, Me) : 0;
+    const int64_t hq_m = (!PLAIN && J->reg_head && m < Me) ? head_chunk0(J, m) : 0;
     GAS char* const res_out = (exportf && hq_all > 0 && J->reg_resid)
         ? (GAS char*)asg(J->reg_resid) + ((int64_t)(c.row0 / TROWS) * hq_all + hq_m) * XIMG_TILE_BYTES : (GAS char*)nullptr;
     const GAS char* const dres_in = (MODE == 2 && hq_all > 0 && J->reg_dres)
@@ -1594,7 +1678,7 @@
       const float* vb = reinterpret_cast<const float*>(slot + OIMG_BYTES);
       const WgGeom Go = geom_out(J, md, ch, opatch);
       if (c.tid < OCH) c.colacc[c.tid] = 0.f;
-      const bool lvo_adam = !RS && bwd && (c.flags & NM_F_ADAM) && !sigm && c.wave == 0;
+      const bool lvo_adam = !RS && bwd && (PLAIN || (c.flags & NM_F_ADAM)) && !sigm && c.wave == 0;
       float lvp, lvm, lvv;
       asm volatile("" : "=v"(lvp), "=v"(lvm), "=v"(lvv));
       if (lvo_adam) {
@@ -1639,6 +1723,10 @@
         if (ch + 1 < nck) load_xin(ch + 1, xnx);
       }
       {
+        float colsum[4];
+        if constexpr (PLAIN) {
+          out_epilogue_plain<RTV>(c, acc, xin, vb, Dq, d0, D, llw_b, colsum, nll_part);
+        } else {
         const f32x4 bo = *reinterpret_cast<const f32x4*>(vb + dl0);
         const f32x4 sv = *reinterpret_cast<const f32x4*>(vb + OCH + dl0);
         float inv[4], colq[4], coef[4];
@@ -1689,7 +1777,6 @@
             *(GAS bf16x4*)(res_out + (int64_t)ch * XIMG_TILE_BYTES + (r * LDX + dl0) * 2) = rk;
           }
         }
-        float colsum[4];
 #pragma unroll
         for (int i = 0; i < 4; ++i) {
           const bool dv = dg0 + i < D;
@@ -1727,6 +1814,7 @@
         if (FWD_ONLY)
           young_prev = RT + (res_out ? RT : 0) +
                        ((exportf && wave_cols) ? RT * ((md.out_loc ? 1 : 0) + (md.out_sqerr ? 1 : 0)) : 0);
+        }
         if (bwd) {
 #pragma unroll
           for (int i = 0; i < 4; ++i) {
@@ -1763,7 +1851,7 @@
       dgrad_tile(c, accg, Dq, dpitch, deferred ? d0 : 0, Wc, LDP, OCH / 32);
       tr(c, 8);
       prof(c, PH_OUT_DGRAD);
-      const int n_wg = deferred ? 0 : wgrad_adam<SCALAR_TR, RTV, RS>(c, Dq, LDX, 0, c.P, LDP, Go);
+      const int n_wg = deferred ? 0 : wgrad_adam<SCALAR_TR, RTV, RS, PLAIN>(c, Dq, LDX, 0, c.P, LDP, Go);
       young_prev = RT + n_wg;
       tr(c, 9);
       prof(c, PH_OUT_WGRAD);
@@ -1801,7 +1889,8 @@
     }
     float nll = block_sum(c, nll_part);
     float ll_this = -nll * c.inv_b;
-    if (J->w_off >= 0) {
+    if constexpr (PLAIN) asm volatile("" : "+v"(ll_this));
+    if (!PLAIN && J->w_off >= 0) {
       if (c.tid == 0 && bwd) apply_grad(c, J->w_off + m, kl - ll_this, nullptr);
       ll_this *= ll_w;
     }
@@ -1841,7 +1930,7 @@
       const __bf16* const Qact = dgrad_hidden(c, acc, dimg, act_img, Nout, Kin);
       tr(c, 10);
       prof(c, PH_DEC_DGRAD);
-      wgrad_adam<SCALAR_TR, RTV, RS>(c, c.P, LDP, 0, Qact, LDP, Gd, 0);
+      wgrad_adam<SCALAR_TR, RTV, RS, PLAIN>(c, c.P, LDP, 0, Qact, LDP, Gd, 0);
       tr(c, 11);
       prof(c, PH_DEC_WGRAD);
       if (d > 0) {
@@ -1876,7 +1965,7 @@
       ll_sum = 0.f;
       for (int m = 0; m < M; ++m) ll_sum += row[NM_LOSS_LL_M + m];
     }
-    const float llw_tot = (J->w_off >= 0) ? 1.0f : J->ll_weight;
+    const float llw_tot = (!PLAIN && J->w_off >= 0) ? 1.0f : J->ll_weight;
     row[NM_LOSS_KL] = kl_w * kl;
     row[NM_LOSS_LL] = ll_sum;
     row[NM_LOSS_TC] = tc;
@@ -1909,7 +1998,7 @@
 
   const bool fused = !(Me == 1 && J->single_bypass);
   const float klw = kl_w * c.inv_b;
-  const float tcw = J->tc_weight / (float)Me;
+  const float tcw = PLAIN ? 0.f : J->tc_weight / (float)Me;
   gbf16 ws_fz = (gbf16)ws_zc0;
   const bool once = fused && Me >= 2 && Me * 2 * Zs <= PW && !split && S == 0;
   const bool once_ws = fused && Me >= 2 && !once && 2 * Zs <= PW && !split && S == 0;
@@ -1952,7 +2041,7 @@
         const f32x4 mj4 = *(const GAS f32x4*)(ws_mu_j + r * Zs + z0), lj4 = *(const GAS f32x4*)(ws_lv_j + r * Zs + z0);
         const f32x4 es4 = *(const GAS f32x4*)(ws_es + r * Zs + z0);
         f32x4 dz4 = load_dz4(r, z0);
-        if (J->dz_extra) {
+        if (!PLAIN && J->dz_extra) {
 #pragma unroll
           for (int i = 0; i < 4; ++i) dz4[i] += asg(J->dz_extra)[(int64_t)(c.row0 + r) * Z + min(z0 + i, Z - 1)];
         }
@@ -1963,8 +2052,9 @@
           Lat Lt;
 #pragma unroll
           for (int m = 0; m < NM_MAX_EXP; ++m) { Lt.mu[m] = mu4[m][i]; Lt.lv[m] = lv4[m][i]; }
-          const float dmu_j = dz4[i] + klw * mj4[i];
-          const float dlv_j = 0.5f * dz4[i] * es4[i] + klw * 0.5f * (fx_exp(lj4[i]) - 1.0f);
+          float dmu_j = dz4[i] + klw * mj4[i];
+          float dlv_j = 0.5f * dz4[i] * es4[i] + klw * 0.5f * (fx_exp(lj4[i]) - 1.0f);
+          if constexpr (PLAIN) plain_latent_deltas<true>(dz4[i], es4[i], mj4[i], lj4[i], klw, dmu_j, dlv_j);
           FuseGrad G = fuse_bwd(J, Lt, al, dmu_j, dlv_j);
           const bool ok = rv && z0 + i < Z;
 #pragma unroll
@@ -1996,9 +2086,10 @@
         Lat Lt;
         load_lat(Lt, r, S + z);
         float mj = ws_mu_j[r * Zs + z], lj = ws_lv_j[r * Zs + z], es = ws_es[r * Zs + z], dz = load_dz(r, z);
-        if (J->dz_extra) dz += asg(J->dz_extra)[(int64_t)(c.row0 + r) * Z + z];
+        if (!PLAIN && J->dz_extra) dz += asg(J->dz_extra)[(int64_t)(c.row0 + r) * Z + z];
         float dmu_j = dz + klw * mj;
         float dlv_j = 0.5f * dz * es + klw * 0.5f * (fx_exp(lj) - 1.0f);
+        if constexpr (PLAIN) plain_latent_deltas<false>(dz, es, mj, lj, klw, dmu_j, dlv_j);
         FuseGrad G = fuse_bwd(J, Lt, al, dmu_j, dlv_j);
         const bool rv = r < c.nrows;
   #pragma unroll
@@ -2090,7 +2181,7 @@
           const f32x4 mj4 = *(const GAS f32x4*)(ws_mu_j + r * Zs + z0), lj4 = *(const GAS f32x4*)(ws_lv_j + r * Zs + z0);
           const f32x4 es4 = *(const GAS f32x4*)(ws_es + r * Zs + z0);
           f32x4 dz4 = load_dz4(r, z0);
-          if (J->dz_extra) {
+          if (!PLAIN && J->dz_extra) {
 #pragma unroll
             for (int i = 0; i < 4; ++i) dz4[i] += asg(J->dz_extra)[(int64_t)(c.row0 + r) * Z + min(z0 + i, Z - 1)];
           }
@@ -2101,8 +2192,9 @@
             Lat Lt;
 #pragma unroll
             for (int q = 0; q < NM_MAX_EXP; ++q) { Lt.mu[q] = mu4[q][i]; Lt.lv[q] = lv4[q][i]; }
-            const float dmu_j = dz4[i] + klw * mj4[i];
-            const float dlv_j = 0.5f * dz4[i] * es4[i] + klw * 0.5f * (fx_exp(lj4[i]) - 1.0f);
+            float dmu_j = dz4[i] + klw * mj4[i];
+            float dlv_j = 0.5f * dz4[i] * es4[i] + klw * 0.5f * (fx_exp(lj4[i]) - 1.0f);
+            if constexpr (PLAIN) plain_latent_deltas<true>(dz4[i], es4[i], mj4[i], lj4[i], klw, dmu_j, dlv_j);
             FuseGrad G = fuse_bwd(J, Lt, al, dmu_j, dlv_j);
             const bool ok = rv && z0 + i < Z;
             float dmu_m = pick(G.dmu, m);
@@ -2122,9 +2214,10 @@
           Lat Lt;
           load_lat(Lt, r, S + z);
           float mj = ws_mu_j[r * Zs + z], lj = ws_lv_j[r * Zs + z], es = ws_es[r * Zs + z], dz = load_dz(r, z);
-          if (J->dz_extra) dz += asg(J->dz_extra)[(int64_t)(c.row0 + r) * Z + z];
+          if (!PLAIN && J->dz_extra) dz += asg(J->dz_extra)[(int64_t)(c.row0 + r) * Z + z];
           float dmu_j = dz + klw * mj;
           float dlv_j = 0.5f * dz * es + klw * 0.5f * (fx_exp(lj) - 1.0f);
+          if constexpr (PLAIN) plain_latent_deltas<false>(dz, es, mj, lj, klw, dmu_j, dlv_j);
           FuseGrad G = fuse_bwd(J, Lt, al, dmu_j, dlv_j);
           const bool rv = r < c.nrows;
           float dmu_m = pick(G.dmu, m);
@@ -2160,9 +2253,9 @@
     tr(c, 13);
     {
       const WgGeom Gm = geom_head(J, md, 0, spatch);
-      wgrad_adam<SCALAR_TR, RTV, RS>(c, c.P, LDP, 0, Qact, LDP, Gm, 0);
+      wgrad_adam<SCALAR_TR, RTV, RS, PLAIN>(c, c.P, LDP, 0, Qact, LDP, Gm, 0);
       const WgGeom Gl = geom_head(J, md, 1, spatch);
-      wgrad_adam<SCALAR_TR, RTV, RS>(c, c.P, LDP, Zs, Qact, LDP, Gl, 0);
+      wgrad_adam<SCALAR_TR, RTV, RS, PLAIN>(c, c.P, LDP, Zs, Qact, LDP, Gl, 0);
     }
     prof(c, PH_ENCB_HEADS_WGRAD);
     finish_delta(c, acc, Qact, Hh, nl);
@@ -2175,7 +2268,7 @@
       const WgGeom Ge = geom_enc(J, md, e, spatch);
       Qact = dgrad_hidden(c, acc, eimg, ws_enc + (int64_t)(m * L + (e - 1)) * ACT_BYTES, Nout, Kin);
       prof(c, PH_ENCB_DGRAD);
-      wgrad_adam<SCALAR_TR, RTV, RS>(c, c.P, LDP, 0, Qact, LDP, Ge, 0);
+      wgrad_adam<SCALAR_TR, RTV, RS, PLAIN>(c, c.P, LDP, 0, Qact, LDP, Ge, 0);
       prof(c, PH_ENCB_WGRAD);
       finish_delta(c, acc, Qact, Kin, nl);
       lds_barrier();
@@ -2193,7 +2286,7 @@
           for (int j = 0; j < nch; ++j) dma_lin<0>(c, xsrc + (int64_t)j * XIMG_TILE_BYTES, Qb + j * XIMG_BYTES, XIMG_BYTES >> 10);
           WgGeom Gall = geom_l0(J, md, 0, spatch);
           Gall.ncols = Kx;
-          wgrad_adam<SCALAR_TR, RTV, RS>(c, c.P, LDP, 0, c.Q, LDX, Gall, 0, ROWS * LDX);
+          wgrad_adam<SCALAR_TR, RTV, RS, PLAIN>(c, c.P, LDP, 0, c.Q, LDX, Gall, 0, ROWS * LDX);
           prof(c, PH_ENCB_L0_WGRAD);
         } else {
         int cnt[NS];
@@ -2209,7 +2302,7 @@
 #pragma unroll
           for (int j = 1; j < NS - 1; ++j) behind += cnt[j];
           const __bf16* Xc = reinterpret_cast<const __bf16*>(Qb + (kc % NS) * XIMG_BYTES);
-          wgrad_adam<SCALAR_TR, RTV, RS>(c, c.P, LDP, 0, Xc, LDX, geom(kc), behind);
+          wgrad_adam<SCALAR_TR, RTV, RS, PLAIN>(c, c.P, LDP, 0, Xc, LDX, geom(kc), behind);
 #pragma unroll
           for (int j = 0; j < NS - 2; ++j) cnt[j] = cnt[j + 1];
           cnt[NS - 2] = n_new;
@@ -2222,7 +2315,7 @@
         int n_next = 0;
         if (kc + 1 < nch) n_next = dma_lin<0>(c, xsrc + (int64_t)(kc + 1) * XIMG_TILE_BYTES, Qb + ((kc + 1) & 1) * XIMG_BYTES, XIMG_BYTES >> 10);
         const __bf16* Xc = reinterpret_cast<const __bf16*>(Qb + (kc & 1) * XIMG_BYTES);
-        wgrad_adam<SCALAR_TR, RTV, RS>(c, c.P, LDP, 0, Xc, LDX, geom(kc), n_next);
+        wgrad_adam<SCALAR_TR, RTV, RS, PLAIN>(c, c.P, LDP, 0, Xc, LDX, geom(kc), n_next);
       }
       prof(c, PH_ENCB_L0_WGRAD);
       }
@@ -2274,13 +2367,13 @@
   while (__builtin_amdgcn_s_memrealtime() - t0 < ticks) __builtin_amdgcn_s_sleep(16);
 }
 
-template <bool SCALAR_TR, int MODE = 0>
+template <bool SCALAR_TR, int MODE = 0, bool PLAIN = false>
 __global__ __launch_bounds__(WG) void nm_step_kernel(const nm_job_t* __restrict__ jobs, int step0, int steps_per_tile,
                                                      int flags, int n_jobs, int nparts) {
   extern __shared__ __attribute__((aligned(16))) unsigned char smem[];
   int job_idx = blockIdx.x, part = -1;
   if ((flags & 64) && blockIdx.y == 0 && blockIdx.x < 512 && threadIdx.x == 0) nm_wg_times[blockIdx.x][0] = __builtin_amdgcn_s_memrealtime();
-  if (flags & NM_F_SPLIT) {
+  if (!PLAIN && (flags & NM_F_SPLIT)) {
     const int xcd = blockIdx.x & 7, idx = blockIdx.x >> 3;
     job_idx = (idx / nparts) * 8 + xcd;
     part = idx % nparts;
@@ -2289,6 +2382,12 @@
   }
   const int tile_idx = blockIdx.y;
   const nm_job_t* J = jobs + job_idx;
+  if constexpr (PLAIN) {
+    if (!plain_job(J)) {
+      ((unsigned*)((char*)J->workspace + ws_layout(J->M, J->L, J->Z).sync))[WS_SYNC_ERR_WORD] = WS_SYNC_ERR_PLAIN;
+      return;
+    }
+  }
   Ctx c;
   c.job = J;
   c.part = part;
@@ -2317,8 +2416,8 @@
     if (flags & 64) c.tlast[c.wave_s] = clock64();
     lds_barrier();
     relaunder(c);
-    run_step<SCALAR_TR, MODE>(c, s);
-    if ((flags & NM_F_SPLIT) && *c.abort != 0u) break;
+    run_step<SCALAR_TR, MODE, RT, PLAIN>(c, s);
+    if (!PLAIN && (flags & NM_F_SPLIT) && *c.abort != 0u) break;
     tr(c, 62);
     handoff_barrier();
     tr(c, 63);
diff --git a/multi_modal_normative_modeling_amd/csrc/nmhip.hip b/multi_modal_normative_modeling_amd/csrc/nmhip.hip
--- a/multi_modal_normative_modeling_amd/csrc/nmhip.hip
+++ b/multi_modal_normative_modeling_amd/csrc/nmhip.hip
@@ -1192,7 +1192,7 @@
 
 extern "C" {
 
-int nm_version(void) { return 10; }
+int nm_version(void) { return 11; }
 
 int nm_prof_read(unsigned long long* out32, int reset) {
   return read_counters(out32, nm_prof_cycles, reset);
@@ -1375,6 +1375,11 @@
   return 0;
 }
 
+int nm_plain_ok(const nm_job_t* j) {
+  if (!j) return NM_E_NULL;
+  return plain_job(j) ? 0 : 1;
+}
+
 static int launch_impl(const nm_job_t* jobs_dev, int n_jobs, int step0, int steps_per_tile, int n_tiles, int flags,
                        void* stream, bool scalar_tr, int parts = 1) {
   if (int bad = check_launch_geometry(jobs_dev, n_jobs, n_tiles, steps_per_tile, step0, flags)) return bad;
@@ -1391,8 +1396,12 @@
     flags |= NM_F_SPLIT;
     nm_sync_reset(jobs_dev, n_jobs, stream);
   }
+  const int mode_flags = NM_F_BACKWARD | NM_F_ADAM | NM_F_GRADS | NM_F_EXPORT | NM_F_ZGIVEN;
+  const bool plain = (flags & NM_F_PLAIN) && parts <= 1 && !scalar_tr && (flags & mode_flags) == (NM_F_BACKWARD | NM_F_ADAM);
+  flags &= ~NM_F_PLAIN;
   auto kernel = nm_step_kernel<false, 3>;
   if (scalar_tr) kernel = nm_step_kernel<true>;
+  else if (plain) kernel = nm_step_kernel<false, 0, true>;
   else if (flags & NM_F_BACKWARD) kernel = nm_step_kernel<false>;
   return launch_kernel(kernel, grid, dim3(WG), SMEM_BYTES, stream, jobs_dev, step0, steps_per_tile, flags, n_jobs, parts);
 }
diff --git a/multi_modal_normative_modeling_amd/engine.py b/multi_modal_normative_modeling_amd/engine.py
--- a/multi_modal_normative_modeling_amd/engine.py
+++ b/multi_modal_normative_modeling_amd/engine.py
@@ -238,6 +238,14 @@
         return (not s.wide and s.kind in ("single", "multimodal") and len(self.kmods) == s.M and s.M <= _lib.NM_MAX_EXP
                 and self.tc_weight == 0.0 and self.rowsplit_limit() is None)
 
+    def plain_ok(self) -> bool:
+        s = self.spec
+        return (not s.wide and s.kind in ("single", "multimodal") and len(self.kmods) == s.M and self.tc_weight == 0.0
+                and self.dz_extra is None and all(t is None for t in self.dloc_extra) and all(t is None for t in self.dloc_rowcoef)
+                and self.out_mu is None and self.out_logvar is None and self.out_z is None
+                and all(t is None for t in self.out_loc) and all(t is None for t in self.out_sqerr)
+                and all(t is None for t in self.out_rowdev))
+
     def rowsplit_limit(self) -> Optional[str]:
         kxs = tuple(self.tables[m].Kx for m, _, _ in self.kmods)
         if self._rs_limit[0] != kxs:
@@ -458,6 +466,8 @@
         self._err_kinds = set()
         self._err_inflight = None
         self._err_dev = self._err_host = None
+        self._plain_sig = self._plain_all = None
+        self.last_launch = None
 
     @functools.cached_property
     def _cus(self) -> int:
@@ -473,7 +483,13 @@
                 kinds = self._err_kinds
                 vals = host.tolist()
                 shape = [i for i, v in enumerate(vals) if v == _lib.NM_SYNC_ERR_SHAPE]
-                bad = [i for i, v in enumerate(vals) if v != 0 and v != _lib.NM_SYNC_ERR_SHAPE]
+                plain = [i for i, v in enumerate(vals) if v == _lib.NM_SYNC_ERR_PLAIN]
+                bad = [i for i, v in enumerate(vals) if v not in (0, _lib.NM_SYNC_ERR_SHAPE, _lib.NM_SYNC_ERR_PLAIN)]
+                if plain:
+                    raise _lib.NmError(f"plain-training launch (NM_F_PLAIN): job(s) {plain[:8]} need the generic step kernel "
+                                       f"(nm_plain_ok: a head, extra gradients, exports, a model kind beyond the plain trunk) and "
+                                       f"were refused by the kernel; their parameters were not updated -- run them with "
+                                       f"plain=False or NMHIP_PLAIN=0")
                 if shape:
                     raise _lib.NmError(f"row-split launch: job(s) {shape[:8]} exceed the Adam sweep's tables (passes, vector "
                                        f"segments or vector elements; nm_rowsplit_ok) -- or the launch's group map lists them "
@@ -546,9 +562,29 @@
             self._split_pending = True
             self._pending_kinds.add(kind)
 
-    def _launch(self, step0, steps_per_tile, n_tiles, flags, scalar_tr=False):
+    def plain_pick(self) -> bool:
+        if self.wide or os.environ.get("NMHIP_PLAIN", "1") == "0":
+            return False
+        sig = tuple(j._version for j in self.jobs)
+        if sig != self._plain_sig:
+            self._plain_sig, self._plain_all = sig, all(j.plain_ok() for j in self.jobs)
+        return self._plain_all
+
+    def _launch(self, step0, steps_per_tile, n_tiles, flags, scalar_tr=False, plain: Optional[bool] = None):
         entry = "nm_launch_wide" if self.wide else ("nm_launch_scalar_tr" if scalar_tr else "nm_launch")
+        mode = flags & (_lib.NM_F_BACKWARD | _lib.NM_F_ADAM | _lib.NM_F_GRADS | _lib.NM_F_EXPORT | _lib.NM_F_ZGIVEN)
+        use_plain = (plain is not False and entry == "nm_launch" and n_tiles == 1
+                     and mode == (_lib.NM_F_BACKWARD | _lib.NM_F_ADAM) and self.plain_pick())
+        if plain and not use_plain:
+            raise ValueError("plain=True: the plain-training kernel serves whole-batch training launches of sets whose jobs all "
+                             "pass Job.plain_ok() (and NMHIP_PLAIN is not 0)")
+        if use_plain:
+            flags |= _lib.NM_F_PLAIN
         self._issue(entry, n_tiles, step0, steps_per_tile, n_tiles, flags)
+        self.last_launch = {"entry": entry, "flags": int(flags), "plain": bool(use_plain)}
+        if use_plain:
+            self._split_pending = True
+            self._pending_kinds.add("plain")
 
     def _launch_split(self, step0, n_steps, flags):
         self._issue("nm_launch_split", 1, len(self.jobs[0].kmods), step0, n_steps, flags)
@@ -605,14 +641,17 @@
         parts = self.split_parts() if split is None else (len(self.jobs[0].kmods) if split else 1)
         return ("split", parts) if parts > 1 else ("whole", 1)
 
-    def _launch_form(self, form, step0: int, n_steps: int, flags: int, helpers: Optional[int], scalar_tr: bool):
+    def _launch_form(self, form, step0: int, n_steps: int, flags: int, helpers: Optional[int], scalar_tr: bool,
+                     plain: Optional[bool] = None):
         kind, k = form
         if kind == "rowsplit":
             self._launch_rowsplit(k, step0, n_steps, flags, helpers)
         elif kind == "split":
             self._launch_split(step0, n_steps, flags)
         else:
-            self._launch(step0, n_steps, 1, flags, scalar_tr)
+            self._launch(step0, n_steps, 1, flags, scalar_tr, plain)
+            return
+        self.last_launch = {"entry": kind, "flags": int(flags), "plain": False}
 
     def _check_jobs(self, head: Optional[str] = None, caller: str = "", at_step: bool = True) -> int:
         step0 = self.jobs[0].step
@@ -633,11 +672,11 @@
             j.t += n_steps
 
     def train(self, n_steps: int, scalar_tr: bool = False, profile: bool = False, split: Optional[bool] = None,
-              rowsplit: Optional[int] = None, helpers: Optional[int] = None):
+              rowsplit: Optional[int] = None, helpers: Optional[int] = None, plain: Optional[bool] = None):
         step0 = self._check_jobs()
         flags = _lib.NM_F_BACKWARD | _lib.NM_F_ADAM | (_lib.NM_F_PROFILE if profile else 0)
         form = ("whole", 1) if scalar_tr else self._training_form(split, rowsplit)
-        self._launch_form(form, step0, n_steps, flags, helpers, scalar_tr)
+        self._launch_form(form, step0, n_steps, flags, helpers, scalar_tr, plain)
         self._advance(n_steps)
 
     def grads(self, step: Optional[int] = None, export: bool = True, scalar_tr: bool = False, split: bool = False,
```
